# jiangzhongshi/SurfaceNetworks

Hardware: AMD Instinct MI355X
Metric: meshes/sec fwd+bwd, Dirac temporal-predict (higher is better)
Workload: dtype f32; 1 GPU; as_rigid_as_possible Dirac temporal prediction: 64 grid-cloth meshes 71x71 (V=5041,F=9800) per GPU, C=128, 15 layers, fwd+loss+bwd+allreduce+Adam; meshes_per_gpu=64, global_batch=64, parallelism=dp1 (mesh sharding, flat-bucket RCCL all-reduce), world_size=1, rccl_ranks=1, collective_backend=nccl, devices_visible=1, operator_format=q3, operators=pool, grad_bucket_bytes=4075488

## Files before the change

include/sn_spmm.h:

```cpp
#ifndef SN_SPMM_H_
#define SN_SPMM_H_

#include <stddef.h>
#include <stdint.h>

#ifdef __cplusplus
extern "C" {
#endif

#define SN_ABI_VERSION 1

#define SN_OK            0
#define SN_E_NULL       -1
#define SN_E_SHAPE      -2
#define SN_E_RANGE      -3
#define SN_E_LD         -4
#define SN_E_ALIGN      -5
#define SN_E_WORKSPACE  -6
#define SN_E_UNSUPPORTED -7

int         sn_abi_version(void);
const char *sn_status_string(int status);

int sn_spmm_csr_f32(const int32_t *rowptr, const int32_t *colind, const float *vals,
                    int64_t M, int64_t K, int64_t nnz,
                    const float *X, int64_t ldx, int32_t x_group,
                    int32_t N,
                    float *Y, int64_t ldy, int32_t y_group,
                    void *stream);

size_t sn_spmm_csr_stats_workspace_bytes(int64_t M);
int sn_spmm_csr_stats_f32(const int32_t *rowptr, const int32_t *colind, const float *vals, int64_t M, int64_t K, int64_t nnz,
                          const float *X, int64_t ldx, int32_t x_group, int32_t N, float *Y, int64_t ldy, int32_t y_group,
                          double *stats_part, void *workspace, size_t workspace_bytes, void *stream);

int sn_spmm_bsr4_f32(const int32_t *b_rowptr, const int32_t *b_colind, const float *b_vals,
                     int64_t Mb, int64_t Kb, int64_t nblocks,
                     const float *X, int64_t ldx, int32_t x_group,
                     int32_t N,
                     float *Y, int64_t ldy, int32_t y_group,
                     void *stream);

int sn_spmm_q3_f32(const int32_t *b_rowptr, const float *q_blk, int64_t Mb, int64_t Kb, int64_t nblocks,
                   const float *X, int64_t ldx, int32_t x_group, int32_t N,
                   float *Y, int64_t ldy, int32_t y_group, void *stream);
size_t sn_spmm_q3_stats_workspace_bytes(int64_t Mb);
int32_t sn_spmm_q3_stats_blocks(void);
int sn_spmm_q3_stats_f32(const int32_t *b_rowptr, const float *q_blk, int64_t Mb, int64_t Kb, int64_t nblocks, const float *X,
                         int64_t ldx, int32_t x_group, int32_t N, float *Y, int64_t ldy, int32_t y_group, double *stats_part,
                         void *workspace, size_t workspace_bytes, void *stream);
int sn_spmm_q3_elubwd_f32(const int32_t *b_rowptr, const float *q_blk, int64_t Mb, int64_t Kb, int64_t nblocks,
                          const float *X, int64_t ldx, int32_t x_group, int32_t N,
                          const float *E, int64_t lde, const float *G, int64_t ldg,
                          float *Y, int64_t ldy, int32_t y_group, void *stream);
int64_t sn_spmm_q3_absmax_blocks(int64_t Mb, int32_t N);
int sn_spmm_q3_elubwd_absmax_f32(const int32_t *b_rowptr, const float *q_blk, int64_t Mb, int64_t Kb, int64_t nblocks,
                                 const float *X, int64_t ldx, int32_t x_group, int32_t N, const float *E, int64_t lde,
                                 const float *G, int64_t ldg, float *Y, int64_t ldy, int32_t y_group, float *y_absmax,
                                 void *stream);
int sn_bsr4_to_q3_f32(const int32_t *b_colind, const float *b_vals, int64_t nblocks, float *q_blk,
                      int32_t *not_quaternion, void *stream);

int sn_spmm_csr_elubwd_f32(const int32_t *rowptr, const int32_t *colind, const float *vals,
                           int64_t M, int64_t K, int64_t nnz,
                           const float *X, int64_t ldx, int32_t x_group,
                           int32_t N,
                           const float *E, int64_t lde, const float *G, int64_t ldg,
                           float *Y, int64_t ldy, int32_t y_group,
                           void *stream);
int sn_spmm_bsr4_elubwd_f32(const int32_t *b_rowptr, const int32_t *b_colind, const float *b_vals,
                            int64_t Mb, int64_t Kb, int64_t nblocks,
                            const float *X, int64_t ldx, int32_t x_group,
                            int32_t N,
                            const float *E, int64_t lde, const float *G, int64_t ldg,
                            float *Y, int64_t ldy, int32_t y_group,
                            void *stream);

int sn_coo_to_csr_i32(const int64_t *idx_batch, const int64_t *idx_row, const int64_t *idx_col,
                      int64_t nnz, int64_t B, int64_t R, int64_t Kb,
                      int32_t *rowptr, int32_t *colind,
                      void *stream);

size_t sn_csr_transpose_workspace_bytes(int64_t M, int64_t K, int64_t nnz);
int sn_csr_transpose_f32(const int32_t *rowptr, const int32_t *colind, const float *vals,
                         int64_t M, int64_t K, int64_t nnz,
                         int32_t *t_rowptr, int32_t *t_colind, float *t_vals,
                         void *workspace, size_t workspace_bytes,
                         void *stream);

size_t sn_scan_workspace_bytes(int64_t n);
int sn_bsr4_count(const int32_t *rowptr, const int32_t *colind, int64_t M, int64_t K,
                  int32_t *b_rowptr, void *workspace, size_t workspace_bytes, void *stream);
int sn_bsr4_fill(const int32_t *rowptr, const int32_t *colind, const float *vals, int64_t M, int64_t K,
                 const int32_t *b_rowptr, int32_t *b_colind, float *b_vals, void *stream);

int sn_rb4_count(const int32_t *rowptr, const int32_t *colind, int64_t M, int64_t K, int32_t *b_ptr,
                 void *workspace, size_t workspace_bytes, void *stream);
int sn_rb4_fill(const int32_t *rowptr, const int32_t *colind, const float *vals, int64_t M, int64_t K,
                const int32_t *b_ptr, int32_t *b_col, float *b_val, void *stream);
int sn_spmm_rb4_f32(const int32_t *b_ptr, const int32_t *b_col, const float *b_val, int64_t M, int64_t K, int64_t capacity,
                    const float *X, int64_t ldx, int32_t N, float *Y, int64_t ldy, void *stream);
int sn_spmm_rb4_elubwd_f32(const int32_t *b_ptr, const int32_t *b_col, const float *b_val, int64_t M, int64_t K,
                           int64_t capacity, const float *X, int64_t ldx, int32_t N, const float *E, int64_t lde,
                           const float *G, int64_t ldg, float *Y, int64_t ldy, void *stream);
int64_t sn_spmm_rb4_absmax_blocks(int64_t M, int32_t N);
int sn_spmm_rb4_elubwd_absmax_f32(const int32_t *b_ptr, const int32_t *b_col, const float *b_val, int64_t M, int64_t K,
                                  int64_t capacity, const float *X, int64_t ldx, int32_t N, const float *E, int64_t lde,
                                  const float *G, int64_t ldg, float *Y, int64_t ldy, float *y_absmax, void *stream);
size_t sn_spmm_rb4_stats_workspace_bytes(int64_t M);
int sn_spmm_rb4_stats_f32(const int32_t *b_ptr, const int32_t *b_col, const float *b_val, int64_t M, int64_t K,
                          int64_t capacity, const float *X, int64_t ldx, int32_t N, float *Y, int64_t ldy,
                          double *stats_part, void *workspace, size_t workspace_bytes, void *stream);
// ... 190 lines not shown
int64_t sn_graph_apsp_max_vertices(void);
int32_t sn_graph_apsp_group(int64_t n);
int32_t sn_graph_apsp_threads(int64_t n);
int sn_graph_apsp_f32(const int32_t *rowptr, const int32_t *colind, const float *w, int64_t n, int64_t src_begin,
                      int64_t src_count, float *out, int64_t ldo, int32_t *unreached, void *stream);
int sn_graph_apsp_sweeps_f32(const int32_t *rowptr, const int32_t *colind, const float *w, int64_t n, int64_t src_begin,
                             int64_t src_count, float *out, int64_t ldo, int32_t *unreached, int32_t *sweeps, void *stream);
int sn_symmetrize_min_f32(float *G, int64_t n, int64_t ld, void *stream);

#define SN_MESH_CORNER_BYTES 40
size_t sn_mesh_corners_workspace_bytes(int64_t nV);
int sn_mesh_corners_f32(const float *V, const int32_t *F, int64_t nV, int64_t nF, int32_t *cptr, void *corners,
                        int32_t *status_flag, void *workspace, size_t workspace_bytes, void *stream);
int sn_mesh_geodesics_f32(const int32_t *cptr, const void *corners, int64_t n, int64_t src_begin, int64_t src_count,
                          float *out, int64_t ldo, int32_t *flags, void *stream);
int sn_mesh_geodesics_sweeps_f32(const int32_t *cptr, const void *corners, int64_t n, int64_t src_begin, int64_t src_count,
                                 float *out, int64_t ldo, int32_t *flags, int32_t *sweeps, void *stream);

#define SN_IDT_BAD_FACE       1
#define SN_IDT_NOT_CONVERGED  2
#define SN_IDT_DEGENERATE     4
#define SN_IDT_NON_MANIFOLD   8
#define SN_IDT_ORIENTATION    16
#define SN_IDT_THRESHOLD      (-1e-12)
size_t sn_mesh_glue_workspace_bytes(int64_t nV, int64_t nF);
int sn_mesh_glue_i32(const float *V, const int32_t *F, int64_t nV, int64_t nF, int32_t *G, double *l, int32_t *status,
                     void *workspace, size_t workspace_bytes, void *stream);
size_t sn_mesh_idt_workspace_bytes(int64_t nF);
int sn_mesh_idt_rounds_f64(int32_t *Fp, double *lp, int32_t *G, int64_t nF, int32_t round_begin, int32_t round_count,
                           int32_t max_rounds, int32_t *counters, int32_t *status, void *workspace, size_t workspace_bytes,
                           void *stream);
int64_t sn_mesh_idt_laplacian_items(int64_t nV, int64_t nF);
size_t sn_mesh_idt_laplacian_workspace_bytes(int64_t nV, int64_t nF);
int sn_mesh_idt_laplacian_f32(const int32_t *Fp, const double *lp, int64_t nV, int64_t nF, int32_t phase, int64_t *keys,
                              const int64_t *order, int32_t *rowptr, int32_t *colind, float *vals, int32_t *status,
                              void *workspace, size_t workspace_bytes, void *stream);

int sn_linear_fwd_f32(const float *x, int64_t ldx, const float *W, int64_t ldw, const float *bias,
                      const float *residual, int64_t ldr, float *y, int64_t ldy, float *y_elu, int64_t lde,
                      int64_t rows, int32_t K, int32_t J, double *elu_stats_part ,
                      void *stream);
int sn_linear_dgrad_f32(const float *dy, int64_t lddy, const float *W, int64_t ldw, const float *x, int64_t ldx,
                        const float *center, const float *B, const float *Cc, float *dx, int64_t lddx,
                        int64_t rows, int32_t J, int32_t C, void *stream);
int sn_linear_dgrad_elu_f32(const float *dy, int64_t lddy, const float *W, int64_t ldw, const float *x, int64_t ldx,
                            const float *center, const float *B, const float *Cc, float *dx_hi, int64_t lddx,
                            float *gact, int64_t ldga, const float *gadd, int64_t ldgadd,
                            int64_t rows, int32_t J, int32_t C, void *stream);
int32_t sn_linear_dgrad_absmax_blocks(void);
int sn_linear_dgrad_elu_absmax_f32(const float *dy, int64_t lddy, const float *W, int64_t ldw, const float *x, int64_t ldx,
                                   const float *center, const float *B, const float *Cc, float *dx_hi, int64_t lddx,
                                   float *gact, int64_t ldga, const float *gadd, int64_t ldgadd,
                                   int64_t rows, int32_t J, int32_t C, float *gact_absmax, void *stream);
int sn_linear_fwd_segbias_f32(const float *x, int64_t ldx, const float *W, int64_t ldw, const float *segbias,
                              int64_t rows_per_seg, const float *residual, int64_t ldr, float *y, int64_t ldy,
                              float *y_elu, int64_t lde, int64_t rows, int32_t K, int32_t J, double *elu_stats_part,
                              void *stream);
int sn_linear_dgrad_eluseg_f32(const float *dy, int64_t lddy, const float *W, int64_t ldw, const float *x, int64_t ldx,
                               const float *center, const float *B, const float *Cc, const float *segvec,
                               int64_t rows_per_seg, const float *rowmask, float *gact, int64_t ldga, const float *gadd,
                               int64_t ldgadd, int64_t rows, int32_t J, int32_t C, void *stream);
int sn_linear_fwd_tiles_f32(const float *x, int64_t ldx, const float *W, int64_t ldw, const float *bias, const float *residual,
                            int64_t ldr, float *y, int64_t ldy, float *y_elu, int64_t lde, int64_t rows, int32_t K, int32_t J,
                            double *elu_stats_part, float *tile_sums, void *stream);
int sn_linear_fwd_segbias_tiles_f32(const float *x, int64_t ldx, const float *W, int64_t ldw, const float *segbias,
                                    int64_t rows_per_seg, const float *residual, int64_t ldr, float *y, int64_t ldy, float *y_elu,
                                    int64_t lde, int64_t rows, int32_t K, int32_t J, double *elu_stats_part, float *tile_sums,
                                    void *stream);
int sn_avg_stats_from_tiles_f32(const float *tile_sums, const double *stats_part, int32_t nblk, const float *e, int64_t ld,
                                const float *mask, const float *inv_count, int64_t rows_per_seg, int64_t nseg, int32_t C,
                                float *m, double *stats, float *workspace, void *stream);
int sn_avg_stats_from_tiles_ragged_f32(const float *tile_sums, const double *stats_part, int32_t nblk, const float *e, int64_t ld,
                                       const int64_t *segoff, const float *inv_count, int64_t nseg, int32_t C, float *m,
                                       double *stats, float *workspace, void *stream);
int sn_linear_fwd_segbias_ragged_tiles_f32(const float *x, int64_t ldx, const float *W, int64_t ldw, const float *segbias,
                                           const int64_t *segoff, int32_t nseg, const float *residual, int64_t ldr, float *y,
                                           int64_t ldy, float *y_elu, int64_t lde, int64_t rows, int32_t K, int32_t J,
                                           double *elu_stats_part, float *tile_sums, void *stream);
int sn_linear_fwd_segbias_ragged_f32(const float *x, int64_t ldx, const float *W, int64_t ldw, const float *segbias,
                                     const int64_t *segoff, int32_t nseg, const float *residual, int64_t ldr, float *y,
                                     int64_t ldy, float *y_elu, int64_t lde, int64_t rows, int32_t K, int32_t J,
                                     double *elu_stats_part, void *stream);
int sn_linear_dgrad_eluseg_ragged_f32(const float *dy, int64_t lddy, const float *W, int64_t ldw, const float *x, int64_t ldx,
                                      const float *center, const float *B, const float *Cc, const float *segvec,
                                      const int64_t *segoff, int32_t nseg, float *gact, int64_t ldga, const float *gadd,
                                      int64_t ldgadd, int64_t rows, int32_t J, int32_t C, void *stream);
int sn_linear_dgrad_eluseg_absmax_f32(const float *dy, int64_t lddy, const float *W, int64_t ldw, const float *x, int64_t ldx,
                                      const float *center, const float *B, const float *Cc, const float *segvec,
                                      int64_t rows_per_seg, const float *rowmask, float *gact, int64_t ldga, const float *gadd,
                                      int64_t ldgadd, int64_t rows, int32_t J, int32_t C, float *gact_absmax, void *stream);
int sn_linear_dgrad_eluseg_ragged_absmax_f32(const float *dy, int64_t lddy, const float *W, int64_t ldw, const float *x,
                                             int64_t ldx, const float *center, const float *B, const float *Cc,
                                             const float *segvec, const int64_t *segoff, int32_t nseg, float *gact, int64_t ldga,
                                             const float *gadd, int64_t ldgadd, int64_t rows, int32_t J, int32_t C,
                                             float *gact_absmax, void *stream);

typedef struct sn_plan sn_plan;
int sn_plan_create(sn_plan **out);
int sn_plan_destroy(sn_plan *plan);
int32_t sn_plan_lookup(const char *entry_point_name);
int32_t sn_plan_entry_count(void);
const char *sn_plan_entry_name(int32_t fn);
const char *sn_plan_entry_signature(int32_t fn);
int64_t sn_plan_length(const sn_plan *plan);
int sn_plan_add_call(sn_plan *plan, int32_t fn, int32_t nargs, const int32_t *kind, const int32_t *slot, const int64_t *ival,
                     const double *dval);
// ... 17 lines not shown
```

surfacenetworks_amd/_lib.py:

```python
from __future__ import annotations

import ctypes as C
import os
import threading

_HERE = os.path.dirname(os.path.abspath(__file__))
LIB_PATH = os.path.join(_HERE, "libsn_hip.so")

_vp, _i64, _i32, _sz = C.c_void_p, C.c_int64, C.c_int32, C.c_size_t

SIGNATURES = {
    "sn_abi_version": (C.c_int, []),
    "sn_status_string": (C.c_char_p, [C.c_int]),
    "sn_spmm_csr_f32": (C.c_int, [_vp, _vp, _vp, _i64, _i64, _i64, _vp, _i64, _i32, _i32, _vp, _i64, _i32, _vp]),
    "sn_spmm_csr_stats_workspace_bytes": (_sz, [_i64]),
    "sn_spmm_csr_stats_f32": (C.c_int, [_vp, _vp, _vp, _i64, _i64, _i64, _vp, _i64, _i32, _i32, _vp, _i64, _i32, _vp, _vp, _sz, _vp]),
    "sn_spmm_bsr4_f32": (C.c_int, [_vp, _vp, _vp, _i64, _i64, _i64, _vp, _i64, _i32, _i32, _vp, _i64, _i32, _vp]),
    "sn_spmm_csr_elubwd_f32": (C.c_int, [_vp, _vp, _vp, _i64, _i64, _i64, _vp, _i64, _i32, _i32, _vp, _i64, _vp, _i64, _vp, _i64,
                                         _i32, _vp]),
    "sn_spmm_bsr4_elubwd_f32": (C.c_int, [_vp, _vp, _vp, _i64, _i64, _i64, _vp, _i64, _i32, _i32, _vp, _i64, _vp, _i64, _vp, _i64,
                                          _i32, _vp]),
    "sn_spmm_q3_f32": (C.c_int, [_vp, _vp, _i64, _i64, _i64, _vp, _i64, _i32, _i32, _vp, _i64, _i32, _vp]),
    "sn_spmm_q3_stats_workspace_bytes": (_sz, [_i64]),
    "sn_spmm_q3_stats_blocks": (_i32, []),
# ... 5 lines not shown
    "sn_csr_transpose_f32": (C.c_int, [_vp, _vp, _vp, _i64, _i64, _i64, _vp, _vp, _vp, _vp, _sz, _vp]),
    "sn_scan_workspace_bytes": (_sz, [_i64]),
    "sn_bsr4_count": (C.c_int, [_vp, _vp, _i64, _i64, _vp, _vp, _sz, _vp]),
    "sn_bsr4_fill": (C.c_int, [_vp, _vp, _vp, _i64, _i64, _vp, _vp, _vp, _vp]),
    "sn_rb4_count": (C.c_int, [_vp, _vp, _i64, _i64, _vp, _vp, _sz, _vp]),
    "sn_rb4_fill": (C.c_int, [_vp, _vp, _vp, _i64, _i64, _vp, _vp, _vp, _vp]),
    "sn_spmm_rb4_f32": (C.c_int, [_vp, _vp, _vp, _i64, _i64, _i64, _vp, _i64, _i32, _vp, _i64, _vp]),
    "sn_spmm_rb4_elubwd_f32": (C.c_int, [_vp, _vp, _vp, _i64, _i64, _i64, _vp, _i64, _i32, _vp, _i64, _vp, _i64, _vp, _i64, _vp]),
    "sn_spmm_rb4_absmax_blocks": (_i64, [_i64, _i32]),
    "sn_spmm_rb4_elubwd_absmax_f32": (C.c_int, [_vp, _vp, _vp, _i64, _i64, _i64, _vp, _i64, _i32, _vp, _i64, _vp, _i64, _vp, _i64, _vp, _vp]),
    "sn_spmm_rb4_stats_workspace_bytes": (_sz, [_i64]),
    "sn_spmm_rb4_stats_f32": (C.c_int, [_vp, _vp, _vp, _i64, _i64, _i64, _vp, _i64, _i32, _vp, _i64, _vp, _vp, _sz, _vp]),
    "sn_spmm_csr_ring_f32": (C.c_int, [_vp, _vp, _vp, _i64, _i64, _i64, _vp, _i64, _i32, _vp, _i64, _vp]),
    "sn_spmm_csr_ring_elubwd_f32": (C.c_int, [_vp, _vp, _vp, _i64, _i64, _i64, _vp, _i64, _i32, _vp, _i64, _vp, _i64, _vp, _i64, _vp]),
    "sn_spmm_csr_ring_absmax_blocks": (_i64, [_i64, _i32]),
    "sn_spmm_csr_ring_elubwd_absmax_f32": (C.c_int, [_vp, _vp, _vp, _i64, _i64, _i64, _vp, _i64, _i32, _vp, _i64, _vp, _i64, _vp, _i64, _vp,
                                                     _vp]),
    "sn_spmm_csr_ring_stats_workspace_bytes": (_sz, [_i64]),
    "sn_spmm_csr_ring_stats_f32": (C.c_int, [_vp, _vp, _vp, _i64, _i64, _i64, _vp, _i64, _i32, _vp, _i64, _vp, _vp, _sz, _vp]),
    "sn_spmm_csr_ring_half_window": (_i32, []),
    "sn_csr_band_i32": (C.c_int, [_vp, _vp, _i64, _i64, _vp, _vp]),
    "sn_blockdiag_concat_i32": (C.c_int, [_vp, _vp, _vp, _vp, _i64, _i64, _i64, _i64, _i32, _vp, _vp, _vp, _vp]),
    "sn_blockdiag_concat_ragged_i32": (C.c_int, [_vp, _vp, _vp, _vp, _i64, _i64, _i64, _i64, _i32, _vp, _vp, _vp, _vp]),
    "sn_validate_csr_i32": (C.c_int, [_vp, _vp, _vp, _i64, _i64, _i64, _vp, _vp]),
    "sn_elu_into_f32": (C.c_int, [_vp, _i64, _vp, _i64, _i64, _i32, _vp]),
    "sn_elu_bwd_acc_f32": (C.c_int, [_vp, _i64, _vp, _i64, _vp, _i64, _vp, _i64, _vp, _i64, _i64, _i32, _i32, _vp]),
    "sn_colstats_workspace_bytes": (_sz, [_i64, _i32]),
    "sn_colstats_f32": (C.c_int, [_vp, _i64, _i64, _i32, _vp, _vp, _sz, _vp]),
    "sn_wgrad_workspace_bytes": (_sz, [_i64, _i32, _i32]),
    "sn_wgrad_f32": (C.c_int, [_vp, _i64, _vp, _i64, _vp, _i64, _i32, _i32, _vp, _vp, _vp, _sz, _vp]),
    "sn_wgrad_seg_workspace_bytes": (_sz, [_i64, _i64, _i32, _i32]),
    "sn_wgrad_seg_f32": (C.c_int, [_vp, _i64, _vp, _i64, _vp, _i64, _i64, _i32, _i32, _vp, _vp, _vp, _vp, _sz, _vp]),
    "sn_wgrad_slabs_f32": (C.c_int, [_vp, _i64, _vp, _i64, _vp, _i64, _vp, _i32, _vp, _i32, _i32, _i32, _vp, _vp, _vp, _vp, _sz, _vp]),
    "sn_wgrad_bounded_f32": (C.c_int, [_vp, _i64, _vp, _i64, _vp, _i64, _i32, _i32, _vp, _vp, _vp, _sz, _vp, _i64, _vp, _i64, _vp]),
    "sn_wgrad_seg_bounded_f32": (C.c_int, [_vp, _i64, _vp, _i64, _vp, _i64, _i64, _i32, _i32, _vp, _vp, _vp, _vp, _sz, _vp, _i64, _vp,
                                           _i64, _vp]),
    "sn_wgrad_slabs_bounded_f32": (C.c_int, [_vp, _i64, _vp, _i64, _vp, _i64, _vp, _i32, _vp, _i32, _i32, _i32, _vp, _vp, _vp, _vp, _sz,
                                             _vp, _i64, _vp, _i64, _vp]),
    "sn_avg_prep_ragged_f32": (C.c_int, [_vp, _vp, _i64, _i32, _vp, _i32, _vp, _vp]),
    "sn_bn_fold_seg_f32": (C.c_int, [_vp, _i64, _vp, _vp, _vp, _vp, _i32, _i32, C.c_double, C.c_double, _vp, _vp, _vp, _vp, _vp, _vp, _vp,
                                     _vp, _vp, _vp, _i64, _vp, _vp]),
    "sn_avg_bn_bwd_f32": (C.c_int, [_vp, _vp, _vp, _vp, _vp, _vp, _vp, _vp, _vp, _i64, _i32, _i32, _i64, _vp, _i64, _vp, _i64, _vp, _vp,
                                    _vp, _vp, _vp, _vp, _vp, _vp, _vp]),
    "sn_linear_dgrad_absmax_blocks": (_i32, []),
    "sn_linear_dgrad_elu_absmax_f32": (C.c_int, [_vp, _i64, _vp, _i64, _vp, _i64, _vp, _vp, _vp, _vp, _i64, _vp, _i64, _vp, _i64, _i64,
                                                 _i32, _i32, _vp, _vp]),
    "sn_linear_dgrad_eluseg_absmax_f32": (C.c_int, [_vp, _i64, _vp, _i64, _vp, _i64, _vp, _vp, _vp, _vp, _i64, _vp, _vp, _i64, _vp,
                                                    _i64, _i64, _i32, _i32, _vp, _vp]),
    "sn_linear_dgrad_eluseg_ragged_absmax_f32": (C.c_int, [_vp, _i64, _vp, _i64, _vp, _i64, _vp, _vp, _vp, _vp, _vp, _i32, _vp, _i64,
                                                           _vp, _i64, _i64, _i32, _i32, _vp, _vp]),
    "sn_spmm_q3_absmax_blocks": (_i64, [_i64, _i32]),
    "sn_spmm_q3_elubwd_absmax_f32": (C.c_int, [_vp, _vp, _i64, _i64, _i64, _vp, _i64, _i32, _i32, _vp, _i64, _vp, _i64, _vp, _i64, _i32,
                                               _vp, _vp]),
    "sn_wgrad_thin_workspace_bytes": (_sz, [_i64, _i32, _i32]),
    "sn_wgrad_thin_f32": (C.c_int, [_vp, _i64, _vp, _i64, _i64, _i32, _i32, _vp, _vp, _vp, _sz, _vp]),
    "sn_masked_smooth_l1_workspace_bytes": (_sz, [_i64, _i32]),
    "sn_masked_smooth_l1_fwd_f32": (C.c_int, [_vp, _i64, _vp, _i64, _vp, _i64, _i32, C.c_double, _vp, _vp, _sz, _vp]),
    "sn_masked_smooth_l1_bwd_f32": (C.c_int, [_vp, _i64, _vp, _i64, _vp, _i64, _i32, C.c_double, _vp, _vp, _i64, _vp]),
    "sn_pair_argmin_f32": (C.c_int, [_vp, _i64, _i64, _vp, _vp, _i64, _vp, _i64, _i64, _vp, _vp]),
    "sn_pair_ce_fwd_f32": (C.c_int, [_vp, _i64, _vp, _i64, _i64, _vp, _vp, _vp]),
    "sn_pair_ce_bwd_f32": (C.c_int, [_vp, _i64, _vp, _vp, _vp, _i64, _i64, _i64, _i64, _vp, _i64, _vp]),
    "sn_pair_fused_workspace_bytes": (C.c_size_t, [_i64, _i64]),
    "sn_pair_fused_fwd_f32": (C.c_int, [_vp, _i64, _vp, _i64, _vp, _i64, _i64, _i64, _i64, C.c_int32, _vp, _vp, _vp, C.c_size_t, _vp]),
    "sn_pair_fused_bwd_f32": (C.c_int, [_vp, _vp, _vp, _i64, _i64, _i64, _i64, C.c_int32, _vp, _i64, _vp, _i64, _vp, C.c_size_t, _vp]),
    "sn_pair_loss_workspace_bytes": (C.c_size_t, [_i64, _i64]),
    "sn_pair_soft_fwd_f32": (C.c_int, [_vp, _i64, _vp, _i64, _vp, _vp, _vp, _i64, _i64, _i64, _i64, _i64, _i64, C.c_int32, _vp, _vp, _vp, C.c_size_t, _vp]),
    "sn_pair_soft_bwd_f32": (C.c_int, [_vp, _vp, _vp, _i64, _i64, _vp, _vp, _i64, _i64, _i64, _i64, C.c_int32, _vp, _i64, _vp, _i64, _vp, C.c_size_t, _vp]),
    "sn_pair_sl1_fwd_f32": (C.c_int, [_vp, _i64, _vp, _i64, _vp, _vp, _vp, _i64, _i64, _i64, _i64, _i64, _i64, C.c_int32, _vp, _vp, C.c_size_t, _vp]),
    "sn_pair_sl1_bwd_f32": (C.c_int, [_vp, _vp, _vp, _i64, _i64, _vp, _i64, _i64, _i64, _i64, C.c_int32, _vp, _i64, _vp, _i64, _vp, C.c_size_t, _vp]),
    "sn_pair_match_workspace_bytes": (C.c_size_t, [_i64, _i64]),
    "sn_pair_match_f32": (C.c_int, [_vp, _i64, _vp, _i64, _i64, _i64, _i64, _i64, C.c_int32, _vp, _vp, _vp, _vp, _vp, _i64, _vp, _vp, _vp,
                                    C.c_size_t, _vp]),
    "sn_gather_segments_f32": (C.c_int, [_vp, _vp, _i64, _i64, _i64, _i32, _vp, _vp]),
    "sn_gather_segments_ragged_f32": (C.c_int, [_vp, _vp, _vp, _i64, _i64, _i64, _i32, _vp, _vp]),
    "sn_linear_thin_fwd_f32": (C.c_int, [_vp, _i64, _vp, _i64, _vp, _i64, _i32, _i32, _vp, _i64, _vp, _i64, _vp]),
    "sn_bn_fold_f32": (C.c_int, [_vp, _i64, _vp, _vp, _vp, _vp, _i32, _i32, C.c_double, C.c_double, _i32, _vp, _vp, _vp,
                                 _vp, _vp, _vp, _vp, _vp, _vp, _vp]),
    "sn_colstats_blocks": (C.c_int32, [_i64]),
    "sn_wgrad_bounded_enabled": (C.c_int32, []),
    "sn_gemm_variant": (C.c_int32, []),
    "sn_colstats_merge2_f64": (C.c_int, [_vp, C.c_int32, C.c_int32, C.c_int32, _vp, C.c_int32, C.c_int32, C.c_int32, _vp, _vp]),
    "sn_colstats_partial_f32": (C.c_int, [_vp, _i64, _i64, C.c_int32, _vp, _vp]),
    "sn_bn_bwd_coeffs_f32": (C.c_int, [_vp, _vp, _vp, _vp, _vp, _vp, _i64, _i32, _i32, _vp, _vp, _vp, _vp, _vp, _vp, _vp]),
    "sn_segment_colsum_ragged_workspace_bytes": (_sz, [_i64, _i32]),
    "sn_segment_colsum_ragged_f32": (C.c_int, [_vp, _i64, _vp, _i64, _vp, _i64, _i32, _vp, _vp, _vp, _sz, _vp]),
    "sn_bcast_rows_ragged_f32": (C.c_int, [_vp, _vp, _i64, _vp, _i64, _i32, _vp]),
    "sn_segment_colsum_workspace_bytes": (_sz, [_i64, _i64, _i32]),
    "sn_segment_colsum_f32": (C.c_int, [_vp, _i64, _vp, _i64, _i64, _i32, _vp, _vp, _sz, _vp]),
    "sn_bcast_rows_f32": (C.c_int, [_vp, _vp, _i64, _i64, _i64, _i32, _vp]),
    "sn_elu_bwd_bcast_f32": (C.c_int, [_vp, _i64, _vp, _i64, _vp, _vp, _vp, _i64, _vp, _i64, _i64, _i64, _i32, _vp]),
    "sn_dirac_workspace_bytes": (_sz, [_i64, _i64]),
    "sn_dirac_bsr4_from_mesh": (C.c_int, [_vp, _vp, _i64, _i64, _vp, _vp, _vp, _vp, _vp, _vp, _vp, _vp, _vp, _sz, _vp]),
    "sn_timing_enable": (C.c_int, [_i32]),
    "sn_timing_count": (_i64, []),
    "sn_timing_drain": (C.c_int, [_vp, _vp, _i64, _vp]),
    "sn_laplacian_workspace_bytes": (_sz, [_i64, _i64]),
    "sn_laplacian_csr_from_mesh": (C.c_int, [_vp, _vp, _i64, _i64, _i32, _vp, _vp, _vp, _vp, _vp, _sz, _vp]),
    "sn_edge_lengths_csr_f32": (C.c_int, [_vp, _vp, _vp, _i64, _vp, _vp]),
    "sn_graph_apsp_max_vertices": (_i64, []),
    "sn_graph_apsp_group": (_i32, [_i64]),
    "sn_graph_apsp_threads": (_i32, [_i64]),
    "sn_graph_apsp_f32": (C.c_int, [_vp, _vp, _vp, _i64, _i64, _i64, _vp, _i64, _vp, _vp]),
    "sn_graph_apsp_sweeps_f32": (C.c_int, [_vp, _vp, _vp, _i64, _i64, _i64, _vp, _i64, _vp, _vp, _vp]),
    "sn_symmetrize_min_f32": (C.c_int, [_vp, _i64, _i64, _vp]),
    "sn_mesh_corners_workspace_bytes": (_sz, [_i64]),
    "sn_mesh_corners_f32": (C.c_int, [_vp, _vp, _i64, _i64, _vp, _vp, _vp, _vp, _sz, _vp]),
# ... 109 lines not shown
```

surfacenetworks_amd/blocks.py:

```python
from __future__ import annotations

import weakref

import torch

from . import kernels, plans
from .functional import (SpmmTimer, _launch, _rows2d, product_form, avg_stage_backward, avg_stage_backward_ragged, avg_stage_forward,
                         avg_stage_forward_ragged, bn_prepare, bnlin_backward,
                         bnlin_backward_elu_input, bnlin_backward_zero_first, bnlin_forward, bnlin_forward_zero_first, stash, unstash,
                         zero_first_supported)
from .graphs import active_capture
from .operators import as_operator

__all__ = ["lap_block", "dirac_block", "avg_block", "avg_block_ragged", "avg_block_ragged_ok", "take_activated", "attach_activated", "zero_faces_ok", "elu_conv", "elu_conv_ok"]


def _version_of(t: torch.Tensor):
    return None if t.is_inference() else t._version


def attach_activated(t: torch.Tensor, cat: torch.Tensor) -> torch.Tensor:
    t._sn_cat = (cat, _version_of(t))
    return t


def take_activated(t: torch.Tensor, rows: int, C: int):
    d = getattr(t, "__dict__", None)
    entry = d.pop("_sn_cat", None) if d is not None else None
    if entry is None:
        return None
    cat, version = entry
    if version != _version_of(t) or tuple(cat.shape) != (rows, 2 * C) or cat.device != t.device or cat.dtype != torch.float32:
        return None
    return cat


def _new_cat(rows, C, device):
    return torch.empty((rows, 2 * C), dtype=torch.float32, device=device)


def _new_part(rows, C, device, narrow=False):
    if not (C == 128 or (narrow and C == 64 and kernels.linear_fwd_supported(2 * C, C))) or not kernels.elu_stats_supported():
        return None
    return kernels.new_elu_stats_part(rows, device)


def _attach_part(cat, part, tiles=None):
    if part is not None:
        cat._sn_part = part
        if tiles is not None:
            cat._sn_tiles = tiles


_TILE_SUMS_MIN_ROWS = 32768


def _new_tiles(rows, C, device, part, wanted):
    if not wanted or part is None or C != 128 or rows < _TILE_SUMS_MIN_ROWS or not kernels.tile_sums_supported():
        return None
    return kernels.new_tile_sums(rows, device)


def _wants_tiles(mod, avg_next) -> bool:
    if avg_next is None:
        return bool(mod.__dict__.get("_sn_avg_next", False))
    return bool(avg_next)

# ... 39 lines not shown


_MISSING = object()


def _op_operands(ops, ncols):
    arrays, key = [], []
    for op, group in ops:
        for o in (op, op.t()):
            kind, arr, scal = product_form(o, group, ncols)
            arrays.extend(arr)
            key.append((kind, scal))
    return arrays, tuple(key)


def _plan_forward(ctx, site, impl, tensors, ops, consts, ncols, n_dyn, scan):
    op_arrays, op_key = _op_operands(ops, ncols) if ops else ((), ())
    ext, attr_key = plans.expand_ext(tensors, scan)
    ext.extend(op_arrays)
    dyn = tensors[:n_dyn]
    ptrs = [t.data_ptr() if t is not None else 0 for t in dyn]
    key = (tuple([None if t is None else (t.shape, t.stride(), t.dtype) for t in dyn]),
           tuple([None if t is None else t.shape for t in tensors[n_dyn:]]), attr_key, op_key, consts,
           tuple([ptrs.index(p_) for p_ in ptrs]),
           _TILE_SUMS_MIN_ROWS)
    plan, may_record = site.lookup(key)
    if plan is None:
        if not may_record:
            return None
        plan = plans.record(site, key, impl, (*tensors, *[o for o, _ in ops], *consts), ext, tensors[0].device, range(n_dyn))
        if plan is None:
            return None
        need = set()

        def slots(d):
            if isinstance(d, plans._Desc):
                if d.slot >= 2:
                    need.add(d.slot - 2)
            elif isinstance(d, tuple):
                for v in d:
                    slots(v)
        slots(plan.result[1])
        plan.saved_ext = sorted(need)
    timer = SpmmTimer.active
    if timer is not None:
        if plan.tags is None:
            return None
        timer.tags.extend(plan.tags)
    big, small = plan.new_arenas(tensors[0].device)
    plan.run(big, small, ext)
    site.replayed += 1
    build = plans._Builder(big, small, ext)
    outs = build(plan.result[0])
    if plan.effects:
        plans.apply_effects(plan, build)
    ctx._sn_plan = (plan, big, small, [ext[j] for j in plan.saved_ext], ops, ncols)
    return outs


def _plan_backward(ctx, site, impl, grads, consts):
    state = ctx._sn_plan
    if state is None:
        raise RuntimeError("a second backward through a block that ran from a launch plan (retain_graph): its workspace was "
                           "released by the first one; run with SN_PLANS=0 for that")
    fplan, big, small, kept, ops, ncols = state
    ctx._sn_plan = None
    op_arrays, op_key = _op_operands(ops, ncols) if ops else ((), ())
    maxima = [kernels.take_absmax(g) if g is not None else None for g in grads]
    ext = [big, small, *kept, *grads, *maxima, *op_arrays]
    gptrs = [g.data_ptr() if g is not None else 0 for g in grads]
    key = (tuple([None if g is None else (g.shape, g.stride(), g.dtype) for g in grads]), tuple([m is not None for m in maxima]),
           op_key, consts, tuple([gptrs.index(p_) for p_ in gptrs]))
    plan = fplan.bwd.get(key, _MISSING)
    if plan is _MISSING or plan is None:
        fext = [None] * fplan.n_ext
        for j, t in zip(fplan.saved_ext, kept):
            fext[j] = t
        saved = plans._Builder(big, small, fext)(fplan.result[1])
        plans.renote(grads, maxima)
        if plan is None:
            return impl(saved, *[o for o, _ in ops], *grads, *consts)
        g0 = 2 + len(kept)
        plan = plans.record(site, (id(fplan), key), impl, (saved, *[o for o, _ in ops], *grads, *consts), ext,
                            grads_device(grads, big, small), range(g0, g0 + len(grads)))
        fplan.bwd[key] = plan
        if plan is None:
            plans.renote(grads, maxima)
            return impl(saved, *[o for o, _ in ops], *grads, *consts)
        for g in grads:
            if g is not None:
                kernels.take_absmax(g)
    timer = SpmmTimer.active
    if timer is not None:
        if plan.tags is None:
            fext = [None] * fplan.n_ext
            for j, t in zip(fplan.saved_ext, kept):
                fext[j] = t
            plans.renote(grads, maxima)
            return impl(plans._Builder(big, small, fext)(fplan.result[1]), *[o for o, _ in ops], *grads, *consts)
        timer.tags.extend(plan.tags)
    b2, s2 = plan.new_arenas(grads_device(grads, big, small))
    plan.run(b2, s2, ext)
    site.replayed += 1
    build = plans._Builder(b2, s2, ext)
    out = build(plan.result)
    if plan.effects:
        plans.apply_effects(plan, build)
    return out


def grads_device(grads, *others):
    for t in (*grads, *others):
        if t is not None:
            return t.device
    raise ValueError("no tensor to take the device from")


_SITES = {name: plans.Site(name) for name in ("dirac_fwd", "dirac_bwd", "propagate_fwd", "propagate_bwd", "avg_fwd", "avg_bwd",
                                              "avg_ragged_fwd", "avg_ragged_bwd", "elu_conv_fwd", "elu_conv_bwd")}


_NAN = {}


def _nan_placeholder(device):
    t = _NAN.get(device)
    if t is None:
        t = torch.full((1, 1), float("nan"), dtype=torch.float32, device=device)
        if device.type != "cuda" or not torch.cuda.is_current_stream_capturing():
            _NAN[device] = t
    return t


def _dirac_fwd(v, f, pre_v, pre_f, g0, b0, W0, c0, rm0, rv0, g1, b1, W1, c1, rm1, rv1, opDi, opDiA, need_f, avg_next, tr0, mo0,
               ep0, tr1, mo1, ep1):
    rv, C = v.shape
    rf = opDi.shape[0] // 4
    cat1 = _activated(v, pre_v)
    nxt_f = _new_cat(rf, C, v.device)
    pf = _new_part(rf, C, v.device, narrow=True)
    if f is None:
        cat0 = torch.empty((rf, C), dtype=torch.float32, device=v.device)
        _attach_hi(cat0, _launch(opDi, cat1[:, :C], cat0, 4, "fwd", stats=tr0))
        f_out, st0 = bnlin_forward_zero_first(cat0, g0, b0, W0, c0, rm0, rv0, tr0, mo0, ep0, nxt_f[:, :C], need_f, pf)
    else:
        cat0 = pre_f if pre_f is not None else _activated(f, None)
        _attach_hi(cat0, _launch(opDi, cat1[:, :C], cat0[:, C:], 4, "fwd", stats=tr0))
        f_out, st0 = bnlin_forward(cat0, g0, b0, W0, c0, rm0, rv0, tr0, mo0, ep0, None, nxt_f[:, :C], want_y=need_f,
                                   elu_stats=pf)
    _attach_part(nxt_f, pf)
    _attach_hi(cat1, _launch(opDiA, nxt_f[:, :C], cat1[:, C:], 4, "fwd", stats=tr1))
    nxt_v = _new_cat(rv, C, v.device)
    pv = _new_part(rv, C, v.device, narrow=True)
    tv = _new_tiles(rv, C, v.device, pv, avg_next)
    v_new, st1 = bnlin_forward(cat1, g1, b1, W1, c1, rm1, rv1, tr1, mo1, ep1, v, nxt_v[:, :C], elu_stats=pv, tile_sums=tv)
    _attach_part(nxt_v, pv, tv)
    return (v_new, f_out, nxt_v, nxt_f), ((cat0, cat1, nxt_f), st0, st1)


def _dirac_bwd(saved, opDi, opDiA, g_vnew, g_fo, f_zero, need_gv, need_gf):
    (cat0, cat1, nxt_f), st0, st1 = saved
    C = cat1.shape[1] // 2
    dev = cat1.device
    gp1 = (None,) * 4
    h1 = None
    if g_vnew is not None:
        (dx1_hi, h1), dg1, db1, dW1, dc1 = bnlin_backward(st1, g_vnew, through_elu=(g_vnew,))
        gp1 = (dg1, db1, dW1, dc1)
        g_sum = torch.empty((nxt_f.shape[0], C), dtype=torch.float32, device=dev)
        _launch(opDiA.t(), dx1_hi, g_sum, 4, "bwd", elubwd=(nxt_f[:, :C], g_fo))
        g_fo = g_sum
    gp0 = (None,) * 4
    g_v = g_f = None
    dx0_hi = None
    if g_fo is not None and f_zero:
        dx0_hi, dg0, db0, dW0, dc0 = bnlin_backward_zero_first(st0, g_fo)
        gp0 = (dg0, db0, dW0, dc0)
    elif g_fo is not None:
        (dx0_hi, g_f), dg0, db0, dW0, dc0 = bnlin_backward(st0, g_fo, through_elu=(None,))
        gp0 = (dg0, db0, dW0, dc0)
    if need_gv:
        if dx0_hi is not None:
            g_v = torch.empty((cat1.shape[0], C), dtype=torch.float32, device=dev)
            _launch(opDi.t(), dx0_hi, g_v, 4, "bwd", elubwd=(cat1[:, :C], h1))
        else:
            g_v = h1
    if f_zero or not need_gf:
        g_f = None
    return (g_v, g_f) + gp0 + gp1


class _DiracBlock(torch.autograd.Function):

    @staticmethod
    def forward(ctx, v, f, opDi, opDiA, pre_v, pre_f, need_f, avg_next, g0, b0, W0, c0, rm0, rv0, tr0, mo0, ep0, g1, b1, W1, c1,
                rm1, rv1, tr1, mo1, ep1):
        v = _rows2d(v)
        if f is not None and pre_f is None:
            f = _rows2d(f)
        ctx.f_zero = f is None
        ctx.ops = (opDi, opDiA)
        tensors = (v, f, pre_v, pre_f, g0, b0, W0, c0, rm0, rv0, g1, b1, W1, c1, rm1, rv1)
        consts = (need_f, avg_next, tr0, mo0, ep0, tr1, mo1, ep1)
        outs = None
        ctx._sn_plan = None
        if plans.usable(v):
            outs = _plan_forward(ctx, _SITES["dirac_fwd"], _dirac_fwd, tensors, ((opDi, 4), (opDiA, 4)), consts, v.shape[1], 4, (2, 3, 8, 14))
            if outs is not None:
                _drop_counters(rm0, rm1)
        ctx._sn_planned = outs is not None
        if outs is None:
            outs, saved = _dirac_fwd(*tensors, opDi, opDiA, *consts)
            stash(ctx, *saved)
        v_new, f_out, nxt_v, nxt_f = outs
        if f_out is None:
            f_out = _nan_placeholder(v.device).expand(nxt_f.shape[0], v.shape[1])
        ctx.mark_non_differentiable(nxt_v, nxt_f)
        ctx.set_materialize_grads(False)
        return v_new, f_out, nxt_v, nxt_f

    @staticmethod
    def backward(ctx, g_vnew, g_fout, _gv, _gf):
        if g_vnew is None and g_fout is None:
            return (None,) * 26
        opDi, opDiA = ctx.ops
        g_vnew = g_vnew.contiguous() if g_vnew is not None else None
        g_fout = g_fout.contiguous() if g_fout is not None else None
        consts = (ctx.f_zero, bool(ctx.needs_input_grad[0]), bool(ctx.needs_input_grad[1]))
        if ctx._sn_planned:
            r = _plan_backward(ctx, _SITES["dirac_bwd"], _dirac_bwd, (g_vnew, g_fout), consts)
        else:
            r = _dirac_bwd(unstash(ctx), opDi, opDiA, g_vnew, g_fout, *consts)
        none5 = (None,) * 5
        return (r[0], r[1], None, None, None, None, None, None) + r[2:6] + none5 + r[6:10] + none5


def _drop_counters(*running_means) -> None:
    for rm in running_means:
        d = getattr(rm, "__dict__", None)
        if d is not None:
            d.pop("_sn_nbt", None)


def dirac_block(mod, Di, DiA, v, f, need_f=True, num_faces=None, avg_next=None):
    B, V, C = v.shape
    F_ = f.shape[1] if f is not None else int(num_faces)
    rv, rf = B * V, B * F_
    opDi, opDiA = as_operator(Di), as_operator(DiA)
    if opDi.shape != (4 * rf, 4 * rv) or opDiA.shape != (4 * rv, 4 * rf):
        raise ValueError(f"DirResNet2: Di {tuple(opDi.shape)} / DiA {tuple(opDiA.shape)} do not match v rows {rv}, f rows {rf}")
    v_new, f_out, nxt_v, nxt_f = _DiracBlock.apply(v.reshape(rv, C), f.reshape(rf, C) if f is not None else None, opDi, opDiA,
                                                  take_activated(v, rv, C),
                                                  take_activated(f, rf, C) if f is not None else None, bool(need_f),
                                                  _wants_tiles(mod, avg_next), *_bn_args(mod._modules["bn_fc0"]), *_bn_args(mod._modules["bn_fc1"]))
    _mark_producer(nxt_v, mod, avg_next)
    return attach_activated(v_new.view(B, V, C), nxt_v), attach_activated(f_out.view(B, F_, C), nxt_f)


def zero_faces_ok(mod, C: int) -> bool:
    return zero_first_supported(C, mod.bn_fc0.fc.weight.shape[0]) and mod.bn_fc0.fc.weight.shape[1] == 2 * C


def _propagate_fwd(x, pre, mask_rows, inv_count, g0, b0, W0, c0, rm0, rv0, g1, b1, W1, c1, rm1, rv1, op, nseg, avg_next, tr0, mo0,
                   ep0, tr1, mo1, ep1):
    rows, C = x.shape
    per = rows // nseg if nseg else 0

    def propagate(cat, training):
        if op is not None:
            _attach_hi(cat, _launch(op, cat[:, :C], cat[:, C:], 1, "fwd", stats=training))
        else:
            mean = kernels.segment_colsum(cat[:, :C], mask_rows, per, nseg) * inv_count
            kernels.bcast_rows(mean, cat[:, C:], per)

    cat_a = _activated(x, pre)
    propagate(cat_a, tr0)
    cat_b = _new_cat(rows, C, x.device)
    pb = _new_part(rows, C, x.device)
    _, st0 = bnlin_forward(cat_a, g0, b0, W0, c0, rm0, rv0, tr0, mo0, ep0, None, cat_b[:, :C],
                           want_y=False, elu_stats=pb)
    _attach_part(cat_b, pb)
# ... 339 lines not shown
```

surfacenetworks_amd/csrc/sn_gemm.hip:

```cpp
#include <hip/hip_runtime.h>
#include <hip/hip_ext.h>
#include <stdint.h>
#include <stdlib.h>

#include "sn_spmm.h"

int sn_internal_cu_count();
hipError_t sn_internal_fill(void *dst, int value, size_t bytes, hipStream_t s);
hipError_t sn_internal_copy2d(void *dst, int64_t dpitch, const void *src, int64_t spitch, int64_t width, int64_t rows, hipStream_t s);
bool sn_internal_timing_slot(int kind, int64_t rows, int64_t width, int64_t bytes, int outw, hipEvent_t *s, hipEvent_t *e);

namespace {

constexpr int kWG = 256;
#define kCUs sn_internal_cu_count()
typedef float f4 __attribute__((ext_vector_type(4)));
typedef float f16v __attribute__((ext_vector_type(16)));

inline int launch_status() {
  const hipError_t e = hipGetLastError();
  return e == hipSuccess ? SN_OK : (int)e;
}
inline bool aligned16(const void *p) { return (reinterpret_cast<uintptr_t>(p) & 15u) == 0; }
inline bool ld32(int64_t a, int64_t b = 0, int64_t c = 0, int64_t d = 0, int64_t e = 0) {
// ... 193 lines not shown
}
__device__ __forceinline__ unsigned row16_umax(unsigned v) {
  v = dpp_umax<0xB1>(v);
  v = dpp_umax<0x4E>(v);
  v = dpp_umax<0x141>(v);
  v = dpp_umax<0x140>(v);
  return v;
}

template <int I>
struct IC {
  static constexpr int value = I;
};
template <int I, int N, class F>
__device__ __forceinline__ void static_for(F &&f) {
  if constexpr (I < N) {
    f(IC<I>{});
    static_for<I + 1, N>(f);
  }
}

#define SN_LDS_BARRIER() asm volatile("s_waitcnt lgkmcnt(0)\n\ts_barrier" ::: "memory")

typedef __amdgpu_buffer_rsrc_t rsrc_t;
struct RowWindow {
  const char *p;
  int step;
  int n_full, n_last;
  __device__ __forceinline__ void init(const float *base, int64_t ld, int64_t row0, int last_rows, int span) {
    step = 128 * (int)ld;
    p = reinterpret_cast<const char *>(base + row0 * ld);
    n_full = 4 * (31 * (int)ld + span);
    n_last = 4 * ((last_rows - 1) * (int)ld + span);
  }
  __device__ __forceinline__ void init_empty() {
    step = 0;
    p = nullptr;
    n_full = n_last = 0;
  }
  __device__ __forceinline__ void next() { p += step; }
  __device__ __forceinline__ void stride(int g) { step *= g; }
  __device__ __forceinline__ rsrc_t rsrc(int to_last) const {
    const int n = to_last > 0 ? n_full : (to_last == 0 ? n_last : 0);
    return __builtin_amdgcn_make_buffer_rsrc(const_cast<char *>(p), 0, n, 0x00020000);
  }
};
__device__ __forceinline__ f4 bld4(rsrc_t r, int voff) {
  return __builtin_bit_cast(f4, __builtin_amdgcn_raw_buffer_load_b128(r, voff, 0, 0));
}
__device__ __forceinline__ void bst4(rsrc_t r, int voff, const f4 &v) {
  __builtin_amdgcn_raw_buffer_store_b128(__builtin_bit_cast(u4, v), r, voff, 0, 2);
}

template <int PC, int K, int NT, bool TRANSW, int EPI, bool SIDE, bool ELU, bool SMALL = false, int WV = 4>
__global__ __launch_bounds__(64 * WV, (PC == 2 && K == 128 && NT == 1 && WV == 4) ? 2 : 1) void gemm_rows_split_k(const float *__restrict__ In, int64_t ldi,
                                                         const float *__restrict__ W, int64_t ldw,
                                                         float *__restrict__ Out, int64_t ldo, int64_t rows, EpiArgs ep) {
  constexpr int KS = K / 16;
  constexpr int RS = 2 * K + 16;
  constexpr int PART = 32 * RS;
  constexpr int SEG = K / 64;
  constexpr int NCH = 8 / WV;
  constexpr int NL = NCH * SEG;
  constexpr int CSTEP = KS / 2;
  constexpr int NOUT = 32 * WV * NT;
  constexpr int CPR = 8 * NT;
  constexpr int SROW = 16 * CPR + 16;
  constexpr int RPI = 64 / CPR;
  constexpr int NST = 32 / RPI;
  static_assert(PC == 2, "two fp16 pieces");
  __shared__ __attribute__((aligned(16))) unsigned char img[2][PC][PART];
  __shared__ __attribute__((aligned(16))) unsigned char stg[WV][32 * SROW];
  __shared__ float s_rs[2][32];
  __shared__ float s_amax[WV];
  __shared__ __attribute__((aligned(16))) float s_cs[NOUT];
  const int wave = __builtin_amdgcn_readfirstlane(threadIdx.x >> 6), lane = threadIdx.x & 63;
  const int n = lane & 31, h = lane >> 5;
  u4 wh[NT][KS], wl[NT][KS];
  constexpr int kOob = 0x7fffff00;
  const f4 zero4 = {0.f, 0.f, 0.f, 0.f};
  auto load_w = [&](int col, int ks, f4 &p, f4 &q) {
    if constexpr (!TRANSW) {
      p = q = zero4;
      if (col < ep.jv) {
        p = *reinterpret_cast<const f4 *>(W + (int64_t)col * ldw + 16 * ks + 8 * h);
        q = *reinterpret_cast<const f4 *>(W + (int64_t)col * ldw + 16 * ks + 8 * h + 4);
      }
    } else {
      const int k0w = 16 * ks + 8 * h;
      const float *w0 = W + (int64_t)k0w * ldw + col;
      p = q = zero4;
      if (k0w < ep.jv) p = f4{w0[0], w0[ldw], w0[2 * ldw], w0[3 * ldw]};
      if (k0w + 4 < ep.jv) q = f4{w0[4 * ldw], w0[5 * ldw], w0[6 * ldw], w0[7 * ldw]};
    }
  };
#pragma unroll
  for (int t = 0; t < NT; ++t) {
    const int col = 32 * (wave * NT + t) + n;
    float cup = 1.f;
    constexpr bool ONEPASS = SMALL && !(PC == 2 && K == 128 && NT == 1 && !TRANSW && !SIDE);
    f4 wp[ONEPASS ? KS : 1], wq[ONEPASS ? KS : 1];
    if constexpr (ONEPASS) {
#pragma unroll
      for (int ks = 0; ks < KS; ++ks) load_w(col, ks, wp[ks], wq[ks]);
    }
    {
      float cm = 0.f;
#pragma unroll
      for (int ks = 0; ks < KS; ++ks) {
        f4 p, q;
        if constexpr (ONEPASS) p = wp[ks], q = wq[ks];
        else load_w(col, ks, p, q);
        cm = fmaxf(cm, fmaxf(absmax4(p), absmax4(q)));
      }
      cm = fmaxf(cm, __shfl_xor(cm, 32));
      float cdown;
      pow2_scales(cm, cup, cdown);
      if (h == 0) s_cs[col] = cdown;
    }
#pragma unroll
    for (int ks = 0; ks < KS; ++ks) {
      f4 p, q;
      if constexpr (ONEPASS) p = wp[ks], q = wq[ks];
      else load_w(col, ks, p, q);
      split8_h2(p, q, cup, wh[t][ks], wl[t][ks]);
    }
  }
  __syncthreads();
  const int64_t ntiles = (rows + 31) / 32;
  const int64_t per = (ntiles + gridDim.x - 1) / gridDim.x;
  const int G = ep.interleave ? (int)gridDim.x : 1;
  int64_t tile = G > 1 ? (int64_t)blockIdx.x : (int64_t)blockIdx.x * per;
  const int64_t tend = G > 1 ? ntiles : (tile + per < ntiles ? tile + per : ntiles);
  constexpr bool STATS = (EPI == EPI_FWD) && ELU && NT == 1;
  if (tile >= tend) {
    if constexpr (STATS)
      if (ep.stats)
        for (int64_t b = blockIdx.x; b < ep.stats_blocks; b += gridDim.x) ep.stats[b * 256 + threadIdx.x] = 0.0;
    if constexpr (EPI == EPI_DGRAD_ELU)
      if (ep.absmax && threadIdx.x == 0)
        for (int b = blockIdx.x; b < kAbsmaxBlocks; b += gridDim.x) ep.absmax[b] = 0.f;
    return;
  }
  float amax = 0.f;
  double ssum[STATS ? 4 : 1], ssq[STATS ? 4 : 1];
#pragma unroll
  for (int i = 0; i < (STATS ? 4 : 1); ++i) ssum[i] = ssq[i] = 0.0;
  const int erow = lane / CPR;
  const int ecol = 32 * NT * wave + 4 * (lane % CPR);
  f4 k0 = {0.f, 0.f, 0.f, 0.f}, k1 = k0, k2 = k0;
  constexpr bool DGE = (EPI == EPI_DGRAD_ELU);
  static_assert(!DGE || SIDE, "the ELU variant needs the BatchNorm tail operand");
  const bool lowhalf = DGE && 32 * NT * wave < ep.half;
  const bool colv = EPI != EPI_FWD || ecol < ep.jv;
  if constexpr (EPI == EPI_FWD) {
    if (colv) k0 = *reinterpret_cast<const f4 *>(ep.v0 + ecol);
  } else if constexpr (SIDE) {
    if (ep.v1) k0 = *reinterpret_cast<const f4 *>(ep.v1 + ecol);
    k1 = *reinterpret_cast<const f4 *>(ep.v2 + ecol);
    k2 = *reinterpret_cast<const f4 *>(ep.v3 + ecol);
  }
  const f4 kcs = *reinterpret_cast<const f4 *>(s_cs + ecol);
  unsigned char *const sw = &stg[wave][0] + n * SROW + 16 * h;
  const unsigned char *const sr = &stg[wave][0] + erow * SROW + 16 * (lane % CPR);
  const float *side_p = (EPI == EPI_FWD) ? ep.v1 : ep.v0;
  const bool has_out = (EPI != EPI_FWD && !DGE) || Out != nullptr;
  const bool has_ga = DGE && lowhalf && ep.v4 != nullptr;
  const int vo_side = colv ? 4 * (erow * (int)ep.ld1 + ecol) : kOob, js_side = 4 * RPI * (int)ep.ld1;
  const int vo_out = colv ? 4 * (erow * (int)ldo + ecol) : kOob, js_out = 4 * RPI * (int)ldo;
  const int vo_o2 = colv ? 4 * (erow * (int)ep.ld2 + ecol) : kOob, js_o2 = 4 * RPI * (int)ep.ld2;
  const int vo_ga = 4 * (erow * (int)ep.ld3 + ecol), js_ga = 4 * RPI * (int)ep.ld3;
  RowWindow w_in, w_side, w_out, w_o2, w_ga;
  const int64_t row0 = tile * 32;
  const int last_nrt = (int)(rows - (ntiles - 1) * 32);
  int to_last = (int)(ntiles - 1 - tile);
  const int ispan = EPI == EPI_FWD ? K : ep.jv;
  const int ospan = EPI == EPI_FWD ? ep.jv : NOUT;
  w_in.init(In, ldi, row0, last_nrt, ispan);
  if constexpr (SIDE) w_side.init(side_p, ep.ld1, row0, last_nrt, ospan);
  if (has_out) w_out.init(Out, ldo, row0, last_nrt, ospan);
  else w_out.init_empty();
  if constexpr (DGE || (EPI == EPI_FWD && ELU)) w_o2.init(ep.o2, ep.ld2, row0, last_nrt, DGE ? ep.half : ospan);
  if constexpr (DGE) {
    if (has_ga) w_ga.init(ep.v4, ep.ld3, row0, last_nrt, ep.half);
    else w_ga.init_empty();
  }
  if (G > 1) {
    w_in.stride(G);
    if constexpr (SIDE) w_side.stride(G);
    w_out.stride(G);
    if constexpr (DGE || (EPI == EPI_FWD && ELU)) w_o2.stride(G);
    if constexpr (DGE) w_ga.stride(G);
  }
  const bool useseg = (ep.period > 0 || ep.segoff != nullptr) && (EPI == EPI_FWD || (DGE && lowhalf));
  int64_t seg_m = 0;
  int seg_left = 0;
  if (useseg) {
    if (ep.segoff) {
      int lo = 0, hi = ep.nseg - 1;
      while (lo < hi) {
        const int mid = (lo + hi + 1) >> 1;
        if (ep.segoff[mid] <= row0) lo = mid;
        else hi = mid - 1;
      }
      seg_m = lo;
      seg_left = (int)(ep.segoff[lo + 1] - row0);
    } else {
      seg_m = row0 / ep.period;
      seg_left = (int)((seg_m + 1) * ep.period - row0);
    }
  }

  const int lr = lane >> 4, lc = lane & 15;
  const int lrow = 4 * NCH * wave + lr;
  int lvo[SEG];
#pragma unroll
  for (int s = 0; s < SEG; ++s)
    lvo[s] = (EPI == EPI_FWD || 64 * s + 4 * lc < ep.jv) ? 4 * (lrow * (int)ldi + 4 * lc) + 256 * s : kOob;
  const int lps = 16 * (int)ldi;
  f4 raw[NL];
  auto load_chunk = [&](rsrc_t r, int p) {
#pragma unroll
    for (int s = 0; s < SEG; ++s) raw[p * SEG + s] = bld4(r, lvo[s] + p * lps);
  };
  auto convert_chunk = [&](int buf, int p) {
    unsigned char *d = &img[buf][0][0] + (lrow + 4 * p) * RS + 8 * lc;
    float m = absmax4(raw[p * SEG]);
#pragma unroll
    for (int s = 1; s < SEG; ++s) m = fmaxf(m, absmax4(raw[p * SEG + s]));
    float up, down;
    pow2_scales(__uint_as_float(row16_umax(__float_as_uint(m))), up, down);
#pragma unroll
    for (int s = 0; s < SEG; ++s) {
      u2 H, L;
      split4_h2(raw[p * SEG + s], up, H, L);
      *reinterpret_cast<u2 *>(d + 128 * s) = H;
      *reinterpret_cast<u2 *>(d + 128 * s + PART) = L;
    }
    if (lc == 0) s_rs[buf][lrow + 4 * p] = down;
  };
  {
    const rsrc_t r0 = w_in.rsrc(to_last);
#pragma unroll
    for (int p = 0; p < NCH; ++p) load_chunk(r0, p);
    w_in.next();
    const rsrc_t r1 = w_in.rsrc(to_last - G);
#pragma unroll
    for (int p = 0; p < NCH; ++p) {
      convert_chunk(0, p);
      load_chunk(r1, p);
    }
    w_in.next();
  }

  auto do_tile = [&](auto bufc, int64_t tl) {
    constexpr int buf = decltype(bufc)::value;
    SN_LDS_BARRIER();
    const rsrc_t r_in = w_in.rsrc(to_last - 2 * G);
    const int nrt = to_last == 0 ? last_nrt : 32;
    f4 sd[NST];
    if constexpr (SIDE) {
      const rsrc_t r_side = w_side.rsrc(to_last);
#pragma unroll
      for (int j = 0; j < NST; ++j) sd[j] = bld4(r_side, vo_side + j * js_side);
    }
    f4 sg0 = {0.f, 0.f, 0.f, 0.f}, sg1 = sg0;
    float smk[NST];
    int nb = 32;
    const bool usemask = DGE && useseg && ep.rowmask != nullptr;
    if (useseg) {
      while (seg_left <= 0) {
        ++seg_m;
        seg_left += ep.segoff ? (int)(ep.segoff[seg_m + 1] - ep.segoff[seg_m]) : (int)ep.period;
      }
      nb = seg_left < nrt ? seg_left : nrt;
      const float *s0 = ep.segv + seg_m * ep.ldseg + (colv ? ecol : 0);
      const float *s1 = nb < nrt ? s0 + ep.ldseg : s0;
      sg0 = *reinterpret_cast<const f4 *>(s0);
      sg1 = *reinterpret_cast<const f4 *>(s1);
      if constexpr (DGE) {
        if (usemask) {
          const float *mrow = ep.rowmask + tl * 32;
#pragma unroll
          for (int j = 0; j < NST; ++j) {
            const int rt = erow + RPI * j;
            smk[j] = mrow[rt < nrt ? rt : nrt - 1];
          }
        }
      }
    }
    f4 ga[NST];
    if constexpr (DGE) {
      if (lowhalf) {
        const rsrc_t r_ga = w_ga.rsrc(to_last);
#pragma unroll
        for (int j = 0; j < NST; ++j) ga[j] = bld4(r_ga, vo_ga + j * js_ga);
      }
    }
    f16v acc0[NT], acc1[NT];
    const f16v zero = {0.f, 0.f, 0.f, 0.f, 0.f, 0.f, 0.f, 0.f, 0.f, 0.f, 0.f, 0.f, 0.f, 0.f, 0.f, 0.f};
    const unsigned char *fp = &img[buf][0][0] + n * RS + 16 * h;
    constexpr int LOWP = PART;
    const float rs = s_rs[buf][n];
    u4 dh = *reinterpret_cast<const u4 *>(fp), dl = *reinterpret_cast<const u4 *>(fp + LOWP);
    static_for<0, KS>([&](auto ic) {
      constexpr int ks = decltype(ic)::value;
      __builtin_amdgcn_sched_barrier(0);
      u4 nh, nl;
      if constexpr (ks + 1 < KS) {
        nh = *reinterpret_cast<const u4 *>(fp + 32 * (ks + 1));
        nl = *reinterpret_cast<const u4 *>(fp + LOWP + 32 * (ks + 1));
      }
      if constexpr (ks % CSTEP == 0 && ks / CSTEP < NCH) {
        constexpr int p = ks / CSTEP;
        convert_chunk(buf ^ 1, p);
        load_chunk(r_in, p);
      }
#pragma unroll
      for (int t = 0; t < NT; ++t) acc1[t] = mfma_f16(wl[t][ks], dh, ks == 0 ? zero : acc1[t]);
#pragma unroll
      for (int t = 0; t < NT; ++t) acc0[t] = mfma_f16(wh[t][ks], dh, ks == 0 ? zero : acc0[t]);
#pragma unroll
      for (int t = 0; t < NT; ++t) acc1[t] = mfma_f16(wh[t][ks], dl, acc1[t]);
      if constexpr (ks + 1 < KS) {
        dh = nh; dl = nl;
      }
    });
    __builtin_amdgcn_sched_barrier(0);
#pragma unroll
    for (int t = 0; t < NT; ++t)
#pragma unroll
      for (int g = 0; g < 4; ++g)
        *reinterpret_cast<f4 *>(sw + 128 * t + 32 * g) =
            f4{__builtin_fmaf(acc1[t][4 * g], kLowDown, acc0[t][4 * g]) * rs,
               __builtin_fmaf(acc1[t][4 * g + 1], kLowDown, acc0[t][4 * g + 1]) * rs,
               __builtin_fmaf(acc1[t][4 * g + 2], kLowDown, acc0[t][4 * g + 2]) * rs,
               __builtin_fmaf(acc1[t][4 * g + 3], kLowDown, acc0[t][4 * g + 3]) * rs};
    const rsrc_t r_out = w_out.rsrc(to_last);
    rsrc_t r_o2 = r_out;
    if constexpr (DGE || (EPI == EPI_FWD && ELU)) r_o2 = w_o2.rsrc(to_last);
    auto out_row = [&](int j) {
      f4 v = *reinterpret_cast<const f4 *>(sr + RPI * j * SROW);
      v *= kcs;
      if constexpr (EPI == EPI_FWD) {
        if (useseg) v += (erow + RPI * j < nb ? sg0 : sg1);
        else v += k0;
        if constexpr (SIDE) v += sd[j];
      } else if constexpr (SIDE) {
        const f4 xv = sd[j] - k0;
        v.x += __builtin_fmaf(xv.x, k1.x, k2.x);
        v.y += __builtin_fmaf(xv.y, k1.y, k2.y);
        v.z += __builtin_fmaf(xv.z, k1.z, k2.z);
        v.w += __builtin_fmaf(xv.w, k1.w, k2.w);
      }
      return v;
    };
    if constexpr (DGE) {
      if (lowhalf) {
#pragma unroll
        for (int j = 0; j < NST; ++j) {
          f4 v = out_row(j);
          const f4 o = sd[j];
          if (useseg) {
            f4 sv = erow + RPI * j < nb ? sg0 : sg1;
            if (usemask) sv *= smk[j];
            v += sv;
          }
          v = f4{__builtin_fmaf(v.x, fminf(o.x, 0.f), v.x), __builtin_fmaf(v.y, fminf(o.y, 0.f), v.y),
                 __builtin_fmaf(v.z, fminf(o.z, 0.f), v.z), __builtin_fmaf(v.w, fminf(o.w, 0.f), v.w)};
          v += ga[j];
          bst4(r_o2, vo_o2 + j * js_o2, v);
          const float m4 = fmaxf(fmaxf(__builtin_fabsf(v.x), __builtin_fabsf(v.y)), fmaxf(__builtin_fabsf(v.z), __builtin_fabsf(v.w)));
          amax = (erow + RPI * j < nrt) ? fmaxf(amax, m4) : amax;
        }
      } else {
#pragma unroll
        for (int j = 0; j < NST; ++j) bst4(r_out, vo_out + j * js_out, out_row(j));
      }
    } else {
      f4 tsum = {0.f, 0.f, 0.f, 0.f};
#pragma unroll
      for (int j = 0; j < NST; ++j) {
        const f4 v = out_row(j);
        bst4(r_out, vo_out + j * js_out, v);
        if constexpr (EPI == EPI_FWD && ELU) {
          const f4 ev = f4{elu1(v.x), elu1(v.y), elu1(v.z), elu1(v.w)};
          bst4(r_o2, vo_o2 + j * js_o2, ev);
          if constexpr (STATS) {
            if (erow + RPI * j < nrt) {
              const double e0 = ev.x, e1 = ev.y, e2 = ev.z, e3 = ev.w;
              ssum[0] += e0; ssum[1] += e1; ssum[2] += e2; ssum[3] += e3;
              ssq[0] = __builtin_fma(e0, e0, ssq[0]); ssq[1] = __builtin_fma(e1, e1, ssq[1]);
              ssq[2] = __builtin_fma(e2, e2, ssq[2]); ssq[3] = __builtin_fma(e3, e3, ssq[3]);
              tsum += ev;
            }
          }
        }
      }
      if constexpr (STATS) {
        if (ep.tile_sums) {
#pragma unroll
          for (int o = CPR; o < 64; o <<= 1) {
            tsum.x += __shfl_xor(tsum.x, o); tsum.y += __shfl_xor(tsum.y, o);
            tsum.z += __shfl_xor(tsum.z, o); tsum.w += __shfl_xor(tsum.w, o);
          }
          if (erow == 0) *reinterpret_cast<f4 *>(ep.tile_sums + tl * 128 + ecol) = tsum;
        }
      }
    }
    w_in.next();
// ... 236 lines not shown
    }
    w_in.next();
    to_last -= G;
    if constexpr (SIDE) w_side.next();
    w_out.next();
    if constexpr (ELU) w_o2.next();
  };
  while (true) {
    do_tile(IC<0>{});
    if ((tile += G) >= tend) break;
    do_tile(IC<1>{});
    if ((tile += G) >= tend) break;
  }
  if constexpr (STATS) {
    if (ep.stats) {
#pragma unroll
      for (int i = 0; i < 4; ++i)
#pragma unroll
        for (int o = 4; o < 64; o <<= 1) {
          ssum[i] += __shfl_xor(ssum[i], o);
          ssq[i] += __shfl_xor(ssq[i], o);
        }
      if (erow == 0) {
#pragma unroll
        for (int i = 0; i < 4; ++i) {
          ep.stats[(int64_t)blockIdx.x * 256 + ecol + i] = ssum[i];
          ep.stats[(int64_t)blockIdx.x * 256 + 128 + ecol + i] = ssq[i];
        }
      }
      if (threadIdx.x < 256)
        for (int64_t b = blockIdx.x + gridDim.x; b < ep.stats_blocks; b += gridDim.x) ep.stats[b * 256 + threadIdx.x] = 0.0;
    }
  }
}

inline int gemm_variant() {
  static const int v = [] {
    const char *e = getenv("SN_GEMM_VARIANT");
    return (e && atoi(e) == 0) ? 0 : 2;
  }();
  return v;
}

#define SN_UNPAREN(...) __VA_ARGS__
constexpr int64_t kSmallRows = 131072;
#define SN_SPLIT_LAUNCH(TARGS, ...)                                                                                    \
  do {                                                                                                                 \
    if (rows <= kSmallRows) {                                                                                          \
      if (t_start) hipExtLaunchKernelGGL((gemm_rows_split_k<2, SN_UNPAREN TARGS, true>), dim3(grid), dim3(kWG), 0, s, t_start, t_stop, 0, __VA_ARGS__); \
      else hipLaunchKernelGGL((gemm_rows_split_k<2, SN_UNPAREN TARGS, true>), dim3(grid), dim3(kWG), 0, s, __VA_ARGS__); \
    } else {                                                                                                           \
      if (t_start) hipExtLaunchKernelGGL((gemm_rows_split_k<2, SN_UNPAREN TARGS>), dim3(grid), dim3(kWG), 0, s, t_start, t_stop, 0, __VA_ARGS__); \
      else hipLaunchKernelGGL((gemm_rows_split_k<2, SN_UNPAREN TARGS>), dim3(grid), dim3(kWG), 0, s, __VA_ARGS__);     \
    }                                                                                                                  \
  } while (0)
#define SN_SPLIT_LAUNCH_NT2(K_, EPI_, SIDE_, ...) SN_SPLIT_LAUNCH((K_, 2, true, EPI_, SIDE_, false), __VA_ARGS__)

inline int gemm_wgs(int K, int NT) { return (gemm_variant() == 2 && K == 128 && NT == 1) ? 2 : 1; }
inline unsigned gemm_grid(int64_t rows, int wgs) {
  const int64_t ntiles = (rows + 31) / 32;
  int64_t b = (int64_t)kCUs * wgs;
  if (b > ntiles) b = ntiles;
  return (unsigned)(b < 1 ? 1 : b);
}

}

extern "C" {

int32_t sn_gemm_variant(void) { return gemm_variant(); }

int32_t sn_linear_fwd_stats_blocks(int64_t rows) { return rows > 0 ? (int32_t)gemm_grid(rows, 2) : 0; }

int sn_linear_fwd_f32(const float *x, int64_t ldx, const float *W, int64_t ldw, const float *bias,
                      const float *residual, int64_t ldr, float *y, int64_t ldy, float *y_elu, int64_t lde,
                      int64_t rows, int32_t K, int32_t J, double *elu_stats_part, void *stream) {
  return sn_linear_fwd_tiles_f32(x, ldx, W, ldw, bias, residual, ldr, y, ldy, y_elu, lde, rows, K, J, elu_stats_part, nullptr, stream);
}

int sn_linear_fwd_tiles_f32(const float *x, int64_t ldx, const float *W, int64_t ldw, const float *bias,
                            const float *residual, int64_t ldr, float *y, int64_t ldy, float *y_elu, int64_t lde,
                            int64_t rows, int32_t K, int32_t J, double *elu_stats_part, float *tile_sums, void *stream) {
  (void)hipGetLastError();
  if (tile_sums && (!elu_stats_part || J != 128)) return SN_E_UNSUPPORTED;
  if (rows < 0 || K < 1 || J < 1 || ldx < K || ldw < K || (y && ldy < J)) return SN_E_SHAPE;
  if (J > 128 || (J % 4) || (J != 128 && gemm_variant() == 0) || (K != 128 && K != 256) || !ld32(ldx, ldy, ldr, lde))
    return SN_E_UNSUPPORTED;
  if (rows == 0) return SN_OK;
  if (!x || !W || !bias || (!y && !(y_elu && gemm_variant() != 0))) return SN_E_NULL;
  if (!aligned16(x) || !aligned16(W) || !aligned16(bias) || (y && (!aligned16(y) || (ldy % 4))) || (ldx % 4) || (ldw % 4) ||
      (residual && (!aligned16(residual) || (ldr % 4) || ldr < J)) || (y_elu && (!aligned16(y_elu) || (lde % 4) || lde < J)))
    return SN_E_ALIGN;
  if (elu_stats_part && (!y_elu || gemm_variant() == 0)) return SN_E_UNSUPPORTED;
  EpiArgs ep{bias, residual, nullptr, nullptr, y_elu, ldr, lde, nullptr, 0, 0, nullptr, 0, 0, nullptr, elu_stats_part,
             sn_linear_fwd_stats_blocks(rows), (int)J, nullptr, 0, nullptr, 1, tile_sums};
  hipStream_t s = static_cast<hipStream_t>(stream);
  const unsigned grid = gemm_grid(rows, gemm_wgs(K, 1));
  const bool x3 = gemm_variant() != 0;
  hipEvent_t t_start = nullptr, t_stop = nullptr;
  if (x3)
    sn_internal_timing_slot(0x100 | (residual ? 2 : 0) | (y_elu ? 1 : 0) | (y ? 4 : 0), rows, K,
                            rows * 4 * ((int64_t)K + (y ? J : 0) + (residual ? J : 0) + (y_elu ? J : 0)), J, &t_start, &t_stop);
#define SN_X3_FWD(KK, RES, EL) SN_SPLIT_LAUNCH((KK, 1, false, EPI_FWD, RES, EL), x, ldx, W, ldw, y, ldy, rows, ep)
#define SN_W8_FWD(KK, RES, EL)                                                                                         \
  do {                                                                                                                 \
    if (t_start) hipExtLaunchKernelGGL((gemm_fwd_w8_k<KK, RES, EL>), dim3(grid8), dim3(512), 0, s, t_start, t_stop, 0, x, ldx, W, ldw, y, ldy, rows, ep); \
// ... 49 lines not shown
    SN_SPLIT_LAUNCH_NT2(128, EPI_DGRAD, false, dy, lddy, W, ldw, dx, lddx, rows, ep);
  else if (C == 256)
    hipLaunchKernelGGL((gemm_rows_k<128, 2, true, EPI_DGRAD>), dim3(grid), dim3(kWG), 0, s, dy, lddy, W, ldw, dx, lddx, rows, ep);
  else if (x3 && B)
    SN_SPLIT_LAUNCH((128, 1, true, EPI_DGRAD, true, false), dy, lddy, W, ldw, dx, lddx, rows, ep);
  else if (x3)
    SN_SPLIT_LAUNCH((128, 1, true, EPI_DGRAD, false, false), dy, lddy, W, ldw, dx, lddx, rows, ep);
  else
    hipLaunchKernelGGL((gemm_rows_k<128, 1, true, EPI_DGRAD>), dim3(grid), dim3(kWG), 0, s, dy, lddy, W, ldw, dx, lddx, rows, ep);
  return launch_status();
}

int32_t sn_linear_dgrad_absmax_blocks(void) { return kAbsmaxBlocks; }

int sn_linear_dgrad_elu_f32(const float *dy, int64_t lddy, const float *W, int64_t ldw, const float *x, int64_t ldx,
                            const float *center, const float *B, const float *Cc, float *dx_hi, int64_t lddx, float *gact,
                            int64_t ldga, const float *gadd, int64_t ldgadd, int64_t rows, int32_t J, int32_t C,
                            void *stream) {
  return sn_linear_dgrad_elu_absmax_f32(dy, lddy, W, ldw, x, ldx, center, B, Cc, dx_hi, lddx, gact, ldga, gadd, ldgadd, rows, J, C,
                                        nullptr, stream);
}

int sn_linear_dgrad_elu_absmax_f32(const float *dy, int64_t lddy, const float *W, int64_t ldw, const float *x, int64_t ldx,
                                   const float *center, const float *B, const float *Cc, float *dx_hi, int64_t lddx, float *gact,
                                   int64_t ldga, const float *gadd, int64_t ldgadd, int64_t rows, int32_t J, int32_t C,
                                   float *gact_absmax, void *stream) {
  (void)hipGetLastError();
  if (rows < 0 || J < 1 || C < 2 || lddy < J || ldw < C || lddx < C / 2 || ldga < C / 2 || ldx < C) return SN_E_SHAPE;
  if (J > 128 || (J % 4) || (C != 128 && C != 256) || gemm_variant() == 0 || !ld32(lddy, ldx, lddx, ldga, ldgadd))
    return SN_E_UNSUPPORTED;
  if (rows == 0) {
    if (gact_absmax && sn_internal_fill(gact_absmax, 0, kAbsmaxBlocks * sizeof(float), static_cast<hipStream_t>(stream)) != hipSuccess)
      return (int)hipGetLastError();
    return SN_OK;
  }
  if (!dy || !W || !dx_hi || !gact || !x || !B || !Cc) return SN_E_NULL;
  if (!aligned16(dy) || !aligned16(W) || !aligned16(dx_hi) || !aligned16(gact) || !aligned16(x) || !aligned16(B) ||
      !aligned16(Cc) || (center && !aligned16(center)) || (gadd && (!aligned16(gadd) || (ldgadd % 4) || ldgadd < C / 2)) ||
      (lddy % 4) || (ldw % 4) || (lddx % 4) || (ldga % 4) || (ldx % 4))
    return SN_E_ALIGN;
  const int half = C / 2;
  EpiArgs ep{x, center, B, Cc, gact, ldx, ldga, gadd, ldgadd, half, nullptr, 0, 0, nullptr, nullptr, 0, (int)J, nullptr, 0, gact_absmax, 1, nullptr};
  float *out = dx_hi - half;
  hipStream_t s = static_cast<hipStream_t>(stream);
  const unsigned grid = gemm_grid(rows, gemm_wgs(128, C / 128));
  hipEvent_t t_start = nullptr, t_stop = nullptr;
  sn_internal_timing_slot(0x200 | 2 | (gadd ? 4 : 0), rows, C, rows * 4 * ((int64_t)J + C + C + (gadd ? half : 0)), J, &t_start, &t_stop);
  if (C == 256)
    SN_SPLIT_LAUNCH_NT2(128, EPI_DGRAD_ELU, true, dy, lddy, W, ldw, out,
                       lddx, rows, ep);
  else
    SN_SPLIT_LAUNCH((128, 1, true, EPI_DGRAD_ELU, true, false), dy, lddy, W, ldw, out,
                       lddx, rows, ep);
  return launch_status();
}

static int fwd_segbias_launch(const float *x, int64_t ldx, const float *W, int64_t ldw, const float *segbias,
                              int64_t rows_per_seg, const int64_t *segoff, int32_t nseg, const float *residual, int64_t ldr,
                              float *y, int64_t ldy, float *y_elu, int64_t lde, int64_t rows, int32_t K, int32_t J,
                              double *elu_stats_part, void *stream, float *tile_sums = nullptr) {
  (void)hipGetLastError();
  if (rows < 0 || K < 1 || J < 1 || ldx < K || ldw < K || (y && ldy < J) || (!segoff && rows_per_seg < 1) || (segoff && nseg < 1))
    return SN_E_SHAPE;
  if (J > 128 || (J % 4) || (K != 128 && K != 256) || gemm_variant() == 0 || !ld32(ldx, ldy, ldr, lde) ||
      (!segoff && (rows_per_seg < 32 || rows_per_seg > 0x7fffffffLL)))
    return SN_E_UNSUPPORTED;
  if (rows == 0) return SN_OK;
  if (!x || !W || !segbias || (!y && !y_elu)) return SN_E_NULL;
  if (!aligned16(x) || !aligned16(W) || !aligned16(segbias) || (y && (!aligned16(y) || (ldy % 4))) || (ldx % 4) || (ldw % 4) ||
      (residual && (!aligned16(residual) || (ldr % 4) || ldr < J)) || (y_elu && (!aligned16(y_elu) || (lde % 4) || lde < J)))
    return SN_E_ALIGN;
  if (elu_stats_part && !y_elu) return SN_E_UNSUPPORTED;
  if (tile_sums && (!elu_stats_part || J != 128)) return SN_E_UNSUPPORTED;
  EpiArgs ep{segbias, residual, nullptr, nullptr, y_elu, ldr, lde, nullptr, 0, 0, segbias, segoff ? 0 : rows_per_seg, J, nullptr,
             elu_stats_part, sn_linear_fwd_stats_blocks(rows), (int)J, segoff, nseg, nullptr, 1, tile_sums};
  hipStream_t s = static_cast<hipStream_t>(stream);
  const unsigned grid = gemm_grid(rows, gemm_wgs(K, 1));
  hipEvent_t t_start = nullptr, t_stop = nullptr;
  sn_internal_timing_slot(0x100 | 8 | (residual ? 2 : 0) | (y_elu ? 1 : 0) | (y ? 4 : 0), rows, K,
                          rows * 4 * ((int64_t)K + (y ? J : 0) + (residual ? J : 0) + (y_elu ? J : 0)), J, &t_start, &t_stop);
  const int sel = (K == 256 ? 4 : 0) + (residual ? 2 : 0) + (y_elu ? 1 : 0);
  switch (sel) {
    case 0: SN_X3_FWD(128, false, false); break;
    case 1: SN_X3_FWD(128, false, true); break;
    case 2: SN_X3_FWD(128, true, false); break;
    case 3: SN_X3_FWD(128, true, true); break;
    case 4: SN_X3_FWD(256, false, false); break;
    case 5: SN_X3_FWD(256, false, true); break;
    case 6: SN_X3_FWD(256, true, false); break;
    default: SN_X3_FWD(256, true, true); break;
  }
  return launch_status();
}

int sn_linear_fwd_segbias_f32(const float *x, int64_t ldx, const float *W, int64_t ldw, const float *segbias,
                              int64_t rows_per_seg, const float *residual, int64_t ldr, float *y, int64_t ldy, float *y_elu,
                              int64_t lde, int64_t rows, int32_t K, int32_t J, double *elu_stats_part, void *stream) {
  return fwd_segbias_launch(x, ldx, W, ldw, segbias, rows_per_seg, nullptr, 0, residual, ldr, y, ldy, y_elu, lde, rows, K, J,
                            elu_stats_part, stream);
}

int sn_linear_fwd_segbias_tiles_f32(const float *x, int64_t ldx, const float *W, int64_t ldw, const float *segbias,
                                    int64_t rows_per_seg, const float *residual, int64_t ldr, float *y, int64_t ldy, float *y_elu,
                                    int64_t lde, int64_t rows, int32_t K, int32_t J, double *elu_stats_part, float *tile_sums,
                                    void *stream) {
  return fwd_segbias_launch(x, ldx, W, ldw, segbias, rows_per_seg, nullptr, 0, residual, ldr, y, ldy, y_elu, lde, rows, K, J,
// ... 96 lines not shown
```

surfacenetworks_amd/csrc/sn_kernels.hip:

```cpp

#include <hip/hip_runtime.h>
#include <hip/hip_ext.h>
#include <limits.h>
#include <stdint.h>
#include <stdlib.h>

#include <mutex>
#include <vector>

#include "sn_spmm.h"

int sn_internal_cu_count();
hipError_t sn_internal_fill(void *dst, int value, size_t bytes, hipStream_t s);
hipError_t sn_internal_copy2d(void *dst, int64_t dpitch, const void *src, int64_t spitch, int64_t width, int64_t rows, hipStream_t s);

namespace {

constexpr int kWG = 256;
__constant__ int c_xcd = 8;
#define kCUs sn_internal_cu_count()

typedef float f4 __attribute__((ext_vector_type(4)));

__device__ __forceinline__ f4 ld4(const float *p) { return *reinterpret_cast<const f4 *>(p); }
__device__ __forceinline__ void st4(float *p, f4 v) { *reinterpret_cast<f4 *>(p) = v; }
__device__ __forceinline__ void st4_stream(float *p, f4 v) { __builtin_nontemporal_store(v, reinterpret_cast<f4 *>(p)); }
constexpr int kStreamNT = 1;
__device__ __forceinline__ f4 ld4_s(const float *p, int nt) {
  return nt ? __builtin_nontemporal_load(reinterpret_cast<const f4 *>(p)) : *reinterpret_cast<const f4 *>(p);
}
__device__ __forceinline__ void st4_s(float *p, f4 v, int nt) {
  if (nt) __builtin_nontemporal_store(v, reinterpret_cast<f4 *>(p));
  else *reinterpret_cast<f4 *>(p) = v;
}
__device__ __forceinline__ f4 fma4(float a, f4 x, f4 acc) {
  acc.x = __builtin_fmaf(a, x.x, acc.x);
  acc.y = __builtin_fmaf(a, x.y, acc.y);
  acc.z = __builtin_fmaf(a, x.z, acc.z);
  acc.w = __builtin_fmaf(a, x.w, acc.w);
  return acc;
}

template <int G, int N>
__device__ __forceinline__ int64_t row_off(int r, int64_t ld) {
  if constexpr (G == 1) return (int64_t)r * ld;
  else return (int64_t)(r >> 2) * ld + (int64_t)(r & 3) * N;
}

__device__ __forceinline__ int my_chunk(int nchunks) {
  const int X = c_xcd;
  const int cpx = (nchunks + X - 1) / X;
  return (blockIdx.x % X) * cpx + blockIdx.x / X;
}


struct SpmmEpi {
  const float *e;
  int64_t lde;
  const float *g;
  int64_t ldg;
  float *absmax = nullptr;
};
__device__ __forceinline__ f4 fabs4(const f4 &a) {
  return f4{__builtin_fabsf(a.x), __builtin_fabsf(a.y), __builtin_fabsf(a.z), __builtin_fabsf(a.w)};
}
__device__ __forceinline__ float hmax_abs4(const f4 &a) {
  return fmaxf(fmaxf(__builtin_fabsf(a.x), __builtin_fabsf(a.y)), fmaxf(__builtin_fabsf(a.z), __builtin_fabsf(a.w)));
}
__device__ __forceinline__ float wave_max_nonneg(float m) {
  unsigned mb = __float_as_uint(m);
#pragma unroll
  for (int o = 32; o > 0; o >>= 1) {
    const unsigned other = (unsigned)__shfl_xor((int)mb, o);
    mb = other > mb ? other : mb;
  }
  return __uint_as_float(mb);
}
__device__ __forceinline__ f4 elu_bwd4(const f4 &a, const f4 &o) {
  return f4{a.x * (o.x > 0.f ? 1.f : o.x + 1.f), a.y * (o.y > 0.f ? 1.f : o.y + 1.f), a.z * (o.z > 0.f ? 1.f : o.z + 1.f),
            a.w * (o.w > 0.f ? 1.f : o.w + 1.f)};
}

template <int N, int XG, int YG, bool EPI, bool STATS>
__device__ __forceinline__ void spmm_csr_rows_body(const int *__restrict__ rowptr, const int *__restrict__ colind,
                                                   const float *__restrict__ vals, int M, const float *__restrict__ X,
                                                   int64_t ldx, float *__restrict__ Y, int64_t ldy, int nchunks, int iters,
                                                   SpmmEpi epi, float *__restrict__ stats_part) {
  constexpr int LPR = N / 4;
  constexpr int P = 64 / LPR;
  constexpr int WAVES = kWG / 64;
  constexpr int CAP = 512;
  constexpr int KB = 8;
  __shared__ int s_col[WAVES][CAP];
  __shared__ float s_val[WAVES][CAP];
  __shared__ int s_rp[WAVES][68];
  const int wave = threadIdx.x >> 6, lane = threadIdx.x & 63;
  const int sub = lane % LPR, grp = lane / LPR;
  const float *xb = X + sub * 4;
  int *sc = s_col[wave];
  float *sv = s_val[wave];
  int *rp = s_rp[wave];
  const int R = P * iters;
  const int r0 = (my_chunk(nchunks) * WAVES + wave) * R;
  if constexpr (!STATS) {
    if (r0 >= M) return;
  }
  {
    int rl = r0 + lane;
    rl = rl < M ? rl : M;
    rp[lane] = rowptr[rl];
    int re = r0 + R;
    re = re < M ? re : M;
    if (lane == 0) rp[64] = rowptr[r0 < M ? re : M];
  }
  __builtin_amdgcn_wave_barrier();
  const int k0 = rp[0];
  const int k1 = R < 64 ? rp[R] : rp[64];
  const bool fast = (k1 - k0) <= CAP;
  if (fast) {
    for (int p0 = 0; p0 < k1 - k0; p0 += 64) {
      int p = p0 + lane;
      p = p < k1 - k0 ? p : k1 - k0 - 1;
      __builtin_amdgcn_global_load_lds(colind + k0 + p, sc + p0, 4, 0, 0);
      __builtin_amdgcn_global_load_lds(vals + k0 + p, sv + p0, 4, 0, 0);
    }
    asm volatile("s_waitcnt vmcnt(0)" ::: "memory");
    __builtin_amdgcn_wave_barrier();
  }
  f4 ssum = {0.f, 0.f, 0.f, 0.f}, ssq = ssum;
  for (int i = 0; i < iters; ++i) {
    const int lr = i * P + grp;
    const int r = r0 + lr;
    const int kb = rp[lr];
// ... 178 lines not shown
      st4_stream(yp, acc0);
      st4_stream(yp + ys, acc1);
      st4_stream(yp + 2 * ys, acc2);
      st4_stream(yp + 3 * ys, acc3);
    }
  }
}
#define SN_FOUR_WAVES __attribute__((amdgpu_waves_per_eu(4, 4)))
#define SN_SIX_WAVES __attribute__((amdgpu_waves_per_eu(6, 6)))
#define SN_FIVE_WAVES __attribute__((amdgpu_waves_per_eu(5, 5)))
template <int N, int XG, int YG>
__global__ __launch_bounds__(kWG) SN_FOUR_WAVES void spmm_bsr4_lds(const int *__restrict__ b_rowptr, const int *__restrict__ b_colind,
                                                     const float *__restrict__ b_vals, int Mb,
                                                     const float *__restrict__ X, int64_t ldx,
                                                     float *__restrict__ Y, int64_t ldy, int nchunks) {
  spmm_bsr4_lds_body<N, XG, YG, false>(b_rowptr, b_colind, b_vals, Mb, X, ldx, Y, ldy, nchunks, SpmmEpi{nullptr, 0, nullptr, 0});
}
template <int N, int XG, int YG>
__global__ __launch_bounds__(kWG) SN_FOUR_WAVES void spmm_bsr4_lds_epi(const int *__restrict__ b_rowptr, const int *__restrict__ b_colind,
                                                         const float *__restrict__ b_vals, int Mb,
                                                         const float *__restrict__ X, int64_t ldx,
                                                         float *__restrict__ Y, int64_t ldy, int nchunks, SpmmEpi epi) {
  spmm_bsr4_lds_body<N, XG, YG, true>(b_rowptr, b_colind, b_vals, Mb, X, ldx, Y, ldy, nchunks, epi);
}

template <int N, int XG, int YG, bool EPI, bool STATS = false, int UNROLL = 3>
__device__ __forceinline__ void spmm_q3_lds_body(const int *__restrict__ b_rowptr, const f4 *__restrict__ q_blk, int Mb,
                                                 const float *__restrict__ X, int64_t ldx, float *__restrict__ Y,
                                                 int64_t ldy, int nchunks, SpmmEpi epi, float *__restrict__ stats_part = nullptr) {
  constexpr int LPR = N / 4;
  constexpr int RPW = 64 / LPR;
  constexpr int WAVES = kWG / 64;
  constexpr int TILE = 64;
  __shared__ f4 s_blk[WAVES][TILE];
  const int wave = threadIdx.x >> 6, lane = threadIdx.x & 63;
  const int sub = lane % LPR, grp = lane / LPR;
  const int64_t xq = (XG == 4) ? ldx : 4 * ldx;
  const int64_t xs = (XG == 4) ? (int64_t)N : ldx;
  const int64_t yq = (YG == 4) ? ldy : 4 * ldy;
  const int64_t ys = (YG == 4) ? (int64_t)N : ldy;
  const float *xb = X + sub * 4;
  f4 *sv = s_blk[wave];
  const int r0 = (my_chunk(nchunks) * WAVES + wave) * RPW;
  const bool stays = STATS || (EPI && epi.absmax != nullptr);
  if (!stays) {
    if (r0 >= Mb) return;
  }
  const int br = r0 + grp;
  const int brc = br < Mb ? br : Mb;
  const int kb = b_rowptr[brc];
  const int ke = b_rowptr[brc + 1 <= Mb ? brc + 1 : Mb];
  const int k0 = __builtin_amdgcn_readfirstlane(kb);
  const int k1 = (stays && r0 >= Mb) ? k0 : __builtin_amdgcn_readlane(ke, 63);
  f4 acc0 = {0.f, 0.f, 0.f, 0.f}, acc1 = acc0, acc2 = acc0, acc3 = acc0;
  for (int t0 = k0; t0 < k1; t0 += TILE) {
    const int nt = (k1 - t0) < TILE ? (k1 - t0) : TILE;
    {
      const int p = lane < nt ? lane : nt - 1;
      __builtin_amdgcn_global_load_lds(q_blk + t0 + p, sv, 16, 0, 0);
    }
    asm volatile("s_waitcnt vmcnt(0)" ::: "memory");
    __builtin_amdgcn_wave_barrier();
    int k = kb > t0 ? kb : t0;
    const int kend = ke < t0 + nt ? ke : t0 + nt;
#pragma unroll UNROLL
    for (; k < kend; ++k) {
      const f4 q = sv[k - t0];
      const int bc = __float_as_int(q.w);
      const float *xp = xb + (int64_t)bc * xq;
      const f4 x0 = ld4(xp), x1 = ld4(xp + xs), x2 = ld4(xp + 2 * xs), x3 = ld4(xp + 3 * xs);
      acc0 = fma4(q.x, x1, acc0);  acc0 = fma4(q.y, x2, acc0);  acc0 = fma4(q.z, x3, acc0);
      acc1 = fma4(-q.x, x0, acc1); acc1 = fma4(q.z, x2, acc1);  acc1 = fma4(-q.y, x3, acc1);
      acc2 = fma4(-q.y, x0, acc2); acc2 = fma4(-q.z, x1, acc2); acc2 = fma4(q.x, x3, acc2);
      acc3 = fma4(-q.z, x0, acc3); acc3 = fma4(q.y, x1, acc3);  acc3 = fma4(-q.x, x2, acc3);
    }
    __builtin_amdgcn_wave_barrier();
  }
  if constexpr (EPI) {
    if (br < Mb) {
      const int64_t eq = (YG == 4) ? epi.lde : 4 * epi.lde, es = (YG == 4) ? (int64_t)N : epi.lde;
      const float *ep = epi.e + (int64_t)br * eq + sub * 4;
      const f4 e0 = ld4_s(ep, kStreamNT), e1 = ld4_s(ep + es, kStreamNT), e2 = ld4_s(ep + 2 * es, kStreamNT),
               e3 = ld4_s(ep + 3 * es, kStreamNT);
      acc0 = elu_bwd4(acc0, e0); acc1 = elu_bwd4(acc1, e1); acc2 = elu_bwd4(acc2, e2); acc3 = elu_bwd4(acc3, e3);
      if (epi.g) {
        const int64_t gq = (YG == 4) ? epi.ldg : 4 * epi.ldg, gs = (YG == 4) ? (int64_t)N : epi.ldg;
        const float *gp = epi.g + (int64_t)br * gq + sub * 4;
        acc0 += ld4_s(gp, kStreamNT); acc1 += ld4_s(gp + gs, kStreamNT);
        acc2 += ld4_s(gp + 2 * gs, kStreamNT); acc3 += ld4_s(gp + 3 * gs, kStreamNT);
      }
    }
  }
  if (br < Mb) {
    float *yp = Y + (int64_t)br * yq + sub * 4;
    st4_stream(yp, acc0);
    st4_stream(yp + ys, acc1);
    st4_stream(yp + 2 * ys, acc2);
    st4_stream(yp + 3 * ys, acc3);
  }
  if constexpr (EPI) {
    if (epi.absmax) {
      __shared__ float s_am[WAVES];
      float m = 0.f;
      if (br < Mb) {
        const f4 a = fabs4(acc0), b = fabs4(acc1), c = fabs4(acc2), d = fabs4(acc3);
        m = fmaxf(fmaxf(fmaxf(fmaxf(a.x, a.y), fmaxf(a.z, a.w)), fmaxf(fmaxf(b.x, b.y), fmaxf(b.z, b.w))),
                  fmaxf(fmaxf(fmaxf(c.x, c.y), fmaxf(c.z, c.w)), fmaxf(fmaxf(d.x, d.y), fmaxf(d.z, d.w))));
      }
      unsigned mb = __float_as_uint(m);
#pragma unroll
      for (int o = 32; o > 0; o >>= 1) {
        const unsigned other = (unsigned)__shfl_xor((int)mb, o);
        mb = other > mb ? other : mb;
      }
      if (lane == 0) s_am[wave] = __uint_as_float(mb);
      __syncthreads();
      if (threadIdx.x == 0) {
        float t = s_am[0];
#pragma unroll
        for (int w = 1; w < WAVES; ++w) t = fmaxf(t, s_am[w]);
        epi.absmax[blockIdx.x] = t;
      }
    }
  }
  if constexpr (STATS) {
    static_assert((N == 32 || N == 16) && YG == 4 && !EPI, "statistics: 128- or 64-channel rows in the group-4 layout");
    constexpr int CH = 4 * N;
    constexpr int ST = N == 32 ? 160 : 80;
    __shared__ float s_st[WAVES][RPW * ST];
    __shared__ float s_wv[WAVES][2 * CH];
    float *st = s_st[wave];
    const bool live = br < Mb;
    const f4 z = {0.f, 0.f, 0.f, 0.f};
    f4 *row = reinterpret_cast<f4 *>(st + grp * ST + sub * 4);
    row[0] = live ? acc0 : z;
    row[N / 4] = live ? acc1 : z;
    row[2 * N / 4] = live ? acc2 : z;
    row[3 * N / 4] = live ? acc3 : z;
    __builtin_amdgcn_wave_barrier();
    if constexpr (N == 32) {
      float sa = 0.f, sb = 0.f, qa = 0.f, qb = 0.f;
#pragma unroll
// ... 1704 lines not shown
  hipStream_t s = static_cast<hipStream_t>(stream);
  hipEvent_t t_start, t_stop;
  timing_slot(1 | (epi.e ? 2 : 0) | (epi.g ? 4 : 0), 4 * Mb, 4 * Kb, nblocks, N, &t_start, &t_stop);
  const int rpb = kWG / (N / 4);
  const int64_t nchunks = (Mb + rpb - 1) / rpb;
  const unsigned grid = chunk_grid(nchunks);
  if (epi.e)
    SN_DISPATCH_N(spmm_bsr4_lds_epi, N, x_group, y_group, grid, s, b_rowptr, b_colind, b_vals, (int)Mb, X, ldx, Y, ldy, (int)nchunks, epi);
  else
    SN_DISPATCH_N(spmm_bsr4_lds, N, x_group, y_group, grid, s, b_rowptr, b_colind, b_vals, (int)Mb, X, ldx, Y, ldy, (int)nchunks);
  return launch_status();
}

int sn_spmm_bsr4_f32(const int32_t *b_rowptr, const int32_t *b_colind, const float *b_vals, int64_t Mb,
                     int64_t Kb, int64_t nblocks, const float *X, int64_t ldx, int32_t x_group,
                     int32_t N, float *Y, int64_t ldy, int32_t y_group, void *stream) {
  (void)hipGetLastError();
  return spmm_bsr4_launch(b_rowptr, b_colind, b_vals, Mb, Kb, nblocks, X, ldx, x_group, N, Y, ldy, y_group,
                          SpmmEpi{nullptr, 0, nullptr, 0}, stream);
}

int sn_spmm_bsr4_elubwd_f32(const int32_t *b_rowptr, const int32_t *b_colind, const float *b_vals, int64_t Mb, int64_t Kb,
                            int64_t nblocks, const float *X, int64_t ldx, int32_t x_group, int32_t N, const float *E,
                            int64_t lde, const float *G, int64_t ldg, float *Y, int64_t ldy, int32_t y_group,
                            void *stream) {
  (void)hipGetLastError();
  if (!E) return SN_E_NULL;
  return spmm_bsr4_launch(b_rowptr, b_colind, b_vals, Mb, Kb, nblocks, X, ldx, x_group, N, Y, ldy, y_group,
                          SpmmEpi{E, lde, G, ldg}, stream);
}

static int spmm_q3_launch(const int32_t *b_rowptr, const float *q_blk, int64_t Mb, int64_t Kb, int64_t nblocks, const float *X,
                          int64_t ldx, int32_t x_group, int32_t N, float *Y, int64_t ldy, int32_t y_group, SpmmEpi epi,
                          void *stream, float *stats_part = nullptr, double *stats_out = nullptr) {
  (void)hipGetLastError();
  if (Mb < 0 || Kb < 0 || nblocks < 0 || N < 1) return SN_E_SHAPE;
  if (!fits_i32(4 * Mb + 1) || !fits_i32(4 * Kb) || !fits_i32(nblocks)) return SN_E_RANGE;
  if (Mb == 0) return SN_OK;
  if (!b_rowptr || (nblocks > 0 && !q_blk)) return SN_E_NULL;
  int st = check_dense(Y, ldy, y_group, N);
  if (st) return st;
  if (Kb > 0 || nblocks > 0) {
    st = check_dense(X, ldx, x_group, N);
    if (st) return st;
  }
  if (!(N == 16 || N == 32 || N == 64 || N == 128)) return SN_E_UNSUPPORTED;
  if (!aligned16(X) || !aligned16(Y) || !aligned16(q_blk) || ldx % 4 || ldy % 4) return SN_E_ALIGN;
  if (epi.e) {
    st = check_dense(epi.e, epi.lde, y_group, N);
    if (!st && epi.g) st = check_dense(epi.g, epi.ldg, y_group, N);
    if (st) return st;
    if (!aligned16(epi.e) || epi.lde % 4 || (epi.g && (!aligned16(epi.g) || epi.ldg % 4))) return SN_E_ALIGN;
  }
  hipStream_t s = static_cast<hipStream_t>(stream);
  hipEvent_t t_start, t_stop;
  timing_slot(1 | 8 | (epi.e ? 2 : 0) | (epi.g ? 4 : 0) | (stats_part ? 16 : 0), 4 * Mb, 4 * Kb, nblocks, N, &t_start, &t_stop);
  const int rpb = kWG / (N / 4);
  const int64_t nchunks = (Mb + rpb - 1) / rpb;
  const unsigned grid = chunk_grid(nchunks);
  const f4 *q = reinterpret_cast<const f4 *>(q_blk);
  const bool wide = nblocks <= 4 * Mb || grid < 8u * kCUs;
  if (stats_part) {
    if (epi.e || (N != 32 && N != 16) || y_group != 4) return SN_E_UNSUPPORTED;
    if (!stats_out) return SN_E_NULL;
    if (N == 16) {
      if (wide) {
        if (x_group == 4) SN_KLAUNCH((spmm_q3_lds_stats_wide<16, 4, 4>), grid, s, b_rowptr, q, (int)Mb, X, ldx, Y, ldy, (int)nchunks, stats_part);
        else SN_KLAUNCH((spmm_q3_lds_stats_wide<16, 1, 4>), grid, s, b_rowptr, q, (int)Mb, X, ldx, Y, ldy, (int)nchunks, stats_part);
      } else {
        if (x_group == 4) SN_KLAUNCH((spmm_q3_lds_stats<16, 4, 4>), grid, s, b_rowptr, q, (int)Mb, X, ldx, Y, ldy, (int)nchunks, stats_part);
        else SN_KLAUNCH((spmm_q3_lds_stats<16, 1, 4>), grid, s, b_rowptr, q, (int)Mb, X, ldx, Y, ldy, (int)nchunks, stats_part);
      }
      hipLaunchKernelGGL(spmm_stats_reduce_k, dim3(kSpmmStatsBlocks), dim3(kWG), 0, s, stats_part, (int64_t)grid, stats_out, 128);
      return launch_status();
    }
    if (wide) {
      if (x_group == 4) SN_KLAUNCH((spmm_q3_lds_stats_wide<32, 4, 4>), grid, s, b_rowptr, q, (int)Mb, X, ldx, Y, ldy, (int)nchunks, stats_part);
      else SN_KLAUNCH((spmm_q3_lds_stats_wide<32, 1, 4>), grid, s, b_rowptr, q, (int)Mb, X, ldx, Y, ldy, (int)nchunks, stats_part);
    } else {
      if (x_group == 4) SN_KLAUNCH((spmm_q3_lds_stats<32, 4, 4>), grid, s, b_rowptr, q, (int)Mb, X, ldx, Y, ldy, (int)nchunks, stats_part);
      else SN_KLAUNCH((spmm_q3_lds_stats<32, 1, 4>), grid, s, b_rowptr, q, (int)Mb, X, ldx, Y, ldy, (int)nchunks, stats_part);
    }
    hipLaunchKernelGGL(spmm_stats_reduce_k, dim3(kSpmmStatsBlocks), dim3(kWG), 0, s, stats_part, (int64_t)grid, stats_out);
    return launch_status();
  }
  if (epi.e) {
    if (wide) SN_DISPATCH_N(spmm_q3_lds_epi_wide, N, x_group, y_group, grid, s, b_rowptr, q, (int)Mb, X, ldx, Y, ldy, (int)nchunks, epi);
    else SN_DISPATCH_N(spmm_q3_lds_epi, N, x_group, y_group, grid, s, b_rowptr, q, (int)Mb, X, ldx, Y, ldy, (int)nchunks, epi);
  } else {
    if (wide) SN_DISPATCH_N(spmm_q3_lds_wide, N, x_group, y_group, grid, s, b_rowptr, q, (int)Mb, X, ldx, Y, ldy, (int)nchunks);
    else SN_DISPATCH_N(spmm_q3_lds, N, x_group, y_group, grid, s, b_rowptr, q, (int)Mb, X, ldx, Y, ldy, (int)nchunks);
  }
  return launch_status();
}

int sn_spmm_q3_f32(const int32_t *b_rowptr, const float *q_blk, int64_t Mb, int64_t Kb, int64_t nblocks, const float *X,
                   int64_t ldx, int32_t x_group, int32_t N, float *Y, int64_t ldy, int32_t y_group, void *stream) {
  return spmm_q3_launch(b_rowptr, q_blk, Mb, Kb, nblocks, X, ldx, x_group, N, Y, ldy, y_group, SpmmEpi{nullptr, 0, nullptr, 0},
                        stream);
}

size_t sn_spmm_q3_stats_workspace_bytes(int64_t Mb) {
  if (Mb < 1) return 0;
  const int64_t nchunks = (Mb + 31) / 32;
  return (size_t)chunk_grid(nchunks) * 256 * sizeof(float);
}

int sn_spmm_q3_stats_f32(const int32_t *b_rowptr, const float *q_blk, int64_t Mb, int64_t Kb, int64_t nblocks, const float *X,
                         int64_t ldx, int32_t x_group, int32_t N, float *Y, int64_t ldy, int32_t y_group, double *stats_part,
                         void *workspace, size_t workspace_bytes, void *stream) {
  if (!stats_part || !workspace) return SN_E_NULL;
  if (workspace_bytes < sn_spmm_q3_stats_workspace_bytes(Mb)) return SN_E_WORKSPACE;
  return spmm_q3_launch(b_rowptr, q_blk, Mb, Kb, nblocks, X, ldx, x_group, N, Y, ldy, y_group, SpmmEpi{nullptr, 0, nullptr, 0},
                        stream, static_cast<float *>(workspace), stats_part);
}

int32_t sn_spmm_q3_stats_blocks(void) { return kSpmmStatsBlocks; }

int sn_spmm_q3_elubwd_f32(const int32_t *b_rowptr, const float *q_blk, int64_t Mb, int64_t Kb, int64_t nblocks,
                          const float *X, int64_t ldx, int32_t x_group, int32_t N, const float *E, int64_t lde,
                          const float *G, int64_t ldg, float *Y, int64_t ldy, int32_t y_group, void *stream) {
  if (!E) return SN_E_NULL;
  return spmm_q3_launch(b_rowptr, q_blk, Mb, Kb, nblocks, X, ldx, x_group, N, Y, ldy, y_group, SpmmEpi{E, lde, G, ldg}, stream);
}

int64_t sn_spmm_q3_absmax_blocks(int64_t Mb, int32_t N) {
  if (Mb < 1 || !(N == 16 || N == 32 || N == 64 || N == 128)) return 0;
  const int rpb = kWG / (N / 4);
  return (int64_t)chunk_grid((Mb + rpb - 1) / rpb);
}

int sn_spmm_q3_elubwd_absmax_f32(const int32_t *b_rowptr, const float *q_blk, int64_t Mb, int64_t Kb, int64_t nblocks,
                                 const float *X, int64_t ldx, int32_t x_group, int32_t N, const float *E, int64_t lde,
                                 const float *G, int64_t ldg, float *Y, int64_t ldy, int32_t y_group, float *y_absmax,
                                 void *stream) {
  if (!E) return SN_E_NULL;
  return spmm_q3_launch(b_rowptr, q_blk, Mb, Kb, nblocks, X, ldx, x_group, N, Y, ldy, y_group, SpmmEpi{E, lde, G, ldg, y_absmax},
                        stream);
}

int sn_bsr4_to_q3_f32(const int32_t *b_colind, const float *b_vals, int64_t nblocks, float *q_blk, int32_t *not_quaternion,
                      void *stream) {
  (void)hipGetLastError();
  if (nblocks < 0) return SN_E_SHAPE;
  if (!not_quaternion) return SN_E_NULL;
  hipStream_t s = static_cast<hipStream_t>(stream);
  hipError_t e = sn_internal_fill(not_quaternion, 0, sizeof(int32_t), s);
  if (e != hipSuccess) return (int)e;
  if (nblocks == 0) return SN_OK;
  if (!b_colind || !b_vals || !q_blk) return SN_E_NULL;
  if (!aligned16(b_vals) || !aligned16(q_blk)) return SN_E_ALIGN;
  hipLaunchKernelGGL(bsr4_to_q3_k, dim3(grid_for(nblocks, kWG)), dim3(kWG), 0, s, b_colind, b_vals, nblocks,
                     reinterpret_cast<f4 *>(q_blk), not_quaternion);
  return launch_status();
}

int sn_coo_to_csr_i32(const int64_t *idx_batch, const int64_t *idx_row, const int64_t *idx_col,
                      int64_t nnz, int64_t B, int64_t R, int64_t Kb, int32_t *rowptr, int32_t *colind,
                      void *stream) {
  (void)hipGetLastError();
  if (nnz < 0 || B < 1 || R < 0 || Kb < 0) return SN_E_SHAPE;
  const int64_t M = B * R;
  if (!fits_i32(M + 1) || !fits_i32(B * Kb) || !fits_i32(nnz)) return SN_E_RANGE;
  if (!rowptr || (nnz > 0 && (!idx_row || !idx_col || !colind))) return SN_E_NULL;
  const int64_t n = (M + 1 > nnz) ? M + 1 : nnz;
  hipLaunchKernelGGL(coo_to_csr_k, dim3(grid_for(n, kWG)), dim3(kWG), 0, static_cast<hipStream_t>(stream),
                     idx_batch, idx_row, idx_col, nnz, M, R, Kb, rowptr, colind);
  return launch_status();
}

size_t sn_scan_workspace_bytes(int64_t n) {
  if (n < 0) n = 0;
  return (size_t)((n + kScanTile - 1) / kScanTile + 1) * sizeof(int);
}

size_t sn_csr_transpose_workspace_bytes(int64_t M, int64_t K, int64_t nnz) {
  (void)M;
  (void)nnz;
  if (K < 0) K = 0;
  const size_t cursor = ((size_t)K * sizeof(int) + 15) & ~(size_t)15;
  return cursor + sn_scan_workspace_bytes(K + 1);
}

int sn_csr_transpose_f32(const int32_t *rowptr, const int32_t *colind, const float *vals, int64_t M,
                         int64_t K, int64_t nnz, int32_t *t_rowptr, int32_t *t_colind, float *t_vals,
                         void *workspace, size_t workspace_bytes, void *stream) {
  (void)hipGetLastError();
  if (M < 0 || K < 0 || nnz < 0) return SN_E_SHAPE;
  if (!fits_i32(M + 1) || !fits_i32(K + 1) || !fits_i32(nnz)) return SN_E_RANGE;
  if (!t_rowptr || !rowptr) return SN_E_NULL;
  if (nnz > 0 && (!colind || !vals || !t_colind || !t_vals)) return SN_E_NULL;
// ... 246 lines not shown
```

surfacenetworks_amd/csrc/sn_plan_table.inc:

```
SN_PLAN_FN(sn_spmm_csr_f32)
SN_PLAN_FN(sn_spmm_csr_stats_f32)
SN_PLAN_FN(sn_spmm_bsr4_f32)
SN_PLAN_FN(sn_spmm_csr_elubwd_f32)
SN_PLAN_FN(sn_spmm_bsr4_elubwd_f32)
SN_PLAN_FN(sn_spmm_q3_f32)
SN_PLAN_FN(sn_spmm_q3_stats_f32)
SN_PLAN_FN(sn_spmm_q3_elubwd_f32)
SN_PLAN_FN(sn_bsr4_to_q3_f32)
SN_PLAN_FN(sn_coo_to_csr_i32)
SN_PLAN_FN(sn_csr_transpose_f32)
SN_PLAN_FN(sn_bsr4_count)
SN_PLAN_FN(sn_bsr4_fill)
SN_PLAN_FN(sn_rb4_count)
SN_PLAN_FN(sn_rb4_fill)
SN_PLAN_FN(sn_spmm_rb4_f32)
SN_PLAN_FN(sn_spmm_rb4_elubwd_f32)
SN_PLAN_FN(sn_spmm_rb4_elubwd_absmax_f32)
SN_PLAN_FN(sn_spmm_rb4_stats_f32)
SN_PLAN_FN(sn_spmm_csr_ring_f32)
SN_PLAN_FN(sn_spmm_csr_ring_elubwd_f32)
SN_PLAN_FN(sn_spmm_csr_ring_elubwd_absmax_f32)
SN_PLAN_FN(sn_spmm_csr_ring_stats_f32)
SN_PLAN_FN(sn_csr_band_i32)
SN_PLAN_FN(sn_blockdiag_concat_i32)
SN_PLAN_FN(sn_blockdiag_concat_ragged_i32)
SN_PLAN_FN(sn_validate_csr_i32)
SN_PLAN_FN(sn_elu_into_f32)
SN_PLAN_FN(sn_elu_bwd_acc_f32)
SN_PLAN_FN(sn_colstats_f32)
SN_PLAN_FN(sn_wgrad_f32)
SN_PLAN_FN(sn_wgrad_seg_f32)
SN_PLAN_FN(sn_wgrad_slabs_f32)
SN_PLAN_FN(sn_wgrad_bounded_f32)
SN_PLAN_FN(sn_wgrad_seg_bounded_f32)
SN_PLAN_FN(sn_wgrad_slabs_bounded_f32)
SN_PLAN_FN(sn_avg_prep_ragged_f32)
SN_PLAN_FN(sn_bn_fold_seg_f32)
SN_PLAN_FN(sn_avg_bn_bwd_f32)
SN_PLAN_FN(sn_linear_dgrad_elu_absmax_f32)
SN_PLAN_FN(sn_linear_dgrad_eluseg_absmax_f32)
SN_PLAN_FN(sn_linear_dgrad_eluseg_ragged_absmax_f32)
SN_PLAN_FN(sn_spmm_q3_elubwd_absmax_f32)
SN_PLAN_FN(sn_wgrad_thin_f32)
SN_PLAN_FN(sn_masked_smooth_l1_fwd_f32)
SN_PLAN_FN(sn_masked_smooth_l1_bwd_f32)
SN_PLAN_FN(sn_pair_argmin_f32)
SN_PLAN_FN(sn_pair_ce_fwd_f32)
SN_PLAN_FN(sn_pair_ce_bwd_f32)
SN_PLAN_FN(sn_pair_fused_fwd_f32)
SN_PLAN_FN(sn_pair_fused_bwd_f32)
SN_PLAN_FN(sn_pair_soft_fwd_f32)
SN_PLAN_FN(sn_pair_soft_bwd_f32)
SN_PLAN_FN(sn_pair_sl1_fwd_f32)
SN_PLAN_FN(sn_pair_sl1_bwd_f32)
SN_PLAN_FN(sn_pair_match_f32)
SN_PLAN_FN(sn_gather_segments_f32)
SN_PLAN_FN(sn_gather_segments_ragged_f32)
SN_PLAN_FN(sn_linear_thin_fwd_f32)
SN_PLAN_FN(sn_bn_fold_f32)
SN_PLAN_FN(sn_colstats_merge2_f64)
SN_PLAN_FN(sn_colstats_partial_f32)
SN_PLAN_FN(sn_bn_bwd_coeffs_f32)
SN_PLAN_FN(sn_segment_colsum_ragged_f32)
SN_PLAN_FN(sn_bcast_rows_ragged_f32)
SN_PLAN_FN(sn_segment_colsum_f32)
SN_PLAN_FN(sn_bcast_rows_f32)
SN_PLAN_FN(sn_elu_bwd_bcast_f32)
SN_PLAN_FN(sn_dirac_bsr4_from_mesh)
SN_PLAN_FN(sn_laplacian_csr_from_mesh)
SN_PLAN_FN(sn_edge_lengths_csr_f32)
SN_PLAN_FN(sn_graph_apsp_f32)
SN_PLAN_FN(sn_graph_apsp_sweeps_f32)
SN_PLAN_FN(sn_symmetrize_min_f32)
SN_PLAN_FN(sn_mesh_corners_f32)
SN_PLAN_FN(sn_mesh_geodesics_f32)
SN_PLAN_FN(sn_mesh_geodesics_sweeps_f32)
SN_PLAN_FN(sn_mesh_glue_i32)
SN_PLAN_FN(sn_mesh_idt_rounds_f64)
SN_PLAN_FN(sn_mesh_idt_laplacian_f32)
SN_PLAN_FN(sn_linear_fwd_f32)
SN_PLAN_FN(sn_linear_fwd_tiles_f32)
SN_PLAN_FN(sn_linear_fwd_segbias_tiles_f32)
SN_PLAN_FN(sn_avg_stats_from_tiles_ragged_f32)
SN_PLAN_FN(sn_linear_fwd_segbias_ragged_tiles_f32)
SN_PLAN_FN(sn_avg_stats_from_tiles_f32)
SN_PLAN_FN(sn_colstats_into_f32)
SN_PLAN_FN(sn_colstats_merge_f64)
SN_PLAN_FN(sn_linear_dgrad_f32)
SN_PLAN_FN(sn_linear_dgrad_elu_f32)
SN_PLAN_FN(sn_linear_fwd_segbias_f32)
SN_PLAN_FN(sn_linear_dgrad_eluseg_f32)
SN_PLAN_FN(sn_avg_fwd_prep_f32)
SN_PLAN_FN(sn_avg_stats_f32)
SN_PLAN_FN(sn_seg_affine_f32)
SN_PLAN_FN(sn_avg_bwd_gc_f32)
// ... 7 lines not shown
```

surfacenetworks_amd/functional.py:

```python
from __future__ import annotations

import os

import torch

from . import _lib as _lib_mod
from . import kernels
from .operators import SparseOperator, as_operator

__all__ = ["spmm", "lap_propagate", "dirac_face_stage", "dirac_vert_stage", "avg_propagate", "avg_propagate_ragged", "bn_linear", "bnlin_forward",
           "bnlin_backward", "bn_prepare", "avg_stage_forward_ragged", "avg_stage_backward_ragged", "set_dirac_format", "set_laplacian_format", "SpmmTimer", "thin_linear", "thin_linear_supported"]

_DIRAC_FORMAT = "q3"
_LAPLACIAN_FORMAT = "ring"


def set_laplacian_format(fmt: str) -> None:
    global _LAPLACIAN_FORMAT
    if fmt not in ("ring", "rb4", "csr"):
        raise ValueError(fmt)
    _LAPLACIAN_FORMAT = fmt


def set_dirac_format(fmt: str) -> None:
# ... 69 lines not shown
        return out




def _ctypes_i64_ref():
    import ctypes

    _ctypes_i64_ref.slot = ctypes.c_int64(0)
    return ctypes.addressof(_ctypes_i64_ref.slot)


def product_form(op: SparseOperator, group: int, ncols: int):
    M, K = op.shape
    own = getattr(op, "format", None)
    dfmt = own if own in ("q3", "bsr4", "csr") else _DIRAC_FORMAT
    lfmt = own if own in ("ring", "rb4", "csr") else _LAPLACIAN_FORMAT
    ck = (group, ncols, dfmt, lfmt, kernels.RING_MIN_ROWS)
    cache = op.__dict__.get("_form_cache")
    if cache is not None and cache[0] == ck:
        return cache[1]
    vec = (ncols // group) in (16, 32, 64, 128)
    form = None
    if group == 4 and dfmt == "q3" and vec:
        q = op.q3()
        if q is not None:
            form = ("q3", q, (M, K, int(q[1].shape[0])))
    if form is None:
        b = op.bsr4() if (dfmt != "csr" and group == 4 and vec) else None
        if b is not None:
            form = ("bsr4", b, (M, K, int(b[1].numel())))
        elif lfmt == "ring" and group == 1 and op.ring_ok(ncols):
            form = ("ring", (op.rowptr, op.colind, op.vals), (M, K, int(op.colind.numel())))
        elif lfmt in ("ring", "rb4") and kernels.spmm_rb4_supported(ncols // group, group) and op.rb4() is not None:
            r = op.rb4()
            form = ("rb4", r, (M, K, int(r[1].numel())))
        else:
            form = ("csr", (op.rowptr, op.colind, op.vals), (M, K, int(op.colind.numel())))
    if not (op.is_cuda and torch.cuda.is_current_stream_capturing()):
        op.__dict__["_form_cache"] = (ck, form)
    return form


def _launch(op: SparseOperator, x: torch.Tensor, y: torch.Tensor, group: int, tag: str = "", elubwd=None, stats: bool = False):
    M, K = op.shape
    timer = SpmmTimer.active
    rec = _lib_mod.recorder() if _lib_mod._recorder is not None else None
    if timer is not None or rec is not None:
        known = op._nnz_cache if op._nnz_cache is not None else (int(op._csr[1].numel()) if op._csr is not None else None)
        if rec is not None:
            rec.tags.append((tag, known))
        else:
            timer.tags.append((tag, op if known is None else known))
    e, g = elubwd if elubwd is not None else (None, None)
    vec = (y.shape[1] // group) in (16, 32, 64, 128)
    kind, arr, _ = product_form(op, group, y.shape[1])
    if kind == "q3":
        if stats and e is None and kernels.spmm_q3_stats_supported(y.shape[1] // group, group):
            return kernels.spmm_q3_stats(arr[0], arr[1], M // 4, K // 4, x, y, group)
        am = kernels.spmm_q3(arr[0], arr[1], M // 4, K // 4, x, y, group, e, g, want_absmax=e is not None and kernels.absmax_wanted())
        if am is not None:
            kernels.note_absmax(y, am)
    elif kind == "bsr4":
        if elubwd is None:
            kernels.spmm_bsr4(arr[0], arr[1], arr[2], M // 4, K // 4, x, y, group)
        else:
            kernels.spmm_bsr4_elubwd(arr[0], arr[1], arr[2], M // 4, K // 4, x, e, g, y, group)
    elif kind == "ring":
        if stats and e is None and y.shape[1] == 128:
            return kernels.spmm_ring_stats(arr[0], arr[1], arr[2], M, K, x, y)
        am = kernels.spmm_ring(arr[0], arr[1], arr[2], M, K, x, y, e, g, want_absmax=e is not None and kernels.absmax_wanted())
        if am is not None:
            kernels.note_absmax(y, am)
    elif kind == "rb4":
        if stats and e is None and y.shape[1] == 128:
            return kernels.spmm_rb4_stats(arr[0], arr[1], arr[2], M, K, x, y)
        am = kernels.spmm_rb4(arr[0], arr[1], arr[2], M, K, x, y, e, g, want_absmax=e is not None and kernels.absmax_wanted())
        if am is not None:
            kernels.note_absmax(y, am)
    elif elubwd is None:
        if stats and kernels.spmm_csr_stats_supported(y.shape[1] // group, group):
            return kernels.spmm_csr_stats(arr[0], arr[1], arr[2], M, K, x, y)
        kernels.spmm_csr(arr[0], arr[1], arr[2], M, K, x, y, group)
    elif vec:
        kernels.spmm_csr_elubwd(arr[0], arr[1], arr[2], M, K, x, e, g, y, group)
    else:
        tmp = torch.empty(y.shape, dtype=torch.float32, device=y.device)
        kernels.spmm_csr(arr[0], arr[1], arr[2], M, K, x, tmp, group)
        kernels.elu_bwd(tmp, e, y, False, None, g)
    return None


def _rows2d(x: torch.Tensor) -> torch.Tensor:
    if x.dim() != 2:
        raise ValueError("expected a 2-D dense operand")
    if x.dtype != torch.float32:
        raise TypeError("the Surface-Network path is fp32")
    if x.shape[1] > 1 and x.stride(1) != 1:
        x = x.contiguous()
    return x


class _SpMM(torch.autograd.Function):
    @staticmethod
    def forward(ctx, x, op, group):
        x = _rows2d(x)
        M, K = op.shape
        N = x.shape[1] // group
        y = torch.empty((M // group, group * N), dtype=torch.float32, device=x.device)
        _launch(op, x, y, group, "fwd")
        ctx.op, ctx.group = op, group
        return y

# ... 238 lines not shown
            raise ValueError("bnlin_forward: elu_stats needs a shape the fused GEMM covers")
        _library_gemm("the forward", x.shape[1], W.shape[0])
        y = torch.addmm(bf, x, Wf.t())
        if residual is not None:
            y += residual
        if elu_out is not None:
            kernels.elu_into(y, elu_out)
    return y, (x, W, Wf, s, mean, invstd, beta, training, b is not None, rows_g)


_STRICT = os.environ.get("SN_STRICT", "0") == "1"


def _library_gemm(what: str, K: int, J: int) -> None:
    if _STRICT:
        raise RuntimeError(f"SN_STRICT: {what} of a {K} -> {J} Linear would run on the library GEMM (no hand-written kernel for this shape)")


def _dy_bounds(dy, invstd, rows_g, training):
    if not training or not kernels.absmax_wanted():
        return None
    am = kernels.take_absmax(dy)
    if am is None:
        return None
    return am, invstd, rows_g


def _centered_wgrad(dy, x, mean, bounds=None):
    rows, C = x.shape
    J = dy.shape[1]
    if kernels.wgrad_supported(J, C):
        return kernels.wgrad(dy, x, mean, want_colsum=True, bounds=bounds)
    if C == 64 and rows % 2 == 0 and rows > 0 and x.is_contiguous() and dy.is_contiguous() and kernels.wgrad_supported(2 * J, 2 * C):
        if bounds is not None:
            bounds = (bounds[0], torch.cat([bounds[1], bounds[1]]), bounds[2])
        G2, s2 = kernels.wgrad(dy.view(rows // 2, 2 * J), x.view(rows // 2, 2 * C), torch.cat([mean, mean]), want_colsum=True,
                               bounds=bounds)
        return G2[:J, :C] + G2[J:, C:], s2[:J] + s2[J:]
    _library_gemm("the weight gradient", C, J)
    return dy.t().mm(x - mean), kernels.colstats(dy)


def _wgrad_and_coeffs(dy, x, W, s, mean, invstd, beta, training, has_bias, rows_g):
    bounds = _dy_bounds(dy, invstd, rows_g, training)
    Gc, sdy = _centered_wgrad(dy, x, mean, bounds)
    scale = 1.0
    if training:
        Gc, sdy, scale = _sync_grad_stats(Gc, sdy)
    dW, db, dgamma, dbeta, Bc, Cc = kernels.bn_bwd_coeffs(Gc, sdy, W, s, invstd, beta, rows_g, has_bias)
    dW, db, dgamma, dbeta = _scale_param_grads(scale, dW, db, dgamma, dbeta)
    return dW, db, dgamma, dbeta, Bc, Cc


def bnlin_backward(state, dy, need_dx=True, through_elu=None):
    x, W, Wf, s, mean, invstd, beta, training, has_bias, rows_g = state
    dy = dy.contiguous()
    rows, C = x.shape
    J = dy.shape[1]
    dW, db, dgamma, dbeta, Bc, Cc = _wgrad_and_coeffs(dy, x, W, s, mean, invstd, beta, training, has_bias, rows_g)
    dx = None
    if through_elu is not None and training and kernels.linear_dgrad_elu_supported(J, C):
        dx = kernels.linear_dgrad_elu(dy, Wf, x, mean, Bc, Cc, through_elu[0])
    elif need_dx or through_elu is not None:
        if kernels.linear_dgrad_supported(J, C):
            dx = kernels.linear_dgrad(dy, Wf, x, mean, Bc, Cc) if training else kernels.linear_dgrad(dy, Wf)
        else:
            _library_gemm("the input gradient", C, J)
            dx = dy.mm(Wf)
            if training:
                kernels.affine_cols_acc(dx, x, Bc, Cc, mean)
        if through_elu is not None:
            h = C // 2
            gact = torch.empty((rows, h), dtype=torch.float32, device=dx.device)
            kernels.elu_bwd(dx[:, :h], x[:, :h], gact, False, None, through_elu[0])
            dx = (dx[:, h:], gact)
    return dx, dgamma, dbeta, dW, db


def zero_first_supported(C: int, J: int) -> bool:
    return C == 128 and J == 128 and kernels.linear_fwd_supported(C, J) and kernels.wgrad_supported(J, C) and \
        kernels.linear_dgrad_supported(J, C)


def bnlin_forward_zero_first(p, gamma, beta, W, b, running_mean, running_var, training, momentum, eps, elu_out=None,
                             want_y=True, elu_stats=None):
    part_hi = getattr(p, "_sn_part_hi", None)
    p = _rows2d(p)
    rows, C = p.shape
    stats = None
    rows_g = rows
    nbt = _take_counter(running_mean)
    if training:
        stats = torch.zeros((2, 2 * C), dtype=torch.float64, device=p.device)
        if part_hi is not None and C == 128:
            kernels.colstats_merge_into(part_hi, stats, C)
        else:
            kernels.colstats_into(p, stats, C)
        stats, rows_g = _sync_stats(stats, rows)
    mean, invstd, s, t, Wf, bf = kernels.bn_fold(stats, rows_g, gamma, beta, W, b, eps, momentum, training, running_mean,
                                                 running_var, nbt)
    y = kernels.linear_fwd(p, Wf[:, C:], bf, None, elu_out, want_y, elu_stats)
    return y, (p, W, Wf, s, mean, invstd, beta, training, b is not None, rows_g)


def bnlin_backward_zero_first(state, dy):
    p, W, Wf, s, mean, invstd, beta, training, has_bias, rows_g = state
    dy = dy.contiguous()
    rows, C = p.shape
    J = dy.shape[1]
    b2 = _dy_bounds(dy, invstd[C:], rows_g, training)
    G2, sdy = kernels.wgrad(dy, p, mean[C:], want_colsum=True, bounds=b2)
    Gc = torch.empty((J, 2 * C), dtype=torch.float32, device=G2.device)
    if training:
# ... 256 lines not shown
```

surfacenetworks_amd/kernels.py:

```python
from __future__ import annotations

import torch

from . import _lib

__all__ = [
    "note_absmax", "take_absmax", "absmax_wanted", "clear_absmax", "tile_sums_supported", "new_tile_sums", "avg_stats_from_tiles", "spmm_csr", "spmm_bsr4", "spmm_csr_elubwd", "spmm_bsr4_elubwd", "spmm_q3", "spmm_q3_stats", "spmm_q3_stats_supported", "spmm_csr_stats", "spmm_csr_stats_supported", "csr_to_rb4", "spmm_rb4", "spmm_rb4_stats", "spmm_rb4_supported", "spmm_ring", "spmm_ring_stats", "spmm_ring_supported", "ring_half_window", "csr_band", "bsr4_to_q3", "coo_to_csr", "csr_transpose", "csr_to_bsr4", "blockdiag_concat", "blockdiag_concat_ragged", "validate_csr",
    "elu_into", "elu_bwd", "colstats", "wgrad", "wgrad_supported", "affine_cols_acc", "affine_cols_elu_bwd",
    "bn_fold", "bn_bwd_coeffs", "segment_colsum", "bcast_rows", "segment_colsum_ragged", "bcast_rows_ragged", "elu_bwd_bcast", "dirac_from_mesh", "laplacian_from_mesh", "linear_fwd", "linear_fwd_supported", "linear_dgrad",
    "linear_dgrad_supported", "linear_dgrad_elu", "linear_dgrad_elu_supported",
    "avg_stage_supported", "avg_fwd_prep", "avg_stats", "seg_affine", "avg_bwd_gc", "avg_bwd_segvec", "linear_fwd_segbias", "linear_dgrad_eluseg", "wgrad_seg", "wgrad_slabs", "avg_bwd_segvec_ragged", "linear_fwd_segbias_ragged", "linear_dgrad_eluseg_ragged", "avg_stage_ragged_supported", "wgrad_thin", "wgrad_thin_supported", "linear_thin_fwd", "masked_smooth_l1_fwd", "masked_smooth_l1_bwd", "gather_segments", "pair_argmin", "pair_ce_fwd", "pair_ce_bwd", "pair_fused_fwd", "pair_fused_bwd", "colstats_partial", "linear_fwd_stats_blocks", "elu_stats_supported", "new_elu_stats_part", "colstats_halves", "colstats_into", "colstats_from_part", "colstats_merge_into",
    "avg_merged_supported", "avg_stats_ragged", "avg_stats_from_tiles_ragged", "gather_segments_ragged",
]


def _dev(*tensors) -> None:
    if _lib._recorder is not None and _lib.recorder() is not None and _lib._recorder.allow_cpu:
        return
    for t in tensors:
        if t is not None and not t.is_cuda:
            raise RuntimeError(
                "surfacenetworks_amd kernels run on the MI355X only: got a CPU tensor. There is no CPU/eager "
                "fallback in this package (the reference's CPU torch.sparse path lives in oracle/ for tests).")

# ... 154 lines not shown
            return am
        _lib.call("sn_spmm_csr_ring_elubwd_f32", _p(rowptr), _p(colind), _p(vals), M, K, nnz, _p(x), ldx, N, _p(e), lde, _p(g), ldg,
                  _p(y), ldy, _stream())
    return None


def spmm_ring_stats(rowptr, colind, vals, M: int, K: int, x, y):
    _dev(rowptr, colind, vals, x, y)
    N = y.shape[1]
    if N != 128:
        raise ValueError("spmm_ring_stats: 128-column operands only")
    ldx = _check_dense(x, K, 1, N, "x")
    ldy = _check_dense(y, M, 1, N, "y")
    lib = _lib.load()
    part = torch.empty((int(lib.sn_spmm_q3_stats_blocks()), 2, 128), dtype=torch.float64, device=y.device)
    ws_bytes = int(lib.sn_spmm_csr_ring_stats_workspace_bytes(M))
    ws = torch.empty(max(ws_bytes, 16), dtype=torch.uint8, device=y.device)
    _lib.call("sn_spmm_csr_ring_stats_f32", _p(rowptr), _p(colind), _p(vals), M, K, int(colind.numel()), _p(x), ldx, N, _p(y), ldy,
              _p(part), _p(ws), ws_bytes, _stream())
    return part


def spmm_bsr4(b_rowptr, b_colind, b_vals, Mb: int, Kb: int, x, y, group: int = 1) -> None:
    _dev(b_rowptr, b_colind, b_vals, x, y)
    N = y.shape[1] // group
    ldx = _check_dense(x, 4 * Kb, group, N, "x")
    ldy = _check_dense(y, 4 * Mb, group, N, "y")
    _lib.call("sn_spmm_bsr4_f32", _p(b_rowptr), _p(b_colind), _p(b_vals), Mb, Kb, int(b_colind.numel()),
              _p(x), ldx, group, N, _p(y), ldy, group, _stream())


def spmm_csr_elubwd(rowptr, colind, vals, M: int, K: int, x, e, g, y, group: int = 1) -> None:
    _dev(rowptr, colind, vals, x, e, g, y)
    N = y.shape[1] // group
    ldx = _check_dense(x, K, group, N, "x")
    ldy = _check_dense(y, M, group, N, "y")
    lde = _check_dense(e, M, group, N, "e")
    ldg = _check_dense(g, M, group, N, "g") if g is not None else 0
    _lib.call("sn_spmm_csr_elubwd_f32", _p(rowptr), _p(colind), _p(vals), M, K, int(colind.numel()),
              _p(x), ldx, group, N, _p(e), lde, _p(g), ldg, _p(y), ldy, group, _stream())


def spmm_bsr4_elubwd(b_rowptr, b_colind, b_vals, Mb: int, Kb: int, x, e, g, y, group: int = 1) -> None:
    _dev(b_rowptr, b_colind, b_vals, x, e, g, y)
    N = y.shape[1] // group
    ldx = _check_dense(x, 4 * Kb, group, N, "x")
    ldy = _check_dense(y, 4 * Mb, group, N, "y")
    lde = _check_dense(e, 4 * Mb, group, N, "e")
    ldg = _check_dense(g, 4 * Mb, group, N, "g") if g is not None else 0
    _lib.call("sn_spmm_bsr4_elubwd_f32", _p(b_rowptr), _p(b_colind), _p(b_vals), Mb, Kb, int(b_colind.numel()),
              _p(x), ldx, group, N, _p(e), lde, _p(g), ldg, _p(y), ldy, group, _stream())


def spmm_q3(b_rowptr, q_blk, Mb: int, Kb: int, x, y, group: int = 1, e=None, g=None, want_absmax: bool = False):
    _dev(b_rowptr, q_blk, x, y, e, g)
    N = y.shape[1] // group
    ldx = _check_dense(x, 4 * Kb, group, N, "x")
    ldy = _check_dense(y, 4 * Mb, group, N, "y")
    nblk = int(q_blk.shape[0])
    if e is None:
        _lib.call("sn_spmm_q3_f32", _p(b_rowptr), _p(q_blk), Mb, Kb, nblk, _p(x), ldx, group, N, _p(y), ldy, group, _stream())
    else:
        lde = _check_dense(e, 4 * Mb, group, N, "e")
        ldg = _check_dense(g, 4 * Mb, group, N, "g") if g is not None else 0
        if want_absmax and Mb > 0:
            am = torch.empty(int(_lib.load().sn_spmm_q3_absmax_blocks(Mb, N)), dtype=torch.float32, device=y.device)
            _lib.call("sn_spmm_q3_elubwd_absmax_f32", _p(b_rowptr), _p(q_blk), Mb, Kb, nblk, _p(x), ldx, group, N, _p(e), lde, _p(g),
                      ldg, _p(y), ldy, group, _p(am), _stream())
            return am
        _lib.call("sn_spmm_q3_elubwd_f32", _p(b_rowptr), _p(q_blk), Mb, Kb, nblk, _p(x), ldx, group, N, _p(e), lde, _p(g), ldg,
                  _p(y), ldy, group, _stream())
    return None


def spmm_q3_stats_supported(N: int, group: int) -> bool:
    return N in (16, 32) and group == 4


def spmm_q3_stats(b_rowptr, q_blk, Mb: int, Kb: int, x, y, group: int = 4):
    _dev(b_rowptr, q_blk, x, y)
    N = y.shape[1] // group
    if not spmm_q3_stats_supported(N, group):
        raise ValueError("spmm_q3_stats: 128- or 64-channel operands in the group-4 layout only")
    ldx = _check_dense(x, 4 * Kb, group, N, "x")
    ldy = _check_dense(y, 4 * Mb, group, N, "y")
    lib = _lib.load()
    part = torch.empty((int(lib.sn_spmm_q3_stats_blocks()), 2, 4 * N), dtype=torch.float64, device=y.device)
    ws_bytes = int(lib.sn_spmm_q3_stats_workspace_bytes(Mb))
    ws = torch.empty(max(ws_bytes, 16), dtype=torch.uint8, device=y.device)
    _lib.call("sn_spmm_q3_stats_f32", _p(b_rowptr), _p(q_blk), Mb, Kb, int(q_blk.shape[0]), _p(x), ldx, group, N, _p(y), ldy,
              group, _p(part), _p(ws), ws_bytes, _stream())
    return part


def bsr4_to_q3(b_colind, b_vals):
    _dev(b_colind, b_vals)
    nblk = int(b_colind.numel())
    q = torch.empty((nblk, 4), dtype=torch.float32, device=b_colind.device)
    flag = torch.empty(1, dtype=torch.int32, device=b_colind.device)
    _lib.call("sn_bsr4_to_q3_f32", _p(b_colind), _p(b_vals), nblk, _p(q), _p(flag), _stream())
    return q, flag


def coo_to_csr(idx_batch, idx_row, idx_col, B: int, R: int, Kb: int):
    _dev(idx_batch, idx_row, idx_col)
    nnz = int(idx_row.numel())
    dev = idx_row.device
    rowptr = torch.empty(B * R + 1, dtype=torch.int32, device=dev)
    colind = torch.empty(nnz, dtype=torch.int32, device=dev)
    ib = None if idx_batch is None else idx_batch.contiguous()
    _lib.call("sn_coo_to_csr_i32", _p(ib), _p(idx_row.contiguous()), _p(idx_col.contiguous()), nnz, B, R, Kb,
              _p(rowptr), _p(colind), _stream())
    return rowptr, colind


def csr_transpose(rowptr, colind, vals, M: int, K: int):
    _dev(rowptr, colind, vals)
# ... 67 lines not shown
def elu_bwd(gdst, out, gsrc, accumulate: bool, gdst2=None, gadd=None) -> None:
    _dev(gdst, out, gsrc, gdst2, gadd)
    for t in (gdst2, gadd):
        if t is not None and t.shape != out.shape:
            raise ValueError("elu_bwd: shape mismatch")
    if not (gdst.shape == out.shape == gsrc.shape):
        raise ValueError("elu_bwd: shape mismatch")
    _lib.call("sn_elu_bwd_acc_f32", _p(gdst), _ld(gdst), _p(gdst2), _ld(gdst2) if gdst2 is not None else 0, _p(gadd),
              _ld(gadd) if gadd is not None else 0, _p(out), _ld(out), _p(gsrc), _ld(gsrc), out.shape[0], out.shape[1],
              1 if accumulate else 0, _stream())


def colstats(x):
    _dev(x)
    rows, C = x.shape
    out = torch.empty((2, C), dtype=torch.float64, device=x.device)
    ws_bytes = int(_lib.load().sn_colstats_workspace_bytes(rows, C))
    ws = torch.empty(max(ws_bytes, 16), dtype=torch.uint8, device=x.device)
    _lib.call("sn_colstats_f32", _p(x), _ld(x), rows, C, _p(out), _p(ws), ws_bytes, _stream())
    return out


def wgrad_supported(J: int, C: int) -> bool:
    return C in (128, 256) and J <= 128 and J % 4 == 0


_ABSMAX_KEEP = 8
_absmax_table = {}
_absmax_enabled = None


def absmax_wanted() -> bool:
    global _absmax_enabled
    if _absmax_enabled is None:
        _absmax_enabled = bool(_lib.load().sn_wgrad_bounded_enabled())
    return _absmax_enabled


def note_absmax(t, maxima) -> None:
    if maxima is None:
        return
    if len(_absmax_table) >= _ABSMAX_KEEP:
        for k in list(_absmax_table)[: len(_absmax_table) - _ABSMAX_KEEP + 1]:
            del _absmax_table[k]
    _absmax_table.pop(t.data_ptr(), None)
    _absmax_table[t.data_ptr()] = (t, t._version if not t.is_inference() else None, maxima)
    rec = _lib.recorder() if _lib._recorder is not None else None
    if rec is not None:
        rec.notes.append((t, maxima))


def clear_absmax() -> None:
    _absmax_table.clear()


def take_absmax(t):
    ent = _absmax_table.pop(t.data_ptr(), None)
    if ent is None:
        return None
    src, version, maxima = ent
    rec = _lib.recorder() if _lib._recorder is not None else None
    if rec is not None:
        rec.notes[:] = [n for n in rec.notes if n[1] is not maxima]
    if src.numel() != t.numel() or not t.is_contiguous() or src.dtype != t.dtype or \
            (version is not None and src._version != version):
        return None
    return maxima


def _bounds_args(bounds, C: int):
    dyb, invstd, stat_rows = bounds
    _dev(dyb, invstd)
    if dyb.dtype != torch.float32 or not dyb.is_contiguous() or invstd.dtype != torch.float32 or invstd.numel() != C or \
            not invstd.is_contiguous():
        raise ValueError("wgrad bounds: fp32 maxima of |dy| (contiguous) and the (C,) fp32 inverse standard deviations of x")
    return _p(dyb), int(dyb.numel()), _p(invstd), int(stat_rows)


def wgrad(dy, x, center=None, want_colsum: bool = False, bounds=None):
    _dev(dy, x, center)
    rows, J = dy.shape
    C = x.shape[1]
    if x.shape[0] != rows:
        raise ValueError("wgrad: row mismatch")
    G = torch.empty((J, C), dtype=torch.float32, device=x.device)
    dysum = torch.empty(J, dtype=torch.float64, device=x.device) if want_colsum else None
    ws_bytes = int(_lib.load().sn_wgrad_workspace_bytes(rows, J, C))
    ws = torch.empty(max(ws_bytes, 16), dtype=torch.uint8, device=x.device)
    if bounds is not None:
        _lib.call("sn_wgrad_bounded_f32", _p(dy), _ld(dy), _p(x), _ld(x), _p(center), rows, J, C, _p(G), _p(dysum), _p(ws), ws_bytes,
                  *_bounds_args(bounds, C), _stream())
    else:
        _lib.call("sn_wgrad_f32", _p(dy), _ld(dy), _p(x), _ld(x), _p(center), rows, J, C, _p(G), _p(dysum), _p(ws), ws_bytes,
                  _stream())
    return (G, dysum) if want_colsum else G


def affine_cols_acc(dx, x, B, Cc, center=None) -> None:
    _dev(dx, x, B, Cc, center)
    if dx.shape != x.shape or B.numel() != x.shape[1] or Cc.numel() != x.shape[1]:
        raise ValueError("affine_cols_acc: shape mismatch")
    _lib.call("sn_affine_cols_acc_f32", _p(dx), _ld(dx), _p(x), _ld(x), _p(center), _p(B), _p(Cc), x.shape[0], x.shape[1], _stream())


def affine_cols_elu_bwd(dx, x, B=None, Cc=None, center=None) -> None:
    _dev(dx, x, B, Cc, center)
# ... 482 lines not shown

def colstats_halves(x, part, part_hi=None):
    _dev(x, part, part_hi)
    rows, C2 = x.shape
    C = C2 // 2
    if part is not None and (C not in (64, 128) or part.dim() != 3 or part.shape[1:] != (2, 128) or part.dtype != torch.float64):
        raise ValueError("colstats_halves: expected a (rows, 256 | 128) buffer and (nblk, 2, 128) float64 GEMM partials")
    if part_hi is not None and (C not in (64, 128) or part_hi.dim() != 3 or part_hi.shape[1:] != (2, C) or part_hi.dtype != torch.float64):
        raise ValueError("colstats_halves: expected (nb, 2, C) float64 partials for the propagated half")
    lib = _lib.load()
    out = torch.empty((2, C2), dtype=torch.float64, device=x.device)
    nlo = int(lib.sn_linear_fwd_stats_blocks(rows)) if part is not None else 0
    if part is not None and part.shape[0] < nlo:
        raise ValueError("colstats_halves: partial buffer smaller than the producing launch's grid")
    if part is not None and part_hi is not None:
        _lib.call("sn_colstats_merge2_f64", _p(part), nlo, C, 128, _p(part_hi), int(part_hi.shape[0]), C, C, _p(out), _stream())
        return out
    for half, p_ in ((0, part), (1, part_hi)):
        if p_ is not None and (half == 1 or C == 128):
            nb = nlo if half == 0 else int(p_.shape[0])
            _lib.call("sn_colstats_merge_f64", _p(p_), nb, C, _p(out), C2, half * C, _stream())
        elif p_ is not None:
            raise ValueError("colstats_halves: 64-channel GEMM partials need the SpMM's partials too")
        else:
            xs = x[:, half * C:(half + 1) * C]
            ws_bytes = int(lib.sn_colstats_workspace_bytes(rows, C))
            ws = torch.empty(max(ws_bytes, 16), dtype=torch.uint8, device=x.device)
            _lib.call("sn_colstats_into_f32", _p(xs), _ld(xs), rows, C, _p(out), C2, half * C, _p(ws), ws_bytes, _stream())
    return out


def linear_dgrad_supported(J: int, C: int) -> bool:
    return C in (128, 256) and (J == 128 or (_split_gemm() and 0 < J < 128 and J % 4 == 0))


def linear_dgrad_elu_supported(J: int, C: int) -> bool:
    return 0 < J <= 128 and J % 4 == 0 and C in (128, 256) and _split_gemm()


def linear_dgrad_elu(dy, W, x, center, B, Cc, gadd=None):
    _dev(dy, W, x, center, B, Cc, gadd)
    rows, J = dy.shape
    C = W.shape[1]
    h = C // 2
    dx_hi = torch.empty((rows, h), dtype=torch.float32, device=dy.device)
    gact = torch.empty((rows, h), dtype=torch.float32, device=dy.device)
    am = _new_dgrad_absmax(dy.device)
    _lib.call("sn_linear_dgrad_elu_absmax_f32", _p(dy), _ld(dy), _p(W), _ld(W), _p(x), _ld(x), _p(center), _p(B), _p(Cc),
              _p(dx_hi), h, _p(gact), h, _p(gadd), _ld(gadd) if gadd is not None else 0, rows, J, C, _p(am), _stream())
    note_absmax(gact, am)
    return dx_hi, gact


def _new_dgrad_absmax(device):
    if not absmax_wanted():
        return None
    return torch.empty(int(_lib.load().sn_linear_dgrad_absmax_blocks()), dtype=torch.float32, device=device)


def linear_dgrad(dy, W, x=None, center=None, B=None, Cc=None):
    _dev(dy, W, x, center, B, Cc)
    rows, J = dy.shape
    C = W.shape[1]
    dx = torch.empty((rows, C), dtype=torch.float32, device=dy.device)
    _lib.call("sn_linear_dgrad_f32", _p(dy), _ld(dy), _p(W), _ld(W), _p(x), _ld(x) if x is not None else 0, _p(center),
              _p(B), _p(Cc), _p(dx), C, rows, J, C, _stream())
    return dx


def avg_stage_supported(C: int, J: int, rows_per_seg: int) -> bool:
    return C == 128 and J == 128 and rows_per_seg >= 32 and _split_gemm()


def avg_fwd_prep(segsum, inv_count, rows_per_seg: int, stats1):
    _dev(segsum, inv_count, stats1)
    nseg, C = segsum.shape
    m = torch.empty((nseg, C), dtype=torch.float32, device=segsum.device)
    stats = torch.empty((2, 2 * C), dtype=torch.float64, device=segsum.device)
    _lib.call("sn_avg_fwd_prep_f32", _p(segsum), _p(inv_count.contiguous()), nseg, C, rows_per_seg, _p(stats1), _p(m), _p(stats),
              _stream())
    return m, stats


def avg_stats(e, mask, inv_count, rows_per_seg: int, nseg: int):
    _dev(e, mask, inv_count)
    C = e.shape[1]
    m = torch.empty((nseg, C), dtype=torch.float32, device=e.device)
    stats = torch.empty((2, 2 * C), dtype=torch.float64, device=e.device)
    ws_bytes = int(_lib.load().sn_avg_stats_workspace_bytes(rows_per_seg, nseg, C))
    ws = torch.empty(max(ws_bytes, 16), dtype=torch.uint8, device=e.device)
    _lib.call("sn_avg_stats_f32", _p(e), _ld(e), _p(mask), _p(inv_count.contiguous()), rows_per_seg, nseg, C, _p(m), _p(stats),
              _p(ws), ws_bytes, _stream())
    return m, stats


def seg_affine(A, W, bias):
    _dev(A, W, bias)
    nseg, K = A.shape
    J = W.shape[0]
    out = torch.empty((nseg, J), dtype=torch.float32, device=A.device)
    _lib.call("sn_seg_affine_f32", _p(A), nseg, K, _p(W), _ld(W), _p(bias), J, _p(out), _stream())
    return out


def avg_stats_ragged(m, seg, part, nblk: int):
    _dev(m, part)
# ... 386 lines not shown
```

surfacenetworks_amd/plans.py:

```python
from __future__ import annotations

import bisect
import collections
import ctypes as C
import os
import threading
from typing import List, Optional, Sequence

import torch
from torch.utils._python_dispatch import TorchDispatchMode

from . import _lib, kernels

__all__ = ["enabled", "set_enabled", "set_graphs", "graph_stats", "Site", "stats", "reset", "PlanError"]

_ENABLED = os.environ.get("SN_PLANS", "1") != "0"
_GRAPHS = os.environ.get("SN_PLAN_GRAPHS", "1") != "0"
MAX_EXECS_PER_PLAN = 256
GRAPH_MAX_ARENA_BYTES = 64 << 20
_graveyard = collections.deque()


def _bury(lib, handle) -> None:
    try:
# ... 19 lines not shown
def set_graphs(on: bool) -> None:
    global _GRAPHS
    _GRAPHS = bool(on)
_BIG_BYTES = 1 << 20
_ALIGN = 256
_ALLOW_CPU = False

K_INT, K_DOUBLE, K_PTR, K_NULL, K_STREAM = 0, 1, 2, 3, 4


class PlanError(RuntimeError):
    """The dry run met something a plan cannot express (the block then keeps its eager path)."""


def enabled() -> bool:
    return _ENABLED


def set_enabled(on: bool) -> None:
    global _ENABLED
    _ENABLED = bool(on)


class _Desc:
    __slots__ = ("slot", "off", "eoff", "shape", "stride", "dtype", "attrs", "exact")

    def __init__(self, slot, off, shape, stride, dtype, exact=False):
        self.slot, self.off, self.shape, self.stride, self.dtype = slot, off, shape, stride, dtype
        self.eoff = off // torch.empty((), dtype=dtype).element_size()
        self.attrs = None
        self.exact = exact


def _span_bytes(t: torch.Tensor) -> int:
    if t.numel() == 0:
        return 0
    return (sum((s - 1) * st for s, st in zip(t.shape, t.stride())) + 1) * t.element_size()


_ALLOC_OPS = {"aten::empty", "aten::empty_strided", "aten::empty_like", "aten::new_empty", "aten::new_empty_strided"}
_ZERO_ALLOC_OPS = {"aten::zeros", "aten::zeros_like", "aten::new_zeros"}
_HARMLESS_OPS = {"aten::detach", "aten::alias", "aten::_unsafe_view", "aten::lift_fresh", "aten::detach_"}


class _Recorder(TorchDispatchMode):

    def __init__(self, ext: Sequence[Optional[torch.Tensor]]):
        super().__init__()
        self.ext = list(ext)
        self.nodes: List[tuple] = []
        self.allocs: List[torch.Tensor] = []
        self.stray: List[str] = []
        self.notes: List[tuple] = []
        self.allow_cpu = _ALLOW_CPU
        self.tags: List[tuple] = []

    def record_call(self, name, args):
        self.nodes.append(("call", name, args))

    def __torch_dispatch__(self, func, types, args=(), kwargs=None):
        out = func(*args, **(kwargs or {}))
        name = func._schema.name
        if name in _ALLOC_OPS:
            self.allocs.append(out)
        elif name in _ZERO_ALLOC_OPS:
            self.allocs.append(out)
            self.nodes.append(("memset", out, 0))
        elif getattr(func, "is_view", False) or name in _HARMLESS_OPS:
            pass
        elif name == "aten::zero_":
            self.nodes.append(("memset", args[0], 0))
        elif name == "aten::fill_" and not isinstance(args[1], torch.Tensor) and float(args[1]) == 0.0:
            self.nodes.append(("memset", args[0], 0))
        elif name == "aten::copy_" and isinstance(args[1], torch.Tensor) and args[0].dtype == args[1].dtype and \
                args[0].shape == args[1].shape and args[0].device == args[1].device:
            self.nodes.append(("copy", args[0], args[1]))
        else:
            self.stray.append(name)
        return out


class _Layout:

    def __init__(self, rec: _Recorder, alias_ok=()):
        regions = {}
        for t in rec.allocs:
            st = t.untyped_storage()
            n = int(st.nbytes())
            if n and st.data_ptr() not in regions:
                regions[st.data_ptr()] = n
        self.starts = sorted(regions)
        self.sizes = [regions[p] for p in self.starts]
        self.where = []
        tot = [0, 0]
        for n in self.sizes:
            a = 0 if n >= _BIG_BYTES else 1
            self.where.append((a, tot[a]))
            tot[a] += (n + _ALIGN - 1) // _ALIGN * _ALIGN
        self.arena_bytes = tuple(tot)
        self.ext = []
        for j, t in enumerate(rec.ext):
            if t is not None and t.numel():
                self.ext.append((t.data_ptr(), _span_bytes(t), j))
        by_addr = sorted(self.ext)
        ok = set(alias_ok)
        for (p0, n0, j0), (p1, n1, j1) in zip(by_addr, by_addr[1:]):
# ... 19 lines not shown
            if e is t:
                self.used_ext.add(j)
                return _Desc(2 + j, 0, tuple(t.shape), tuple(t.stride()), t.dtype, exact=True)
        hit = self.resolve(t.data_ptr())
        if hit is None:
            raise PlanError("a result of the block lives in memory the plan does not know (neither its arenas nor its operands)")
        if hit[1] % t.element_size():
            raise PlanError("misaligned result")
        return _Desc(hit[0], hit[1], tuple(t.shape), tuple(t.stride()), t.dtype)


def _attr_tensors(t: torch.Tensor):
    d = getattr(t, "__dict__", None)
    if not d:
        return []
    return [(k, v) for k, v in d.items() if k.startswith("_sn_") and isinstance(v, torch.Tensor)]


def _map_structure(x, fn):
    if isinstance(x, torch.Tensor):
        return fn(x)
    if isinstance(x, (tuple, list)):
        return tuple(_map_structure(v, fn) for v in x)
    if x is None or isinstance(x, (bool, int, float, str)):
        return x
    raise PlanError(f"a block result of type {type(x).__name__} cannot be described")


class Plan:

    _n_alive = 0

    def __init__(self, rec: _Recorder, result, device, alias_ok=()):
        if rec.stray:
            raise PlanError("torch ops that compute inside the block: " + ", ".join(sorted(set(rec.stray))))
        lay = _Layout(rec, alias_ok)
        lib = _lib.load()
        handle = C.c_void_p()
        _lib.check(lib.sn_plan_create(C.byref(handle)), "sn_plan_create")
        self.handle = handle
        self._lib = lib
        Plan._n_alive += 1
        self.device = device
        self.launches = 0
        for node in rec.nodes:
            if node[0] == "call":
                self._add_call(node[1], node[2], lay)
            elif node[0] == "memset":
                self._add_memset(node[1], node[2], lay)
            else:
                self._add_copy(node[1], node[2], lay)
        self.result = _map_structure(result, lambda t: self._describe(t, lay, rec))
        self.effects = [(lay.describe(t, rec), lay.describe(m, rec)) for t, m in rec.notes]
        self.tags = list(rec.tags) if all(k is not None for _, k in rec.tags) else None
        self.arena_bytes = lay.arena_bytes
        self.n_ext = len(rec.ext)
        self.used_ext = sorted(lay.used_ext)
        self._BasesT = C.c_uint64 * (2 + self.n_ext)
        self.bwd = {}
        self.execs = collections.OrderedDict()
        self.graphable = 0 < sum(lay.arena_bytes) <= GRAPH_MAX_ARENA_BYTES and self.launches >= 2

    def _describe(self, t, lay, rec):
        d = lay.describe(t, rec)
        attrs = _attr_tensors(t)
        if attrs and not d.exact:
            d.attrs = [(k, lay.describe(v, rec)) for k, v in attrs]
        return d

    @staticmethod
    def _2d(t: torch.Tensor):
        es = t.element_size()
        if t.is_contiguous():
            return t.numel() * es, t.numel() * es, 1
        if t.dim() == 2 and t.stride(1) == 1 and t.stride(0) >= t.shape[1]:
            return t.stride(0) * es, t.shape[1] * es, t.shape[0]
        return None

    def _slot_of(self, t, lay):
        hit = lay.resolve(t.data_ptr())
        if hit is None:
            raise PlanError("a fill / copy touches memory the plan does not know")
        return hit

    def _add_memset(self, t, byte, lay):
        if t.numel() == 0:
            return
        g = self._2d(t)
        if g is None:
            raise PlanError("fill of a tensor that is neither contiguous nor a 2-D row-strided view")
        slot, off = self._slot_of(t, lay)
        _lib.check(self._lib.sn_plan_add_memset(self.handle, slot, off, byte, g[0], g[1], g[2]), "sn_plan_add_memset")

    def _add_copy(self, dst, src, lay):
        if dst.numel() == 0:
            return
        gd, gs = self._2d(dst), self._2d(src)
        if gd is None or gs is None or (gd[2] != gs[2] and not (gd[2] == 1 and gs[2] == 1)) or gd[1] != gs[1]:
            if gd is not None and gs is not None and dst.dim() == 2 and src.dim() == 2:
                es = dst.element_size()
                gd = (dst.stride(0) * es, dst.shape[1] * es, dst.shape[0])
                gs = (src.stride(0) * es, src.shape[1] * es, src.shape[0])
            else:
                raise PlanError("copy between tensors a 2-D copy cannot address")
        ds, do = self._slot_of(dst, lay)
        ss, so = self._slot_of(src, lay)
# ... 207 lines not shown
    for s in _SITES:
        s.plans.clear()
        s.recorded = s.replayed = s.refused = s.skipped = 0
        s.reasons.clear()
        s.recent.clear()
        s.cooldown = 0


def usable(*tensors) -> bool:
    if not _ENABLED:
        return False
    from .functional import _BN_SYNC

    if _BN_SYNC is not None:
        return False
    for t in tensors:
        if t is not None:
            return t.is_cuda or _ALLOW_CPU
    return False


def expand_ext(tensors: Sequence[Optional[torch.Tensor]], scan: Sequence[int]):
    ext = list(tensors)
    names = []
    for i in scan:
        t = tensors[i]
        if t is not None:
            d = t.__dict__
            if d:
                for k, v in d.items():
                    if k.startswith("_sn_") and isinstance(v, torch.Tensor):
                        ext.append(v)
                        names.append((i, k, v.shape))
    return ext, tuple(names)


def _dry_run(impl, args, ext):
    rec = _Recorder(ext)
    keep = [(t, dict(t.__dict__)) for t in ext if t is not None and hasattr(t, "__dict__")]
    _lib._record_lock.acquire()
    prev, prev_tid = _lib._recorder, _lib._recorder_tid
    _lib._recorder_tid = threading.get_ident()
    _lib._recorder = rec
    try:
        with torch.no_grad(), rec:
            result = impl(*args)
    finally:
        _lib._recorder, _lib._recorder_tid = prev, prev_tid
        _lib._record_lock.release()
        for t, m in rec.notes:
            ent = kernels._absmax_table.get(t.data_ptr())
            if ent is not None and ent[2] is m:
                del kernels._absmax_table[t.data_ptr()]
        for t, before in keep:
            t.__dict__.clear()
            t.__dict__.update(before)
    return rec, result


def record(site: Site, key, impl, args, ext, device, alias_ok=()) -> Optional[Plan]:
    try:
        rec, result = _dry_run(impl, args, ext)
        plan = Plan(rec, result, device, alias_ok)
    except PlanError as exc:
        site.refuse(key, str(exc)[:200])
        return None
    site.store(key, plan)
    site.recorded += 1
    return plan


def renote(grads, maxima) -> None:
    for g, m in zip(grads, maxima):
        if g is not None and m is not None:
            kernels.note_absmax(g, m)


def apply_effects(plan: Plan, build: _Builder) -> None:
    for dt, dm in plan.effects:
        kernels.note_absmax(build(dt), build(dm))
```

Baseline: 3374 meshes/s.

## Defer face-gradient BatchNorm/ELU tail into the next Dirac block's q3 SpMM

Adds a raw-low-half mode to the fused linear dgrad+ELU kernel that writes the un-finished face gradient, and records the per-channel BatchNorm tail (center, B, Cc) alongside it. The next Dirac block's backward then applies that tail inside the q3 ELU-backward SpMM, or falls back to a standalone finish kernel. The aim is to avoid a full read-modify-write of the face gradient between consecutive Dirac blocks by folding the epilogue into the consumer. In exchange it adds tail bookkeeping through the plan recorder and replay path, plus a failure mode if the raw gradient is copied or edited in place between the two backward calls.

Measured after the change: 3467 meshes/s (median of 6 runs). 2.8% higher.

```diff
diff --git a/include/sn_spmm.h b/include/sn_spmm.h
--- a/include/sn_spmm.h
+++ b/include/sn_spmm.h
@@ -58,6 +58,13 @@
                                  const float *X, int64_t ldx, int32_t x_group, int32_t N, const float *E, int64_t lde,
                                  const float *G, int64_t ldg, float *Y, int64_t ldy, int32_t y_group, float *y_absmax,
                                  void *stream);
+int32_t sn_spmm_q3_tail_supported(int32_t N, int32_t y_group);
+int sn_spmm_q3_elubwd_tail_absmax_f32(const int32_t *b_rowptr, const float *q_blk, int64_t Mb, int64_t Kb, int64_t nblocks,
+                                      const float *X, int64_t ldx, int32_t x_group, int32_t N, const float *E, int64_t lde,
+                                      const float *G, int64_t ldg, const float *center, const float *B, const float *Cc,
+                                      float *Y, int64_t ldy, int32_t y_group, float *y_absmax, void *stream);
+int sn_elu_tail_finish_f32(float *g, int64_t ldg, const float *E, int64_t lde, const float *center, const float *B,
+                           const float *Cc, int64_t rows, int32_t C, void *stream);
 int sn_bsr4_to_q3_f32(const int32_t *b_colind, const float *b_vals, int64_t nblocks, float *q_blk,
                       int32_t *not_quaternion, void *stream);
 
@@ -354,6 +361,9 @@
                                    const float *center, const float *B, const float *Cc, float *dx_hi, int64_t lddx,
                                    float *gact, int64_t ldga, const float *gadd, int64_t ldgadd,
                                    int64_t rows, int32_t J, int32_t C, float *gact_absmax, void *stream);
+int sn_linear_dgrad_elu_rawlow_f32(const float *dy, int64_t lddy, const float *W, int64_t ldw, const float *x, int64_t ldx,
+                                   const float *center, const float *B, const float *Cc, float *dx_hi, int64_t lddx,
+                                   float *graw, int64_t ldgr, int64_t rows, int32_t J, int32_t C, void *stream);
 int sn_linear_fwd_segbias_f32(const float *x, int64_t ldx, const float *W, int64_t ldw, const float *segbias,
                               int64_t rows_per_seg, const float *residual, int64_t ldr, float *y, int64_t ldy,
                               float *y_elu, int64_t lde, int64_t rows, int32_t K, int32_t J, double *elu_stats_part,
diff --git a/surfacenetworks_amd/_lib.py b/surfacenetworks_amd/_lib.py
--- a/surfacenetworks_amd/_lib.py
+++ b/surfacenetworks_amd/_lib.py
@@ -81,6 +81,12 @@
     "sn_spmm_q3_absmax_blocks": (_i64, [_i64, _i32]),
     "sn_spmm_q3_elubwd_absmax_f32": (C.c_int, [_vp, _vp, _i64, _i64, _i64, _vp, _i64, _i32, _i32, _vp, _i64, _vp, _i64, _vp, _i64, _i32,
                                                _vp, _vp]),
+    "sn_spmm_q3_tail_supported": (_i32, [_i32, _i32]),
+    "sn_spmm_q3_elubwd_tail_absmax_f32": (C.c_int, [_vp, _vp, _i64, _i64, _i64, _vp, _i64, _i32, _i32, _vp, _i64, _vp, _i64, _vp, _vp, _vp,
+                                                    _vp, _i64, _i32, _vp, _vp]),
+    "sn_elu_tail_finish_f32": (C.c_int, [_vp, _i64, _vp, _i64, _vp, _vp, _vp, _i64, _i32, _vp]),
+    "sn_linear_dgrad_elu_rawlow_f32": (C.c_int, [_vp, _i64, _vp, _i64, _vp, _i64, _vp, _vp, _vp, _vp, _i64, _vp, _i64, _i64, _i32, _i32,
+                                                 _vp]),
     "sn_wgrad_thin_workspace_bytes": (_sz, [_i64, _i32, _i32]),
     "sn_wgrad_thin_f32": (C.c_int, [_vp, _i64, _vp, _i64, _i64, _i32, _i32, _vp, _vp, _vp, _sz, _vp]),
     "sn_masked_smooth_l1_workspace_bytes": (_sz, [_i64, _i32]),
diff --git a/surfacenetworks_amd/blocks.py b/surfacenetworks_amd/blocks.py
--- a/surfacenetworks_amd/blocks.py
+++ b/surfacenetworks_amd/blocks.py
@@ -13,6 +13,9 @@
 from .operators import as_operator
 
 __all__ = ["lap_block", "dirac_block", "avg_block", "avg_block_ragged", "avg_block_ragged_ok", "take_activated", "attach_activated", "zero_faces_ok", "elu_conv", "elu_conv_ok"]
+
+
+DEFER_FACE_TAIL = True
 
 
 def _version_of(t: torch.Tensor):
@@ -158,7 +161,7 @@
     site.replayed += 1
     build = plans._Builder(big, small, ext)
     outs = build(plan.result[0])
-    if plan.effects:
+    if plan.effects or plan.tail_effects:
         plans.apply_effects(plan, build)
     ctx._sn_plan = (plan, big, small, [ext[j] for j in plan.saved_ext], ops, ncols)
     return outs
@@ -173,17 +176,19 @@
     ctx._sn_plan = None
     op_arrays, op_key = _op_operands(ops, ncols) if ops else ((), ())
     maxima = [kernels.take_absmax(g) if g is not None else None for g in grads]
-    ext = [big, small, *kept, *grads, *maxima, *op_arrays]
+    tails = [kernels.take_tail(g) if g is not None else None for g in grads]
+    flat_tails = [t for tl in tails for t in (tl if tl is not None else (None, None, None))]
+    ext = [big, small, *kept, *grads, *maxima, *flat_tails, *op_arrays]
     gptrs = [g.data_ptr() if g is not None else 0 for g in grads]
     key = (tuple([None if g is None else (g.shape, g.stride(), g.dtype) for g in grads]), tuple([m is not None for m in maxima]),
-           op_key, consts, tuple([gptrs.index(p_) for p_ in gptrs]))
+           tuple([tl is not None for tl in tails]), op_key, consts, tuple([gptrs.index(p_) for p_ in gptrs]))
     plan = fplan.bwd.get(key, _MISSING)
     if plan is _MISSING or plan is None:
         fext = [None] * fplan.n_ext
         for j, t in zip(fplan.saved_ext, kept):
             fext[j] = t
         saved = plans._Builder(big, small, fext)(fplan.result[1])
-        plans.renote(grads, maxima)
+        plans.renote(grads, maxima, tails)
         if plan is None:
             return impl(saved, *[o for o, _ in ops], *grads, *consts)
         g0 = 2 + len(kept)
@@ -191,18 +196,19 @@
                             grads_device(grads, big, small), range(g0, g0 + len(grads)))
         fplan.bwd[key] = plan
         if plan is None:
-            plans.renote(grads, maxima)
+            plans.renote(grads, maxima, tails)
             return impl(saved, *[o for o, _ in ops], *grads, *consts)
         for g in grads:
             if g is not None:
                 kernels.take_absmax(g)
+                kernels.take_tail(g)
     timer = SpmmTimer.active
     if timer is not None:
         if plan.tags is None:
             fext = [None] * fplan.n_ext
             for j, t in zip(fplan.saved_ext, kept):
                 fext[j] = t
-            plans.renote(grads, maxima)
+            plans.renote(grads, maxima, tails)
             return impl(plans._Builder(big, small, fext)(fplan.result[1]), *[o for o, _ in ops], *grads, *consts)
         timer.tags.extend(plan.tags)
     b2, s2 = plan.new_arenas(grads_device(grads, big, small))
@@ -210,7 +216,7 @@
     site.replayed += 1
     build = plans._Builder(b2, s2, ext)
     out = build(plan.result)
-    if plan.effects:
+    if plan.effects or plan.tail_effects:
         plans.apply_effects(plan, build)
     return out
 
@@ -264,23 +270,32 @@
     return (v_new, f_out, nxt_v, nxt_f), ((cat0, cat1, nxt_f), st0, st1)
 
 
-def _dirac_bwd(saved, opDi, opDiA, g_vnew, g_fo, f_zero, need_gv, need_gf):
+def _dirac_bwd(saved, opDi, opDiA, g_vnew, g_fo, f_zero, need_gv, need_gf, defer=False, expect_raw=False):
     (cat0, cat1, nxt_f), st0, st1 = saved
     C = cat1.shape[1] // 2
     dev = cat1.device
+    tail = kernels.take_tail(g_fo) if g_fo is not None else None
+    if expect_raw and g_fo is not None and tail is None:
+        raise RuntimeError("dirac_block: a raw face gradient without its tail")
     gp1 = (None,) * 4
     h1 = None
     if g_vnew is not None:
         (dx1_hi, h1), dg1, db1, dW1, dc1 = bnlin_backward(st1, g_vnew, through_elu=(g_vnew,))
         gp1 = (dg1, db1, dW1, dc1)
         g_sum = torch.empty((nxt_f.shape[0], C), dtype=torch.float32, device=dev)
-        _launch(opDiA.t(), dx1_hi, g_sum, 4, "bwd", elubwd=(nxt_f[:, :C], g_fo))
+        _launch(opDiA.t(), dx1_hi, g_sum, 4, "bwd", elubwd=(nxt_f[:, :C], g_fo) if tail is None else (nxt_f[:, :C], g_fo, tail))
         g_fo = g_sum
+    elif tail is not None:
+        kernels.elu_tail_finish(g_fo, nxt_f[:, :C], tail)
     gp0 = (None,) * 4
     g_v = g_f = None
     dx0_hi = None
     if g_fo is not None and f_zero:
         dx0_hi, dg0, db0, dW0, dc0 = bnlin_backward_zero_first(st0, g_fo)
+        gp0 = (dg0, db0, dW0, dc0)
+    elif g_fo is not None and defer and need_gf:
+        (dx0_hi, g_f), dg0, db0, dW0, dc0, tail_f = bnlin_backward(st0, g_fo, through_elu=(None,), raw_low=True)
+        kernels.note_tail(g_f, tail_f)
         gp0 = (dg0, db0, dW0, dc0)
     elif g_fo is not None:
         (dx0_hi, g_f), dg0, db0, dW0, dc0 = bnlin_backward(st0, g_fo, through_elu=(None,))
@@ -306,6 +321,12 @@
             f = _rows2d(f)
         ctx.f_zero = f is None
         ctx.ops = (opDi, opDiA)
+        box = pre_f.__dict__.get("_sn_rawbox") if pre_f is not None else None
+        ctx.defer = bool(DEFER_FACE_TAIL and box is not None and tr0 and v.is_cuda and
+                         kernels.linear_dgrad_elu_supported(W0.shape[0], W0.shape[1]) and W0.shape[1] == 2 * v.shape[1])
+        if ctx.defer:
+            box[0] = True
+        ctx.rawbox = [False] if not need_f else None
         tensors = (v, f, pre_v, pre_f, g0, b0, W0, c0, rm0, rv0, g1, b1, W1, c1, rm1, rv1)
         consts = (need_f, avg_next, tr0, mo0, ep0, tr1, mo1, ep1)
         outs = None
@@ -321,6 +342,8 @@
         v_new, f_out, nxt_v, nxt_f = outs
         if f_out is None:
             f_out = _nan_placeholder(v.device).expand(nxt_f.shape[0], v.shape[1])
+            if ctx.rawbox is not None:
+                nxt_f._sn_rawbox = ctx.rawbox
         ctx.mark_non_differentiable(nxt_v, nxt_f)
         ctx.set_materialize_grads(False)
         return v_new, f_out, nxt_v, nxt_f
@@ -332,7 +355,12 @@
         opDi, opDiA = ctx.ops
         g_vnew = g_vnew.contiguous() if g_vnew is not None else None
         g_fout = g_fout.contiguous() if g_fout is not None else None
-        consts = (ctx.f_zero, bool(ctx.needs_input_grad[0]), bool(ctx.needs_input_grad[1]))
+        consts = (ctx.f_zero, bool(ctx.needs_input_grad[0]), bool(ctx.needs_input_grad[1]), ctx.defer,
+                  bool(ctx.rawbox is not None and ctx.rawbox[0]))
+        if consts[4] and g_fout is not None and not kernels.has_tail(g_fout):
+            raise RuntimeError("dirac_block: the gradient of the face output was left raw by the next Dirac block (DEFER_FACE_TAIL), but "
+                               "what finishes it is gone — the gradient was copied, edited in place, or kernels.clear_absmax() ran "
+                               "between the two backward calls")
         if ctx._sn_planned:
             r = _plan_backward(ctx, _SITES["dirac_bwd"], _dirac_bwd, (g_vnew, g_fout), consts)
         else:
diff --git a/surfacenetworks_amd/csrc/sn_gemm.hip b/surfacenetworks_amd/csrc/sn_gemm.hip
--- a/surfacenetworks_amd/csrc/sn_gemm.hip
+++ b/surfacenetworks_amd/csrc/sn_gemm.hip
@@ -269,7 +269,7 @@
   __builtin_amdgcn_raw_buffer_store_b128(__builtin_bit_cast(u4, v), r, voff, 0, 2);
 }
 
-template <int PC, int K, int NT, bool TRANSW, int EPI, bool SIDE, bool ELU, bool SMALL = false, int WV = 4>
+template <int PC, int K, int NT, bool TRANSW, int EPI, bool SIDE, bool ELU, bool SMALL = false, int WV = 4, bool RAWLOW = false>
 __global__ __launch_bounds__(64 * WV, (PC == 2 && K == 128 && NT == 1 && WV == 4) ? 2 : 1) void gemm_rows_split_k(const float *__restrict__ In, int64_t ldi,
                                                          const float *__restrict__ W, int64_t ldw,
                                                          float *__restrict__ Out, int64_t ldo, int64_t rows, EpiArgs ep) {
@@ -368,22 +368,26 @@
   f4 k0 = {0.f, 0.f, 0.f, 0.f}, k1 = k0, k2 = k0;
   constexpr bool DGE = (EPI == EPI_DGRAD_ELU);
   static_assert(!DGE || SIDE, "the ELU variant needs the BatchNorm tail operand");
+  static_assert(!RAWLOW || DGE, "the raw low half is a form of the input gradient through the activation");
   const bool lowhalf = DGE && 32 * NT * wave < ep.half;
   const bool colv = EPI != EPI_FWD || ecol < ep.jv;
   if constexpr (EPI == EPI_FWD) {
     if (colv) k0 = *reinterpret_cast<const f4 *>(ep.v0 + ecol);
   } else if constexpr (SIDE) {
-    if (ep.v1) k0 = *reinterpret_cast<const f4 *>(ep.v1 + ecol);
-    k1 = *reinterpret_cast<const f4 *>(ep.v2 + ecol);
-    k2 = *reinterpret_cast<const f4 *>(ep.v3 + ecol);
+    if (!(RAWLOW && lowhalf)) {
+      if (ep.v1) k0 = *reinterpret_cast<const f4 *>(ep.v1 + ecol);
+      k1 = *reinterpret_cast<const f4 *>(ep.v2 + ecol);
+      k2 = *reinterpret_cast<const f4 *>(ep.v3 + ecol);
+    }
   }
   const f4 kcs = *reinterpret_cast<const f4 *>(s_cs + ecol);
   unsigned char *const sw = &stg[wave][0] + n * SROW + 16 * h;
   const unsigned char *const sr = &stg[wave][0] + erow * SROW + 16 * (lane % CPR);
   const float *side_p = (EPI == EPI_FWD) ? ep.v1 : ep.v0;
   const bool has_out = (EPI != EPI_FWD && !DGE) || Out != nullptr;
-  const bool has_ga = DGE && lowhalf && ep.v4 != nullptr;
-  const int vo_side = colv ? 4 * (erow * (int)ep.ld1 + ecol) : kOob, js_side = 4 * RPI * (int)ep.ld1;
+  const bool has_ga = DGE && !RAWLOW && lowhalf && ep.v4 != nullptr;
+  const int scol = RAWLOW ? ecol - ep.half : ecol;
+  const int vo_side = (colv && (!RAWLOW || scol >= 0)) ? 4 * (erow * (int)ep.ld1 + scol) : kOob, js_side = 4 * RPI * (int)ep.ld1;
   const int vo_out = colv ? 4 * (erow * (int)ldo + ecol) : kOob, js_out = 4 * RPI * (int)ldo;
   const int vo_o2 = colv ? 4 * (erow * (int)ep.ld2 + ecol) : kOob, js_o2 = 4 * RPI * (int)ep.ld2;
   const int vo_ga = 4 * (erow * (int)ep.ld3 + ecol), js_ga = 4 * RPI * (int)ep.ld3;
@@ -394,7 +398,10 @@
   const int ispan = EPI == EPI_FWD ? K : ep.jv;
   const int ospan = EPI == EPI_FWD ? ep.jv : NOUT;
   w_in.init(In, ldi, row0, last_nrt, ispan);
-  if constexpr (SIDE) w_side.init(side_p, ep.ld1, row0, last_nrt, ospan);
+  if constexpr (SIDE) {
+    if (RAWLOW && lowhalf) w_side.init_empty();
+    else w_side.init(side_p, ep.ld1, row0, last_nrt, RAWLOW ? NOUT - ep.half : ospan);
+  }
   if (has_out) w_out.init(Out, ldo, row0, last_nrt, ospan);
   else w_out.init_empty();
   if constexpr (DGE || (EPI == EPI_FWD && ELU)) w_o2.init(ep.o2, ep.ld2, row0, last_nrt, DGE ? ep.half : ospan);
@@ -477,9 +484,11 @@
     const int nrt = to_last == 0 ? last_nrt : 32;
     f4 sd[NST];
     if constexpr (SIDE) {
-      const rsrc_t r_side = w_side.rsrc(to_last);
-#pragma unroll
-      for (int j = 0; j < NST; ++j) sd[j] = bld4(r_side, vo_side + j * js_side);
+      if (!(RAWLOW && lowhalf)) {
+        const rsrc_t r_side = w_side.rsrc(to_last);
+#pragma unroll
+        for (int j = 0; j < NST; ++j) sd[j] = bld4(r_side, vo_side + j * js_side);
+      }
     }
     f4 sg0 = {0.f, 0.f, 0.f, 0.f}, sg1 = sg0;
     float smk[NST];
@@ -507,7 +516,7 @@
       }
     }
     f4 ga[NST];
-    if constexpr (DGE) {
+    if constexpr (DGE && !RAWLOW) {
       if (lowhalf) {
         const rsrc_t r_ga = w_ga.rsrc(to_last);
 #pragma unroll
@@ -572,7 +581,19 @@
       }
       return v;
     };
-    if constexpr (DGE) {
+    if constexpr (RAWLOW) {
+      if (lowhalf) {
+#pragma unroll
+        for (int j = 0; j < NST; ++j) {
+          f4 v = *reinterpret_cast<const f4 *>(sr + RPI * j * SROW);
+          v *= kcs;
+          bst4(r_o2, vo_o2 + j * js_o2, v);
+        }
+      } else {
+#pragma unroll
+        for (int j = 0; j < NST; ++j) bst4(r_out, vo_out + j * js_out, out_row(j));
+      }
+    } else if constexpr (DGE) {
       if (lowhalf) {
 #pragma unroll
         for (int j = 0; j < NST; ++j) {
@@ -915,6 +936,16 @@
     } else {                                                                                                           \
       if (t_start) hipExtLaunchKernelGGL((gemm_rows_split_k<2, SN_UNPAREN TARGS>), dim3(grid), dim3(kWG), 0, s, t_start, t_stop, 0, __VA_ARGS__); \
       else hipLaunchKernelGGL((gemm_rows_split_k<2, SN_UNPAREN TARGS>), dim3(grid), dim3(kWG), 0, s, __VA_ARGS__);     \
+    }                                                                                                                  \
+  } while (0)
+#define SN_SPLIT_LAUNCH_RAW(NT_, ...)                                                                                  \
+  do {                                                                                                                 \
+    if (rows <= kSmallRows) {                                                                                          \
+      if (t_start) hipExtLaunchKernelGGL((gemm_rows_split_k<2, 128, NT_, true, EPI_DGRAD_ELU, true, false, true, 4, true>), dim3(grid), dim3(kWG), 0, s, t_start, t_stop, 0, __VA_ARGS__); \
+      else hipLaunchKernelGGL((gemm_rows_split_k<2, 128, NT_, true, EPI_DGRAD_ELU, true, false, true, 4, true>), dim3(grid), dim3(kWG), 0, s, __VA_ARGS__); \
+    } else {                                                                                                           \
+      if (t_start) hipExtLaunchKernelGGL((gemm_rows_split_k<2, 128, NT_, true, EPI_DGRAD_ELU, true, false, false, 4, true>), dim3(grid), dim3(kWG), 0, s, t_start, t_stop, 0, __VA_ARGS__); \
+      else hipLaunchKernelGGL((gemm_rows_split_k<2, 128, NT_, true, EPI_DGRAD_ELU, true, false, false, 4, true>), dim3(grid), dim3(kWG), 0, s, __VA_ARGS__); \
     }                                                                                                                  \
   } while (0)
 #define SN_SPLIT_LAUNCH_NT2(K_, EPI_, SIDE_, ...) SN_SPLIT_LAUNCH((K_, 2, true, EPI_, SIDE_, false), __VA_ARGS__)
@@ -1070,6 +1101,31 @@
   else
     SN_SPLIT_LAUNCH((128, 1, true, EPI_DGRAD_ELU, true, false), dy, lddy, W, ldw, out,
                        lddx, rows, ep);
+  return launch_status();
+}
+
+int sn_linear_dgrad_elu_rawlow_f32(const float *dy, int64_t lddy, const float *W, int64_t ldw, const float *x, int64_t ldx,
+                                   const float *center, const float *B, const float *Cc, float *dx_hi, int64_t lddx, float *graw,
+                                   int64_t ldgr, int64_t rows, int32_t J, int32_t C, void *stream) {
+  (void)hipGetLastError();
+  if (rows < 0 || J < 1 || C < 2 || lddy < J || ldw < C || lddx < C / 2 || ldgr < C / 2 || ldx < C) return SN_E_SHAPE;
+  if (J > 128 || (J % 4) || (C != 128 && C != 256) || gemm_variant() == 0 || !ld32(lddy, ldx, lddx, ldgr)) return SN_E_UNSUPPORTED;
+  if (rows == 0) return SN_OK;
+  if (!dy || !W || !dx_hi || !graw || !x || !B || !Cc) return SN_E_NULL;
+  if (!aligned16(dy) || !aligned16(W) || !aligned16(dx_hi) || !aligned16(graw) || !aligned16(x) || !aligned16(B) ||
+      !aligned16(Cc) || (center && !aligned16(center)) || (lddy % 4) || (ldw % 4) || (lddx % 4) || (ldgr % 4) || (ldx % 4))
+    return SN_E_ALIGN;
+  const int half = C / 2;
+  EpiArgs ep{x + half, center, B, Cc, graw, ldx, ldgr, nullptr, 0, half, nullptr, 0, 0, nullptr, nullptr, 0, (int)J, nullptr, 0, nullptr, 1, nullptr};
+  float *out = dx_hi - half;
+  hipStream_t s = static_cast<hipStream_t>(stream);
+  const unsigned grid = gemm_grid(rows, gemm_wgs(128, C / 128));
+  hipEvent_t t_start = nullptr, t_stop = nullptr;
+  sn_internal_timing_slot(0x200 | 2 | 16, rows, C, rows * 4 * ((int64_t)J + half + C), J, &t_start, &t_stop);
+  if (C == 256)
+    SN_SPLIT_LAUNCH_RAW(2, dy, lddy, W, ldw, out, lddx, rows, ep);
+  else
+    SN_SPLIT_LAUNCH_RAW(1, dy, lddy, W, ldw, out, lddx, rows, ep);
   return launch_status();
 }
 
diff --git a/surfacenetworks_amd/csrc/sn_kernels.hip b/surfacenetworks_amd/csrc/sn_kernels.hip
--- a/surfacenetworks_amd/csrc/sn_kernels.hip
+++ b/surfacenetworks_amd/csrc/sn_kernels.hip
@@ -60,6 +60,7 @@
   const float *g;
   int64_t ldg;
   float *absmax = nullptr;
+  const float *center = nullptr, *B = nullptr, *Cc = nullptr;
 };
 __device__ __forceinline__ f4 fabs4(const f4 &a) {
   return f4{__builtin_fabsf(a.x), __builtin_fabsf(a.y), __builtin_fabsf(a.z), __builtin_fabsf(a.w)};
@@ -79,6 +80,26 @@
 __device__ __forceinline__ f4 elu_bwd4(const f4 &a, const f4 &o) {
   return f4{a.x * (o.x > 0.f ? 1.f : o.x + 1.f), a.y * (o.y > 0.f ? 1.f : o.y + 1.f), a.z * (o.z > 0.f ? 1.f : o.z + 1.f),
             a.w * (o.w > 0.f ? 1.f : o.w + 1.f)};
+}
+
+__device__ __forceinline__ float tail_finish1(float p, float e, float ce, float b, float c) {
+  const float xv = e - ce;
+  const float v = p + __builtin_fmaf(xv, b, c);
+  return __builtin_fmaf(v, fminf(e, 0.f), v);
+}
+__device__ __forceinline__ f4 tail_finish4(const f4 &p, const f4 &e, const f4 &ce, const f4 &b, const f4 &c) {
+  return f4{tail_finish1(p.x, e.x, ce.x, b.x, c.x), tail_finish1(p.y, e.y, ce.y, b.y, c.y),
+            tail_finish1(p.z, e.z, ce.z, b.z, c.z), tail_finish1(p.w, e.w, ce.w, b.w, c.w)};
+}
+__global__ __launch_bounds__(kWG) void tail_finish_k(float *__restrict__ g, int64_t ldg, const float *__restrict__ E, int64_t lde,
+                                                     const float *__restrict__ center, const float *__restrict__ B,
+                                                     const float *__restrict__ Cc, int64_t rows, int C4) {
+  const int64_t i = (int64_t)blockIdx.x * kWG + threadIdx.x;
+  if (i >= rows * C4) return;
+  const int64_t r = i / C4;
+  const int c = 4 * (int)(i - r * C4);
+  float *gp = g + r * ldg + c;
+  st4(gp, tail_finish4(ld4(gp), ld4_s(E + r * lde + c, kStreamNT), ld4(center + c), ld4(B + c), ld4(Cc + c)));
 }
 
 template <int N, int XG, int YG, bool EPI, bool STATS>
@@ -363,6 +384,21 @@
   const int ke = b_rowptr[brc + 1 <= Mb ? brc + 1 : Mb];
   const int k0 = __builtin_amdgcn_readfirstlane(kb);
   const int k1 = (stays && r0 >= Mb) ? k0 : __builtin_amdgcn_readlane(ke, 63);
+  constexpr bool TAILN = EPI && (N == 32 || N == 16);
+  constexpr int TAIL_LOADS = (3 * N + 63) / 64;
+  __shared__ f4 s_tail[TAILN ? WAVES : 1][TAILN ? 64 * TAIL_LOADS : 1];
+  bool tail = false;
+  if constexpr (TAILN) {
+    tail = epi.B != nullptr;
+    if (tail) {
+#pragma unroll
+      for (int i = 0; i < TAIL_LOADS; ++i) {
+        const int idx = lane + 64 * i, vec = idx / N, pos = idx % N;
+        const float *src = (vec == 0 ? epi.center : (vec == 1 ? epi.B : epi.Cc)) + 4 * pos;
+        __builtin_amdgcn_global_load_lds(src, s_tail[wave] + 64 * i, 16, 0, 0);
+      }
+    }
+  }
   f4 acc0 = {0.f, 0.f, 0.f, 0.f}, acc1 = acc0, acc2 = acc0, acc3 = acc0;
   for (int t0 = k0; t0 < k1; t0 += TILE) {
     const int nt = (k1 - t0) < TILE ? (k1 - t0) : TILE;
@@ -388,6 +424,10 @@
     __builtin_amdgcn_wave_barrier();
   }
   if constexpr (EPI) {
+    if (tail) {
+      asm volatile("s_waitcnt vmcnt(0)" ::: "memory");
+      __builtin_amdgcn_wave_barrier();
+    }
     if (br < Mb) {
       const int64_t eq = (YG == 4) ? epi.lde : 4 * epi.lde, es = (YG == 4) ? (int64_t)N : epi.lde;
       const float *ep = epi.e + (int64_t)br * eq + sub * 4;
@@ -397,8 +437,18 @@
       if (epi.g) {
         const int64_t gq = (YG == 4) ? epi.ldg : 4 * epi.ldg, gs = (YG == 4) ? (int64_t)N : epi.ldg;
         const float *gp = epi.g + (int64_t)br * gq + sub * 4;
-        acc0 += ld4_s(gp, kStreamNT); acc1 += ld4_s(gp + gs, kStreamNT);
-        acc2 += ld4_s(gp + 2 * gs, kStreamNT); acc3 += ld4_s(gp + 3 * gs, kStreamNT);
+        f4 g0 = ld4_s(gp, kStreamNT), g1 = ld4_s(gp + gs, kStreamNT), g2 = ld4_s(gp + 2 * gs, kStreamNT),
+           g3 = ld4_s(gp + 3 * gs, kStreamNT);
+        if constexpr (TAILN) {
+          if (tail) {
+            const f4 *tv = s_tail[wave] + sub;
+            g0 = tail_finish4(g0, e0, tv[0], tv[N], tv[2 * N]);
+            g1 = tail_finish4(g1, e1, tv[N / 4], tv[N + N / 4], tv[2 * N + N / 4]);
+            g2 = tail_finish4(g2, e2, tv[2 * (N / 4)], tv[N + 2 * (N / 4)], tv[2 * N + 2 * (N / 4)]);
+            g3 = tail_finish4(g3, e3, tv[3 * (N / 4)], tv[N + 3 * (N / 4)], tv[2 * N + 3 * (N / 4)]);
+          }
+        }
+        acc0 += g0; acc1 += g1; acc2 += g2; acc3 += g3;
       }
     }
   }
@@ -2209,6 +2259,11 @@
     if (st) return st;
     if (!aligned16(epi.e) || epi.lde % 4 || (epi.g && (!aligned16(epi.g) || epi.ldg % 4))) return SN_E_ALIGN;
   }
+  if (epi.center || epi.B || epi.Cc) {
+    if (!epi.e || !epi.g || !epi.center || !epi.B || !epi.Cc) return SN_E_NULL;
+    if (!sn_spmm_q3_tail_supported(N, y_group)) return SN_E_UNSUPPORTED;
+    if (!aligned16(epi.center) || !aligned16(epi.B) || !aligned16(epi.Cc)) return SN_E_ALIGN;
+  }
   hipStream_t s = static_cast<hipStream_t>(stream);
   hipEvent_t t_start, t_stop;
   timing_slot(1 | 8 | (epi.e ? 2 : 0) | (epi.g ? 4 : 0) | (stats_part ? 16 : 0), 4 * Mb, 4 * Kb, nblocks, N, &t_start, &t_stop);
@@ -2294,6 +2349,33 @@
   if (!E) return SN_E_NULL;
   return spmm_q3_launch(b_rowptr, q_blk, Mb, Kb, nblocks, X, ldx, x_group, N, Y, ldy, y_group, SpmmEpi{E, lde, G, ldg, y_absmax},
                         stream);
+}
+
+int32_t sn_spmm_q3_tail_supported(int32_t N, int32_t y_group) { return (N == 32 || N == 16) && y_group == 4; }
+
+int sn_spmm_q3_elubwd_tail_absmax_f32(const int32_t *b_rowptr, const float *q_blk, int64_t Mb, int64_t Kb, int64_t nblocks,
+                                      const float *X, int64_t ldx, int32_t x_group, int32_t N, const float *E, int64_t lde,
+                                      const float *G, int64_t ldg, const float *center, const float *B, const float *Cc, float *Y,
+                                      int64_t ldy, int32_t y_group, float *y_absmax, void *stream) {
+  if (!E || !G || !center || !B || !Cc) return SN_E_NULL;
+  SpmmEpi epi{E, lde, G, ldg, y_absmax};
+  epi.center = center;
+  epi.B = B;
+  epi.Cc = Cc;
+  return spmm_q3_launch(b_rowptr, q_blk, Mb, Kb, nblocks, X, ldx, x_group, N, Y, ldy, y_group, epi, stream);
+}
+
+int sn_elu_tail_finish_f32(float *g, int64_t ldg, const float *E, int64_t lde, const float *center, const float *B,
+                           const float *Cc, int64_t rows, int32_t C, void *stream) {
+  (void)hipGetLastError();
+  if (rows < 0 || C < 4 || (C & 3) || ldg < C || lde < C) return SN_E_SHAPE;
+  if (rows == 0) return SN_OK;
+  if (!g || !E || !center || !B || !Cc) return SN_E_NULL;
+  if (!aligned16(g) || !aligned16(E) || !aligned16(center) || !aligned16(B) || !aligned16(Cc) || (ldg & 3) || (lde & 3))
+    return SN_E_ALIGN;
+  hipLaunchKernelGGL(tail_finish_k, dim3(grid_for(rows * (C / 4), kWG)), dim3(kWG), 0, static_cast<hipStream_t>(stream), g, ldg, E,
+                     lde, center, B, Cc, rows, (int)(C / 4));
+  return launch_status();
 }
 
 int sn_bsr4_to_q3_f32(const int32_t *b_colind, const float *b_vals, int64_t nblocks, float *q_blk, int32_t *not_quaternion,
diff --git a/surfacenetworks_amd/csrc/sn_plan_table.inc b/surfacenetworks_amd/csrc/sn_plan_table.inc
--- a/surfacenetworks_amd/csrc/sn_plan_table.inc
+++ b/surfacenetworks_amd/csrc/sn_plan_table.inc
@@ -41,6 +41,9 @@
 SN_PLAN_FN(sn_linear_dgrad_eluseg_absmax_f32)
 SN_PLAN_FN(sn_linear_dgrad_eluseg_ragged_absmax_f32)
 SN_PLAN_FN(sn_spmm_q3_elubwd_absmax_f32)
+SN_PLAN_FN(sn_spmm_q3_elubwd_tail_absmax_f32)
+SN_PLAN_FN(sn_elu_tail_finish_f32)
+SN_PLAN_FN(sn_linear_dgrad_elu_rawlow_f32)
 SN_PLAN_FN(sn_wgrad_thin_f32)
 SN_PLAN_FN(sn_masked_smooth_l1_fwd_f32)
 SN_PLAN_FN(sn_masked_smooth_l1_bwd_f32)
diff --git a/surfacenetworks_amd/functional.py b/surfacenetworks_amd/functional.py
--- a/surfacenetworks_amd/functional.py
+++ b/surfacenetworks_amd/functional.py
@@ -145,13 +145,24 @@
             rec.tags.append((tag, known))
         else:
             timer.tags.append((tag, op if known is None else known))
-    e, g = elubwd if elubwd is not None else (None, None)
+    e, g = elubwd[:2] if elubwd is not None else (None, None)
+    tail = elubwd[2] if elubwd is not None and len(elubwd) > 2 else None
     vec = (y.shape[1] // group) in (16, 32, 64, 128)
     kind, arr, _ = product_form(op, group, y.shape[1])
+    if tail is not None:
+        if g is None:
+            raise ValueError("_launch: a tail without the raw gradient it finishes")
+        if not (kind == "q3" and kernels.spmm_q3_tail_supported(y.shape[1] // group, group)):
+            kernels.elu_tail_finish(g, e, tail)
+            tail = None
     if kind == "q3":
         if stats and e is None and kernels.spmm_q3_stats_supported(y.shape[1] // group, group):
             return kernels.spmm_q3_stats(arr[0], arr[1], M // 4, K // 4, x, y, group)
-        am = kernels.spmm_q3(arr[0], arr[1], M // 4, K // 4, x, y, group, e, g, want_absmax=e is not None and kernels.absmax_wanted())
+        want_am = e is not None and kernels.absmax_wanted()
+        if tail is not None:
+            am = kernels.spmm_q3(arr[0], arr[1], M // 4, K // 4, x, y, group, e, g, want_absmax=want_am, tail=tail)
+        else:
+            am = kernels.spmm_q3(arr[0], arr[1], M // 4, K // 4, x, y, group, e, g, want_absmax=want_am)
         if am is not None:
             kernels.note_absmax(y, am)
     elif kind == "bsr4":
@@ -496,13 +507,18 @@
     return dW, db, dgamma, dbeta, Bc, Cc
 
 
-def bnlin_backward(state, dy, need_dx=True, through_elu=None):
+def bnlin_backward(state, dy, need_dx=True, through_elu=None, raw_low=False):
     x, W, Wf, s, mean, invstd, beta, training, has_bias, rows_g = state
     dy = dy.contiguous()
     rows, C = x.shape
     J = dy.shape[1]
     dW, db, dgamma, dbeta, Bc, Cc = _wgrad_and_coeffs(dy, x, W, s, mean, invstd, beta, training, has_bias, rows_g)
     dx = None
+    if raw_low:
+        if through_elu != (None,) or not training or not kernels.linear_dgrad_elu_supported(J, C):
+            raise RuntimeError("bnlin_backward: the raw low half exists only for the fused training-mode kernel without gadd")
+        h = C // 2
+        return kernels.linear_dgrad_elu_raw(dy, Wf, x, mean, Bc, Cc), dgamma, dbeta, dW, db, (mean[:h], Bc[:h], Cc[:h])
     if through_elu is not None and training and kernels.linear_dgrad_elu_supported(J, C):
         dx = kernels.linear_dgrad_elu(dy, Wf, x, mean, Bc, Cc, through_elu[0])
     elif need_dx or through_elu is not None:
diff --git a/surfacenetworks_amd/kernels.py b/surfacenetworks_amd/kernels.py
--- a/surfacenetworks_amd/kernels.py
+++ b/surfacenetworks_amd/kernels.py
@@ -230,7 +230,20 @@
               _p(x), ldx, group, N, _p(e), lde, _p(g), ldg, _p(y), ldy, group, _stream())
 
 
-def spmm_q3(b_rowptr, q_blk, Mb: int, Kb: int, x, y, group: int = 1, e=None, g=None, want_absmax: bool = False):
+def spmm_q3_tail_supported(N: int, group: int) -> bool:
+    return bool(_lib.load().sn_spmm_q3_tail_supported(int(N), int(group)))
+
+
+def elu_tail_finish(g, e, tail) -> None:
+    center, B, Cc = tail
+    _dev(g, e, center, B, Cc)
+    rows, C = g.shape
+    if e.shape != g.shape or any(t.shape != (C,) or not t.is_contiguous() for t in tail):
+        raise ValueError(f"elu_tail_finish: g {tuple(g.shape)}, e {tuple(e.shape)} and tail vectors of {C} do not match")
+    _lib.call("sn_elu_tail_finish_f32", _p(g), _ld(g), _p(e), _ld(e), _p(center), _p(B), _p(Cc), rows, C, _stream())
+
+
+def spmm_q3(b_rowptr, q_blk, Mb: int, Kb: int, x, y, group: int = 1, e=None, g=None, want_absmax: bool = False, tail=None):
     _dev(b_rowptr, q_blk, x, y, e, g)
     N = y.shape[1] // group
     ldx = _check_dense(x, 4 * Kb, group, N, "x")
@@ -241,6 +254,17 @@
     else:
         lde = _check_dense(e, 4 * Mb, group, N, "e")
         ldg = _check_dense(g, 4 * Mb, group, N, "g") if g is not None else 0
+        if tail is not None:
+            center, B, Cc = tail
+            _dev(center, B, Cc)
+            if g is None or any(t.shape != (group * N,) or not t.is_contiguous() for t in tail):
+                raise ValueError("spmm_q3: a tail needs the raw gradient g and three contiguous vectors of one value per channel")
+            am = None
+            if want_absmax and Mb > 0:
+                am = torch.empty(int(_lib.load().sn_spmm_q3_absmax_blocks(Mb, N)), dtype=torch.float32, device=y.device)
+            _lib.call("sn_spmm_q3_elubwd_tail_absmax_f32", _p(b_rowptr), _p(q_blk), Mb, Kb, nblk, _p(x), ldx, group, N, _p(e), lde,
+                      _p(g), ldg, _p(center), _p(B), _p(Cc), _p(y), ldy, group, _p(am), _stream())
+            return am
         if want_absmax and Mb > 0:
             am = torch.empty(int(_lib.load().sn_spmm_q3_absmax_blocks(Mb, N)), dtype=torch.float32, device=y.device)
             _lib.call("sn_spmm_q3_elubwd_absmax_f32", _p(b_rowptr), _p(q_blk), Mb, Kb, nblk, _p(x), ldx, group, N, _p(e), lde, _p(g),
@@ -414,6 +438,44 @@
 
 def clear_absmax() -> None:
     _absmax_table.clear()
+    _tail_table.clear()
+
+
+_tail_table = {}
+
+
+def note_tail(t, tail) -> None:
+    if len(_tail_table) >= _ABSMAX_KEEP:
+        for k in list(_tail_table)[: len(_tail_table) - _ABSMAX_KEEP + 1]:
+            del _tail_table[k]
+    _tail_table.pop(t.data_ptr(), None)
+    _tail_table[t.data_ptr()] = (t, t._version if not t.is_inference() else None, tuple(tail))
+    rec = _lib.recorder() if _lib._recorder is not None else None
+    if rec is not None:
+        rec.tail_notes.append((t, tuple(tail)))
+
+
+def has_tail(t) -> bool:
+    ent = _tail_table.get(t.data_ptr())
+    if ent is None:
+        return False
+    src, version, _ = ent
+    return src.numel() == t.numel() and t.is_contiguous() and src.dtype == t.dtype and \
+        (version is None or src._version == version)
+
+
+def take_tail(t):
+    ent = _tail_table.pop(t.data_ptr(), None)
+    if ent is None:
+        return None
+    src, version, tail = ent
+    rec = _lib.recorder() if _lib._recorder is not None else None
+    if rec is not None:
+        rec.tail_notes[:] = [n for n in rec.tail_notes if n[1] is not tail]
+    if src.numel() != t.numel() or not t.is_contiguous() or src.dtype != t.dtype or \
+            (version is not None and src._version != version):
+        return None
+    return tail
 
 
 def take_absmax(t):
@@ -1002,6 +1064,18 @@
     return dx_hi, gact
 
 
+def linear_dgrad_elu_raw(dy, W, x, center, B, Cc):
+    _dev(dy, W, x, center, B, Cc)
+    rows, J = dy.shape
+    C = W.shape[1]
+    h = C // 2
+    dx_hi = torch.empty((rows, h), dtype=torch.float32, device=dy.device)
+    graw = torch.empty((rows, h), dtype=torch.float32, device=dy.device)
+    _lib.call("sn_linear_dgrad_elu_rawlow_f32", _p(dy), _ld(dy), _p(W), _ld(W), _p(x), _ld(x), _p(center), _p(B), _p(Cc),
+              _p(dx_hi), h, _p(graw), h, rows, J, C, _stream())
+    return dx_hi, graw
+
+
 def _new_dgrad_absmax(device):
     if not absmax_wanted():
         return None
diff --git a/surfacenetworks_amd/plans.py b/surfacenetworks_amd/plans.py
--- a/surfacenetworks_amd/plans.py
+++ b/surfacenetworks_amd/plans.py
@@ -95,6 +95,7 @@
         self.allocs: List[torch.Tensor] = []
         self.stray: List[str] = []
         self.notes: List[tuple] = []
+        self.tail_notes: List[tuple] = []
         self.allow_cpu = _ALLOW_CPU
         self.tags: List[tuple] = []
 
@@ -220,6 +221,7 @@
                 self._add_copy(node[1], node[2], lay)
         self.result = _map_structure(result, lambda t: self._describe(t, lay, rec))
         self.effects = [(lay.describe(t, rec), lay.describe(m, rec)) for t, m in rec.notes]
+        self.tail_effects = [(lay.describe(t, rec), tuple(lay.describe(v, rec) for v in tl)) for t, tl in rec.tail_notes]
         self.tags = list(rec.tags) if all(k is not None for _, k in rec.tags) else None
         self.arena_bytes = lay.arena_bytes
         self.n_ext = len(rec.ext)
@@ -533,6 +535,10 @@
             ent = kernels._absmax_table.get(t.data_ptr())
             if ent is not None and ent[2] is m:
                 del kernels._absmax_table[t.data_ptr()]
+        for t, tl in rec.tail_notes:
+            ent = kernels._tail_table.get(t.data_ptr())
+            if ent is not None and ent[2] is tl:
+                del kernels._tail_table[t.data_ptr()]
         for t, before in keep:
             t.__dict__.clear()
             t.__dict__.update(before)
@@ -551,12 +557,17 @@
     return plan
 
 
-def renote(grads, maxima) -> None:
+def renote(grads, maxima, tails=None) -> None:
     for g, m in zip(grads, maxima):
         if g is not None and m is not None:
             kernels.note_absmax(g, m)
+    for g, tl in zip(grads, tails or ()):
+        if g is not None and tl is not None:
+            kernels.note_tail(g, tl)
 
 
 def apply_effects(plan: Plan, build: _Builder) -> None:
     for dt, dm in plan.effects:
         kernels.note_absmax(build(dt), build(dm))
+    for dt, dtl in plan.tail_effects:
+        kernels.note_tail(build(dt), build(dtl))
```
